# manhtuando97/two-stage-gnn

Measured on AMD Instinct MI355X. Metric: graphs/sec fwd+bwd, DD batch=32 SAGE-3L h=128, higher is better.
Workload: dtype f32; 1 GPU; DD-shaped synthetic graphs (avg 269 nodes / 676 edges, F_in=89), batch=32 per GPU, GcnEncoderGraph (GraphSage 'base') 3 layers h=128, Nmax=1000, slot-BN, CE loss, clip 2.0 + Adam; 1 step(s) per hipGraph launch, seed = rank, 128 untimed settle steps before the warm-up; global_batch=32, parallelism=dp1, launch=hipGraph replay (one graph: forward + backward + bucket + optimiser), rows=8151, edges_directed=40970

## Files before the change

include/tsgnn.h:

```cpp
#ifndef TSGNN_H
#define TSGNN_H
#include <stdint.h>

typedef struct ihipStream_t* tsgnn_stream_t;

#ifdef __cplusplus
extern "C" {
#endif

#define TSGNN_ABI_VERSION 2
int tsgnn_abi_version(void);
const char* tsgnn_strerror(int code);
const char* tsgnn_last_kernel(void);


int tsgnn_scan_workspace_ints(int64_t n, int64_t* ws_ints);
int tsgnn_exclusive_scan_i32(const int* in, int64_t n, int* out, int* ws, tsgnn_stream_t stream);

int tsgnn_row_maps(const int* graph_ptr, int B, int64_t n_rows, int* row_graph, int* row_slot,
                   tsgnn_stream_t stream);

int tsgnn_dense_adj_count(const float* adj, int B, int nmax, const int* graph_ptr, const int* row_graph,
                          int64_t n_rows, int* row_cnt, tsgnn_stream_t stream);
int tsgnn_dense_adj_fill(const float* adj, int B, int nmax, const int* graph_ptr, const int* row_graph,
                         int64_t n_rows, const int* rowptr, int* col, float* val, tsgnn_stream_t stream);

int tsgnn_coo_count(const int64_t* key, int64_t E, int64_t n_rows, int* cnt, int* bad_flag,
                    tsgnn_stream_t stream);
int tsgnn_coo_fill(const int64_t* key, const int64_t* other, int64_t E, int64_t n_rows, const int* rowptr,
                   int* cursor, int* col, int* eid, tsgnn_stream_t stream);


int tsgnn_ingest_layout(int B, int nmax, int64_t row_cap, int ell_w, int64_t tail_cap, int64_t* off);
int tsgnn_host_collate_tu(const int64_t* ds_graph_ptr, const int64_t* ds_rowptr, const int64_t* ds_col, const int64_t* ds_node_label,
                          const int64_t* ds_graph_label, const int64_t* ids, int B, int nmax, int64_t row_cap, int ell_w,
                          int64_t tail_cap, int32_t* staging, int64_t* out);
int tsgnn_onehot_rows_f32(const int* label, int64_t n_rows, int64_t total_rows, int F, float* x, int64_t ldx, tsgnn_stream_t stream);

int tsgnn_ingest_upload_f32(int32_t* dev, const int32_t* host, int64_t words, const int* node_label_dev, int64_t n_rows, int64_t total_rows,
                            int F, float* x, int64_t ldx, tsgnn_stream_t stream);
int tsgnn_ingest_compact_layout(int B, int nmax, int64_t row_cap, int64_t edge_cap, int64_t tail_cap, int64_t* off);
int tsgnn_host_collate_compact(const int64_t* ds_graph_ptr, const int64_t* ds_rowptr, const int64_t* ds_col, const int64_t* ds_node_label,
                               const int64_t* ds_graph_label, const int64_t* ids, int B, int nmax, int64_t row_cap, int64_t edge_cap,
                               int ell_w, int64_t tail_cap, int32_t* staging, int64_t* out);
int tsgnn_ingest_pull_expand_f32(const int32_t* host, int32_t* mirror, int B, int nmax, int64_t row_cap, int64_t edge_cap, int ell_w,
                                 int64_t tail_cap, int32_t* row_graph, int32_t* row_slot, int32_t* ell, int32_t* tail_ptr, int32_t* ell_slots, int32_t* tail_slots, int F, float* x,
                                 int64_t ldx, tsgnn_stream_t stream);
int tsgnn_ingest_pull_expand_ack_f32(const int32_t* host, int32_t* mirror, int B, int nmax, int64_t row_cap, int64_t edge_cap, int ell_w,
                                     int64_t tail_cap, int32_t* row_graph, int32_t* row_slot, int32_t* ell, int32_t* tail_ptr, int32_t* ell_slots, int32_t* tail_slots, int F,
                                     float* x, int64_t ldx, int64_t* host_ack, tsgnn_stream_t stream);
int tsgnn_ingest_pull_f32(const int32_t* host, int32_t* mirror, int B, int nmax, int64_t row_cap, int64_t edge_cap, int64_t tail_cap,
                          tsgnn_stream_t stream);
int tsgnn_ingest_expand_ack_f32(int32_t* mirror, int B, int nmax, int64_t row_cap, int64_t edge_cap, int ell_w, int64_t tail_cap,
                                int32_t* row_graph, int32_t* row_slot, int32_t* ell, int32_t* tail_ptr, int32_t* ell_slots, int32_t* tail_slots, int F, float* x, int64_t ldx,
                                int64_t* host_ack, tsgnn_stream_t stream);
int tsgnn_ingest_arm_pull_rider(const int32_t* host, int32_t* mirror, int B, int nmax, int64_t row_cap, int64_t edge_cap, int64_t tail_cap);
int tsgnn_ingest_arm_pull_rider_parts(const int32_t* host, int32_t* mirror, int B, int nmax, int64_t row_cap, int64_t edge_cap, int64_t tail_cap,
                                      int parts, int skip);
int tsgnn_ingest_arm_expand_rider(int32_t* mirror, int B, int nmax, int64_t row_cap, int64_t edge_cap, int ell_w, int64_t tail_cap,
                                  int32_t* row_graph, int32_t* row_slot, int32_t* ell, int32_t* tail_ptr, int32_t* ell_slots, int32_t* tail_slots, int F, float* x, int64_t ldx,
                                  int64_t* host_ack);
int tsgnn_ingest_flush_pull_rider(tsgnn_stream_t stream);
int tsgnn_ingest_disarm_riders(void);
typedef struct tsgnn_collate_pool tsgnn_collate_pool;
int tsgnn_collate_pool_create(int nthreads, tsgnn_collate_pool** pool);
int tsgnn_collate_pool_submit(tsgnn_collate_pool* pool, const int64_t* ds_graph_ptr, const int64_t* ds_rowptr, const int64_t* ds_col,
                              const int64_t* ds_node_label, const int64_t* ds_graph_label, const int64_t* ids, int B, int nmax,
                              int64_t row_cap, int64_t edge_cap, int ell_w, int64_t tail_cap, int32_t* staging, int64_t* out,
                              void* after_event, int64_t* ticket);
int tsgnn_collate_pool_submit_ack(tsgnn_collate_pool* pool, const int64_t* ds_graph_ptr, const int64_t* ds_rowptr, const int64_t* ds_col,
                                  const int64_t* ds_node_label, const int64_t* ds_graph_label, const int64_t* ids, int B, int nmax,
                                  int64_t row_cap, int64_t edge_cap, int ell_w, int64_t tail_cap, int32_t* staging, int64_t* out,
                                  const int64_t* host_ack, int64_t ack_target, int seq, int64_t* ticket);
int tsgnn_collate_pool_wait(tsgnn_collate_pool* pool, int64_t ticket);
int tsgnn_collate_pool_destroy(tsgnn_collate_pool* pool);

int tsgnn_csr_transpose(const int* rowptr, const int* col, const float* val, int64_t n_rows, int64_t n_cols,
                        int64_t nnz, int* rowptr_t, int* col_t, float* val_t, int* src_e, int* cnt_ws,
                        int* scan_ws, tsgnn_stream_t stream);


int tsgnn_csr_spmm_f32(const int* rowptr, const int* col, const float* val, const float* self_w,
                       const float* x, int64_t ldx, float* y, int64_t ldy, int64_t n_rows, int feat,
                       float self_scalar, int relu_in, int accumulate, tsgnn_stream_t stream);

int tsgnn_csr_to_ell(const int* rowptr, const int* col, int64_t n_rows, int W, int* ell, int* tail_cnt, tsgnn_stream_t stream);
int tsgnn_csr_tail_fill(const int* rowptr, const int* col, const int* tail_ptr, int64_t n_rows, int W, int* tail_col,
                        tsgnn_stream_t stream);
int tsgnn_ell_spmm_f32(const int* ell, int W, const float* x, int64_t ldx, float* y, int64_t ldy, int64_t n_rows, int feat,
                       float self_scalar, tsgnn_stream_t stream);

int tsgnn_gcn_norm_f32(const int* rowptr, const int* col, const float* val, int64_t n_rows, float self_fill,
                       float* dinv, float* val_out, float* self_w, tsgnn_stream_t stream);

int tsgnn_sddmm_rows_f32(const int* rowptr, const int* col, const float* dy, int64_t lddy, const float* x, int64_t ldx,
                         int64_t n_rows, int feat, float* dval, float* dself, tsgnn_stream_t stream);


int tsgnn_gemm_f32(const float* A, int64_t sam, int64_t sak, const float* B, int64_t sbk, int64_t sbn, float* C,
                   int64_t scm, int64_t scn, int M, int N, int K, int batch, int64_t stride_a, int64_t stride_b,
                   int64_t stride_c, const int* seg_ptr, int ragged, int max_seg, float alpha, int accumulate,
                   tsgnn_stream_t stream);
int tsgnn_gemm_splitk_plan(int M, int N, int K, int* ksplit, int64_t* ws_floats);
int tsgnn_gemm_splitk_f32(const float* A, int64_t sam, int64_t sak, const float* B, int64_t sbk, int64_t sbn,
                          float* C, int M, int N, int K, int ksplit, float* ws, int accumulate,
                          tsgnn_stream_t stream);
int tsgnn_linear_wgrad_plan(int64_t rows, int K_in, int N, int64_t ldz, int64_t lddu, int* nslab, int64_t* rows_per_slab,
                            int64_t* ws_floats);
int tsgnn_linear_wgrad_f32(const float* z, int64_t ldz, const float* du, int64_t lddu, int64_t rows, int K_in, int N, int nslab,
                           int64_t rows_per_slab, int64_t bias_only_rows, float* ws, float* dw, float* db, tsgnn_stream_t stream);
int tsgnn_wgrad_reduce_sets_blocks(const int64_t* desc);
int tsgnn_wgrad_reduce_sets_f32(const int64_t* desc, float* normparts, float* step_state, tsgnn_stream_t stream);
int tsgnn_wgrad_reduce_multi_f32(const float* ws0, int nslab0, int K0, int N0, float* dw0, float* db0, const float* ws1, int nslab1,
                                 int K1, int N1, float* dw1, float* db1, const float* ws2, int nslab2, int K2, int N2, float* dw2,
                                 float* db2, const float* ws3, int nslab3, int K3, int N3, float* dw3, float* db3,
                                 float* normparts, float* step_state, tsgnn_stream_t stream);
int tsgnn_wgrad_blocks_plan(int64_t rows, int K_in, int N, int64_t ldz, int64_t lddu, int* nslab, int64_t* rows_per_slab,
                            int64_t* ws_floats);
int tsgnn_wgrad_blocks_f32(const float* z, int64_t ldz, const float* du, int64_t lddu, int64_t rows, int K_in, int N, int nslab,
                           int64_t rows_per_slab, float* ws, float* dw, int64_t lddw, tsgnn_stream_t stream);
int tsgnn_wgrad_blocks_oi_f32(const float* z, int64_t ldz, const float* du, int64_t lddu, int64_t rows, int K_in, int N, int nslab,
                              int64_t rows_per_slab, float* ws, float* dw_oi, int64_t lddw, float* db, tsgnn_stream_t stream);
int tsgnn_ragged_tn_f32(const float* s_mat, int64_t lds_, const float* x, int64_t ldx, int K, int N, const int* slab_row_ptr,
                        int nslab, const int* seg_slab_ptr, int nseg, float* ws, float* out, tsgnn_stream_t stream);
int tsgnn_ragged_tn_direct_supported(int K, int64_t max_rows);
int tsgnn_ragged_tn_direct_f32(const float* s_mat, int64_t lds_, int K, const int* graph_ptr, int B, const float* x0, int64_t ldx0,
                               int N0, float* out0, const float* x1, int64_t ldx1, int N1, float* out1, tsgnn_stream_t stream);
int tsgnn_ragged_tn_direct_ro_f32(const float* s_mat, int64_t lds_, int K, const int* graph_ptr, int B, const float* x0, int64_t ldx0,
                                  int N0, float* out0, const float* x1, int64_t ldx1, int N1, float* out1, float* ro_out,
                                  int64_t ro_ldo, int* ro_arg, int nmax, int64_t n_real, int ghost_zero, tsgnn_stream_t stream);
int tsgnn_wgrad_narrow_plan(int64_t rows, int K_in, int N, int64_t* ws_floats);
int tsgnn_wgrad_narrow_f32(const float* z, int64_t ldz, const float* du, int64_t lddu, int64_t rows, int K_in, int N, float* ws,
                           float* dwb, tsgnn_stream_t stream);
int tsgnn_colsum_f32(const float* x, int64_t ld, int64_t rows, int F, float* out, float* ws, int accumulate,
                     tsgnn_stream_t stream);

int tsgnn_linear_l2norm_f32(const float* z, int64_t ldz, const float* w, int64_t ldw, const float* bias, float* v,
                            int64_t ldv, float* rinv, int64_t rows, int K, int N, int normalize,
                            tsgnn_stream_t stream);
int tsgnn_rowgemm_supported(const float* a, int64_t lda, const float* b, int64_t ldb, const float* c, int64_t ldc, int K, int N,
                            int trans_b);
int tsgnn_rowgemm_f32(const float* a, int64_t lda, const float* b, int64_t ldb, int trans_b, const float* bias, float* c,
                      int64_t ldc, float* rinv, int64_t rows, int K, int N, int normalize, int64_t fill_rows,
                      tsgnn_stream_t stream);
int tsgnn_panel_blocks(int64_t rows, int panel_units);
#define TSGNN_SCHED_8x32 32
#define TSGNN_SCHED_16x24 24
int tsgnn_gather_sched_slots(int64_t rows, int64_t fill_rows, int K, int panel_units, int layer0);
int tsgnn_gather_rowgemm_f32(const int* ell, int ell_w, const int* tail_ptr, const int* tail_col, const float* x, int64_t ldx, const float* b, int64_t ldb, int trans_b,
                             const float* bias, float* c, int64_t ldc, float* rinv, float* zout, int64_t ldz, int64_t rows, int K,
                             int N, int normalize, int64_t fill_rows, tsgnn_stream_t stream);
int tsgnn_gather_rowgemm_st_f32(const int* ell, int ell_w, const int* tail_ptr, const int* tail_col, const float* x, int64_t ldx, const float* b, int64_t ldb, const float* bias,
                                float* c, int64_t ldc, float* rinv, float* zout, int64_t ldz, int64_t rows, int K, int N,
                                int64_t fill_rows, const int* row_slot, unsigned long long* sums, float* ghost, int panel_units,
                                const int64_t* pack_desc, tsgnn_stream_t stream);
int tsgnn_sage_layer_fwd_bn_f32(const int* ell, int ell_w, const int* tail_ptr, const int* tail_col, const float* x, int64_t ldx, const float* w, int64_t ldw, const float* bias,
                                float* v, int64_t ldv, float* rinv, float* zout, int64_t ldz, int64_t rows, int K, int64_t fill_rows,
                                const int* graph_ptr, const int* slot_count, int B, int nslots, int n_ghost, unsigned long long* packed,
                                unsigned long long* packed_out, const int* row_graph, const unsigned long long* sums_in,
                                const float* ghost_in, float* mean_out, float* rstd_out, const int* row_slot,
                                unsigned long long* sums_out, float* ghost_out, const int* ro_map, int ro_map_ch, int panel_units,
                                const float* w_img, tsgnn_stream_t stream);
int tsgnn_sage_layer_fwd_bn_plan(int64_t rows, int64_t fill_rows, int B, int nslots, int panel_units, int* ro_ch, int* n_gemm,
                                 int* n_full);
int tsgnn_sage_layer_fwd_f32(const int* ell, int ell_w, const int* tail_ptr, const int* tail_col, const float* x, int64_t ldx, const float* w, int64_t ldw, const float* bias,
                             float* v, int64_t ldv, float* rinv, float* zout, int64_t ldz, int64_t rows, int K, int64_t fill_rows,
                             const int* graph_ptr, int B, int nslots, int n_ghost, unsigned long long* packed, tsgnn_stream_t stream);
int tsgnn_sage_layer_fwd_ro_f32(const int* ell, int ell_w, const int* tail_ptr, const int* tail_col, const float* x, int64_t ldx, const float* w, int64_t ldw, const float* bias,
                                float* v, int64_t ldv, float* rinv, float* zout, int64_t ldz, int64_t rows, int K, int64_t fill_rows,
                                const int* graph_ptr, int B, int nslots, int n_ghost, unsigned long long* packed,
                                unsigned long long* packed_out, const int* row_graph, tsgnn_stream_t stream);
int tsgnn_sage_layer_bwd_f32(const int* ell, int ell_w, const int* tail_ptr, const int* tail_col, const float* du, int64_t lddu, const float* w, int64_t ldw, float* dxs,
                             int64_t lddxs, const float* z, int64_t ldz, int64_t rows, int nslab, int64_t rows_per_slab,
                             int64_t bias_only_rows, float* ws, int panel_units, const float* w_img, tsgnn_stream_t stream);
int tsgnn_l2norm_bwd_f32(const float* v, int64_t ldv, const float* dv, int64_t lddv, const float* rinv, float* du,
                         int64_t lddu, int64_t rows, int F, tsgnn_stream_t stream);


int tsgnn_bn_slots_fwd_f32(const int* graph_ptr, const int* slot_count, const int* row_slot, int B, int nmax,
                           int64_t n_real, int n_ghost, const float* v, int64_t ldv, int F, int relu, int bn,
                           float* mean, float* rstd, float* y, int64_t ldy, tsgnn_stream_t stream);
int tsgnn_bn_slots_bwd_f32(const int* graph_ptr, const int* slot_count, const int* row_slot, int B, int nmax,
                           int64_t n_real, int n_ghost, const float* v, int64_t ldv, const float* dy, int64_t lddy, int F,
                           int relu, int bn, const float* mean, const float* rstd, float* m1, float* m2, float* dv,
                           int64_t lddv, tsgnn_stream_t stream);

int tsgnn_row_ln_fwd_f32(const float* v, int64_t ldv, int64_t rows, int F, int relu, float* mean, float* rstd, float* y, int64_t ldy,
                         tsgnn_stream_t stream);
int tsgnn_row_ln_bwd_f32(const float* v, int64_t ldv, const float* dy, int64_t lddy, int64_t rows, int F, int relu, const float* mean,
                         const float* rstd, float* dv, int64_t lddv, tsgnn_stream_t stream);

int tsgnn_row_post_bwd_f32(const int* row_graph, int B, int64_t n_real, int64_t rows, const float* v, int64_t ldv, const float* dxs,
                           int64_t lddxs, const float* dout, int64_t ldo, const int* arg, int F, int relu, int ln, const float* mean,
                           const float* rstd, const float* rinv, float* du, int64_t lddu, tsgnn_stream_t stream);

int tsgnn_row_post_nodes_bwd_f32(int64_t n_real, int64_t rows, const float* v, int64_t ldv, const float* dxs, int64_t lddxs,
                                 const float* dnode, int64_t lddn, int ghost_zero, int F, int relu, int ln, const float* mean,
                                 const float* rstd, const float* rinv, float* du, int64_t lddu, tsgnn_stream_t stream);

int tsgnn_readout_max_ws_words(int B, int nmax, int F);
int tsgnn_readout_max_fwd_f32(const int* graph_ptr, const int* slot_count, int B, int nmax, int64_t n_real, int n_ghost,
                              const float* x, int64_t ldx, int F, int relu, unsigned long long* packed_ws, float* out,
                              int64_t ldo, int* arg, tsgnn_stream_t stream);
int tsgnn_readout_max_bwd_f32(const float* dout, int64_t ldo, const int* arg, int B, int F, const float* x, int64_t ldx_in,
                              int relu, int64_t n_real, float* dx, int64_t ldx, tsgnn_stream_t stream);
int tsgnn_readout_max_bwd_rows_f32(const float* dout, int64_t ldo, const int* arg, const int* row_graph, int F, int64_t rows,
                                   int64_t rows_total, const float* add, int64_t ldadd, float* dx, int64_t ldx, tsgnn_stream_t stream);

int tsgnn_pack_rows_f32(const float* src, int nmax, int F, const int* row_graph, const int* row_slot, int64_t n_real,
                        float* dst, int64_t ld, tsgnn_stream_t stream);
int tsgnn_unpack_rows_f32(const int* graph_ptr, int B, int nmax, int64_t n_real, int n_ghost, const float* src, int64_t ld,
                          int F, float fill, float* dst, tsgnn_stream_t stream);
int tsgnn_unpack_rows_bwd_ghost_f32(const int* graph_ptr, int B, int nmax, int64_t n_real, const float* ddst, int F,
                                    float* dsrc, int64_t ld, tsgnn_stream_t stream);


int tsgnn_softmax_ce_f32(const float* logits, int64_t ld, const int64_t* label, int B, int C, float* loss, float* dlogits,
                         tsgnn_stream_t stream);
int tsgnn_adam_from_partials_f32(float* param, const float* grad, float* m, float* v, int64_t n, float lr, float beta1, float beta2,
                                 float eps, float weight_decay, float max_norm, float* state, const float* parts, int nparts,
                                 const float* poison, tsgnn_stream_t stream);
int tsgnn_clip_adam_step_f32(float* param, const float* grad, float* m, float* v, int64_t n, float lr, float beta1,
                             float beta2, float eps, float weight_decay, float max_norm, float grad_scale, float* state,
                             float* ws, const float* poison, tsgnn_stream_t stream);


int tsgnn_dense_stack_supported(int B, int K, int nstack, int L, int fin0, int hidden, int last0, int last1);
int tsgnn_dense_stack_fwd_f32(const int64_t* desc, tsgnn_stream_t stream);
int tsgnn_dense_stack_bwd_f32(const int64_t* desc, tsgnn_stream_t stream);
int tsgnn_dense_stack_max_resident(void);
int tsgnn_dense_stack_barrier_selftest(unsigned* sync, float* err, int expect, tsgnn_stream_t stream);


int tsgnn_node_scores_f32(const float* x, int64_t ldx, int64_t rows, int H, int Fh, const float* a, int64_t lda, float* s,
                          tsgnn_stream_t stream);
int tsgnn_node_scores2_f32(const float* x, int64_t ldx, int64_t rows, int H, int Fh, const float* a1, int64_t lda1, float* s1,
                           const float* a2, int64_t lda2, float* s2, tsgnn_stream_t stream);
int tsgnn_edge_softmax_fwd_f32(const int* rowptr, const int* col, int64_t rows, int H, const float* s_grp, const float* s_oth,
                               int mod, float slope, float* alpha, tsgnn_stream_t stream);
int tsgnn_edge_softmax_bwd_f32(const int* rowptr, const int* col, int64_t rows, int H, const float* s_grp, const float* s_oth,
                               int mod, float slope, const float* alpha, const float* dalpha, float* dt, float* ds_grp,
                               tsgnn_stream_t stream);
int tsgnn_edge_permute_f32(const float* src, const int* perm, int64_t n, int H, int scatter, float* dst, tsgnn_stream_t stream);
int tsgnn_csr_row_sum_f32(const int* rowptr, const float* val, int64_t rows, int H, float* out, tsgnn_stream_t stream);
int tsgnn_csr_row_sum_perm_f32(const int* rowptr, const float* val, const int* eperm, int64_t rows, int H, float* out,
                               tsgnn_stream_t stream);
int tsgnn_csr_spmm_heads_f32(const int* rowptr, const int* col, const float* alpha, int H, int Fh, const float* x, int64_t ldx,
                             int mod, float* y, int64_t ldy, int64_t rows, tsgnn_stream_t stream);
int tsgnn_csr_spmm_heads_epi_f32(const int* rowptr, const int* col, const float* alpha, int H, int Fh, const float* x, int64_t ldx,
                                 int mod, float* y, int64_t ldy, int64_t rows, const float* w1, const float* a1, int64_t lda1,
                                 const float* w2, const float* a2, int64_t lda2, const float* u, int64_t ldu, const float* uw,
                                 int rows_per_seg, const int* row_seg, float uscale, const int* eperm, tsgnn_stream_t stream);
int tsgnn_csr_sddmm_heads_f32(const int* rowptr, const int* col, int H, int Fh, const float* dy, int64_t lddy, const float* x,
                              int64_t ldx, int mod, float* dalpha, int64_t rows, tsgnn_stream_t stream);
int tsgnn_segment_wsum_f32(const float* x, int64_t ldx, const float* w, int H, int Fh, const int* seg_ptr, int nseg, int64_t rows,
                           int64_t max_seg, float scale, int mean, float* ws, float* out, int64_t ldo, tsgnn_stream_t stream);
int tsgnn_segment_wsum2_f32(const float* x, int64_t ldx, const float* w1, const float* w2, int H, int Fh, const int* seg_ptr, int nseg,
                            int64_t rows, int64_t max_seg, float scale, float* ws, float* out1, float* out2, int64_t ldo,
                            tsgnn_stream_t stream);
int tsgnn_gather_wsum_f32(const float* x, int64_t ldx, const int* idx, const float* w, const int* seg_ptr, int nseg, int C, float scale,
                          float* out, int64_t ldo, tsgnn_stream_t stream);
int tsgnn_broadcast_add_f32(float* y, int64_t ldy, int64_t rows, int H, int Fh, const float* w, const float* a, int64_t lda,
                            const float* u, int64_t ldu, int rows_per_seg, float scale, tsgnn_stream_t stream);
int tsgnn_pack_heads_max(void);
int tsgnn_pack_heads_f32(const float* w0, const float* w1, const float* w2, const float* w3, const float* w4, const float* w5,
                         const float* w6, const float* w7, const float* a0, const float* a1, const float* a2, const float* a3,
                         const float* a4, const float* a5, const float* a6, const float* a7, int H, int Fin, int Fo, float* W, float* A,
                         tsgnn_stream_t stream);
int tsgnn_unpack_heads_f32(const float* dW, const float* dA0, const float* dA1, int H, int Fin, int Fo, float* gw, float* ga,
                           tsgnn_stream_t stream);

int tsgnn_gat_fused_supported(int H, int Fh);
int tsgnn_gat_attn_fwd_f32(const float* hp, int64_t ldh, const int* rowptr, const int* col, const int* rp_t, const int* col_t,
                           int64_t rows, int H, int Fh, float slope, const int* row_graph, int nmax, const int* iso_idx,
                           const float* iso_w, const int* iso_ptr, float uscale, int mean_heads, int apply_elu, float drop_p,
                           uint64_t seed, const unsigned long long* drop_ctr, float* stat, float* y, int64_t ldy, tsgnn_stream_t stream);
int tsgnn_gat_bwd_parts(int B);
int tsgnn_gat_attn_bwd_f32(const float* hp, int64_t ldh, const float* y, int64_t ldy, const float* dy, int64_t lddy, const int* rp_t,
                           const int* col_t, int64_t rows, int H, int Fh, float slope, int mean_heads, int apply_elu,
                           const int* graph_ptr, int B, const int* iso_idx, const float* iso_w, const int* iso_ptr,
                           const float* iso_row, int iso_row_ld, float uscale, float drop_p, uint64_t seed,
                           const unsigned long long* drop_ctr, const float* stat, float* dhp, int Ns, float* t1, float* t2, float* S,
                           float* dupart, tsgnn_stream_t stream);
int tsgnn_gat_attn_bwd_ro_f32(const float* hp, int64_t ldh, const float* y, int64_t ldy, const float* dy, int64_t lddy, const int* rp_t,
                              const int* col_t, int64_t rows, int H, int Fh, float slope, int mean_heads, int apply_elu,
                              const int* graph_ptr, int B, const int* iso_idx, const float* iso_w, const int* iso_ptr,
                              const float* iso_row, int iso_row_ld, float uscale, float drop_p, uint64_t seed,
                              const unsigned long long* drop_ctr, const float* stat, float* dhp, int Ns, float* t1, float* t2, float* S,
                              float* dupart, const float* ro_dout, int64_t ro_ldo, const int* ro_arg, const int* row_graph,
                              tsgnn_stream_t stream);
int tsgnn_gat_dropout_mult_f32(float drop_p, uint64_t seed, const unsigned long long* drop_ctr, int64_t i0, int64_t ni, int64_t j0,
                               int64_t nj, int H, float* out, tsgnn_stream_t stream);
int tsgnn_gat_score_rowsum_f32(const int* rowptr, const int* col, const int* eperm, const float* t1, const float* t2, const float* S,
                               int64_t rows, int H, float* dhp, int64_t ldh, int C, const float* dupart, int B, const int* iso_idx,
                               const float* iso_w, const int* iso_ptr, float uscale, tsgnn_stream_t stream);
int tsgnn_gat_pack_desc_words(void);
int tsgnn_gat_pack_f32(const int64_t* desc, tsgnn_stream_t stream);
int tsgnn_gat_unpack_f32(const int64_t* desc, tsgnn_stream_t stream);
int tsgnn_elu_heads_fwd_f32(const float* x, int64_t rows, int H, int Fh, int mean_heads, int apply_elu, float* y, tsgnn_stream_t stream);
int tsgnn_elu_heads_bwd_f32(const float* x, const float* dy, int64_t rows, int H, int Fh, int mean_heads, int apply_elu, float* dx,
                            tsgnn_stream_t stream);


int tsgnn_mlp3_supported(int B, int D0, int D1, int D2, int C);
int tsgnn_mlp3_fwd_f32(const float* x, int64_t ldx, const float* w1, const float* b1, const float* keep, float keep_scale, const float* w2,
                       const float* b2, const float* w3, const float* b3, int B, int D0, int D1, int D2, int C, float* a1, float* a2,
                       float* logp, tsgnn_stream_t stream);
int tsgnn_mlp3_fwd_drop_f32(const float* x, int64_t ldx, const float* w1, const float* b1, float p, uint64_t seed,
                            unsigned long long* state, unsigned long long* used, const float* w2, const float* b2, const float* w3,
                            const float* b3, int B, int D0, int D1, int D2, int C, float* a1, float* a2, float* logp,
                            tsgnn_stream_t stream);
int tsgnn_mlp3_dropout_mask_f32(float p, uint64_t seed, uint64_t counter, int B, int D1, float* out, tsgnn_stream_t stream);
int tsgnn_mlp3_bwd_f32(const float* x, int64_t ldx, const float* w1, const float* w2, const float* w3, const float* a1,
                       const float* a2, const float* logp, const float* dlogp, float keep_scale, int B, int D0, int D1, int D2, int C,
                       float* dw1, float* db1, float* dw2, float* db2, float* dw3, float* db3, float* dx, int64_t lddx,
// ... 306 lines not shown
```

two-stage-gnn_amd/csrc/head.hip:

```cpp
#include "common.h"
#include "../../include/tsgnn.h"
#include "readout_body.h"
#include "ingest_rider.h"

namespace {

__device__ __forceinline__ float4 ld4(const float* p) { return *reinterpret_cast<const float4*>(p); }
__device__ __forceinline__ float pick4(const float (&r)[4], int q) { return q == 0 ? r[0] : q == 1 ? r[1] : q == 2 ? r[2] : r[3]; }

constexpr int HW = 16;

__device__ __forceinline__ void head2_fwd_tail(const float* xs, float* vs, int b, const float* __restrict__ w1,
                                               const float* __restrict__ b1, const float* __restrict__ w2, const float* __restrict__ b2,
                                               int P, int E, int C, float* __restrict__ vec, float* __restrict__ y) {
  const int tid = threadIdx.x, lane = tid & 63, wid = tid >> 6;
  const int P4 = P >> 2;
  for (int j0 = wid; j0 < E; j0 += 8 * HW) {
    float acc[8];
#pragma unroll
    for (int u = 0; u < 8; ++u) acc[u] = 0.f;
    for (int k4 = lane; k4 < P4; k4 += 64) {
      const float4 x = *reinterpret_cast<const float4*>(xs + 4 * k4);
      float4 w[8];
#pragma unroll
      for (int u = 0; u < 8; ++u) {
        const int j = j0 + HW * u;
        w[u] = ld4(w1 + (int64_t)(j < E ? j : 0) * P + 4 * k4);
      }
#pragma unroll
      for (int u = 0; u < 8; ++u) acc[u] += (w[u].x * x.x + w[u].y * x.y) + (w[u].z * x.z + w[u].w * x.w);
    }
#pragma unroll
    for (int u = 0; u < 8; ++u) {
      const int j = j0 + HW * u;
      const float r = wave_sum(acc[u]);
      if (lane == 0 && j < E) { const float v = r + (b1 ? b1[j] : 0.f); vs[j] = v; vec[(int64_t)b * E + j] = v; }
    }
  }
  __syncthreads();
  for (int c = wid; c < C; c += HW) {
    float acc = 0.f;
    for (int j = lane; j < E; j += 64) acc = fmaf(w2[(int64_t)c * E + j], vs[j], acc);
    acc = wave_sum(acc);
    if (lane == 0) y[(int64_t)b * C + c] = acc + (b2 ? b2[c] : 0.f);
  }
}

struct RoTail {
  const float* z; int64_t ldz; int N, c0, F;
  int* arg;
  float* dz; int64_t lddz;
};

__global__ __launch_bounds__(64 * HW) void head2_fwd_kernel(float* __restrict__ out, int64_t ldo, const float* __restrict__ w1,
                                                        const float* __restrict__ b1, const float* __restrict__ w2,
                                                        const float* __restrict__ b2, int P, int E, int C,
                                                        float* __restrict__ vec, float* __restrict__ y, RoTail rt) {
  extern __shared__ __attribute__((aligned(16))) float smem[];
  float* xs = smem;
  float* vs = smem + ((P + 3) & ~3);
  const int b = blockIdx.x, tid = threadIdx.x;
  const int c0 = rt.z ? rt.c0 : P;
  for (int k = tid; k < P; k += 64 * HW) {
    if (k < c0) { xs[k] = out[(int64_t)b * ldo + k]; continue; }
    const int f = k - c0;
    unsigned long long best = 0ull;
    for (int n0 = 0; n0 < rt.N; n0 += 16) {
      float val[16];
#pragma unroll
      for (int u = 0; u < 16; ++u) val[u] = rt.z[((int64_t)b * rt.N + min(n0 + u, rt.N - 1)) * rt.ldz + f];
#pragma unroll
      for (int u = 0; u < 16; ++u) {
        if (n0 + u < rt.N) {
          const unsigned long long q = ((unsigned long long)f32_ordered(val[u]) << 32) |
                                       (unsigned long long)(0xFFFFFFFFu - (unsigned)(b * rt.N + n0 + u));
          best = q > best ? q : best;
        }
      }
    }
    const float v = best ? ordered_f32((unsigned)(best >> 32)) : 0.f;
    xs[k] = v;
    out[(int64_t)b * ldo + k] = v;
    rt.arg[(int64_t)b * rt.F + f] = best ? (int)(0xFFFFFFFFu - (unsigned)(best & 0xFFFFFFFFull)) : -1;
  }
  __syncthreads();
  head2_fwd_tail(xs, vs, b, w1, b1, w2, b2, P, E, C, vec, y);
}

struct ReadoutHeadArgs {
  const unsigned long long* packed; int B, L, Fh, Fl;
  const float* v_last; int64_t ldv;
  const int* graph_ptr; int64_t n_real; int nslots; int n_ghost;
  float* out; int64_t ldo; int* arg;
};
__global__ __launch_bounds__(64 * HW) void readout_head_fwd_kernel(ReadoutHeadArgs a, const float* __restrict__ w1,
                                                               const float* __restrict__ b1, const float* __restrict__ w2,
                                                               const float* __restrict__ b2, int P, int E, int C,
                                                               float* __restrict__ vec, float* __restrict__ y) {
  extern __shared__ __attribute__((aligned(16))) float smem[];
  float* xs = smem;
  float* vs = smem + ((P + 3) & ~3);
  unsigned long long* best = reinterpret_cast<unsigned long long*>(smem + ((P + 3) & ~3) + ((E + 3) & ~3));
  const int b = blockIdx.x, tid = threadIdx.x;
  const int PH = (a.L - 1) * a.Fh;
  for (int k = tid; k < PH; k += 64 * HW) {
    const int l = k / a.Fh, f = k % a.Fh;
    const int64_t i = (int64_t)l * a.B * a.Fh + (int64_t)b * a.Fh + f;
    const unsigned long long p = a.packed[i];
    const float val = p ? ordered_f32((unsigned)(p >> 32)) : 0.f;
    xs[k] = val;
    a.out[(int64_t)b * a.ldo + k] = val;
    a.arg[i] = p ? (int)(0xFFFFFFFFu - (unsigned)(p & 0xFFFFFFFFull)) : -1;
  }
  {
    const int c4 = tid & 31, rl = tid >> 5, F4 = a.Fl >> 2;
    const int g0 = a.graph_ptr[b], sz = a.graph_ptr[b + 1] - g0;
    unsigned long long m0 = 0ull, m1 = 0ull, m2 = 0ull, m3 = 0ull;
    if (c4 < F4) {
      const int nrows = sz + ((a.n_ghost && sz < a.nslots) ? 1 : 0);
      for (int n0 = rl; n0 < nrows; n0 += 8 * HW) {
        float4 t[4];
        int64_t r[4];
#pragma unroll
        for (int u = 0; u < 4; ++u) {
          const int n = n0 + 2 * HW * u;
          r[u] = n < sz ? (int64_t)g0 + n : a.n_real + n;
          t[u] = n < nrows ? ld4(a.v_last + r[u] * a.ldv + 4 * c4) : make_float4(0.f, 0.f, 0.f, 0.f);
        }
#pragma unroll
        for (int u = 0; u < 4; ++u) {
          if (n0 + 2 * HW * u < nrows) {
            const unsigned long long p0 = pack_max(t[u].x, (unsigned)r[u]), p1 = pack_max(t[u].y, (unsigned)r[u]),
                                     p2 = pack_max(t[u].z, (unsigned)r[u]), p3 = pack_max(t[u].w, (unsigned)r[u]);
            m0 = p0 > m0 ? p0 : m0; m1 = p1 > m1 ? p1 : m1; m2 = p2 > m2 ? p2 : m2; m3 = p3 > m3 ? p3 : m3;
          }
        }
      }
      best[rl * a.Fl + 4 * c4 + 0] = m0; best[rl * a.Fl + 4 * c4 + 1] = m1; best[rl * a.Fl + 4 * c4 + 2] = m2; best[rl * a.Fl + 4 * c4 + 3] = m3;
    }
    __syncthreads();
    for (int f = tid; f < a.Fl; f += 64 * HW) {
      unsigned long long m = best[f];
      for (int w = 1; w < 2 * HW; ++w) { const unsigned long long o = best[w * a.Fl + f]; m = o > m ? o : m; }
      const float val = m ? ordered_f32((unsigned)(m >> 32)) : 0.f;
      xs[PH + f] = val;
      a.out[(int64_t)b * a.ldo + PH + f] = val;
      a.arg[(int64_t)(a.L - 1) * a.B * a.Fh + (int64_t)b * a.Fl + f] = m ? (int)(0xFFFFFFFFu - (unsigned)(m & 0xFFFFFFFFull)) : -1;
    }
  }
  __syncthreads();
  head2_fwd_tail(xs, vs, b, w1, b1, w2, b2, P, E, C, vec, y);
}

template <int NJ>
__global__ __launch_bounds__(64 * HW) void packed_head_fwd_kernel(const unsigned long long* __restrict__ packed, int B, int L, int Fh,
                                                              int Fl, float* __restrict__ out, int64_t ldo, int* __restrict__ arg,
                                                              const float* __restrict__ w1, const float* __restrict__ b1,
                                                              const float* __restrict__ w2, const float* __restrict__ b2, int P, int E,
                                                              int C, float* __restrict__ vec, float* __restrict__ y, ExpandRider rider,
                                                              unsigned long long* __restrict__ clear, int64_t clear_n, int clear_packed) {
  extern __shared__ __attribute__((aligned(16))) float smem[];
  if ((int)blockIdx.x >= B) {
    expand_rider_body(rider, blockIdx.x - (unsigned)B, 64 * HW);
    return;
  }
  for (int64_t i2 = (int64_t)blockIdx.x * (64 * HW) + threadIdx.x; i2 < clear_n; i2 += (int64_t)B * (64 * HW)) clear[i2] = 0ull;
  float* xs = smem;
  float* vs = smem + ((P + 3) & ~3);
  const int b = blockIdx.x, tid = threadIdx.x, lane = tid & 63, wid = tid >> 6;
  const int PH = (L - 1) * Fh, P4 = P >> 2;
  unsigned long long pk[2];
  int64_t pidx[2];
#pragma unroll
  for (int u = 0; u < 2; ++u) {
    const int k = tid + u * 64 * HW;
    int64_t idx = 0;
    if (k < P) {
      if (k < PH) { const int l = k / Fh, f = k - l * Fh; idx = (int64_t)l * B * Fh + (int64_t)b * Fh + f; }
      else idx = (int64_t)(L - 1) * B * Fh + (int64_t)b * Fl + (k - PH);
    }
    pidx[u] = idx;
    pk[u] = packed[idx];
    if (k >= P) pk[u] = 0ull;
  }
  float4 w[NJ][2];
#pragma unroll
  for (int u = 0; u < NJ; ++u) {
    const int j = wid + HW * u;
    const float* row = w1 + (int64_t)(j < E ? j : 0) * P;
    w[u][0] = ld4(row + 4 * (lane < P4 ? lane : 0));
    w[u][1] = ld4(row + 4 * (lane + 64 < P4 ? lane + 64 : 0));
  }
#pragma unroll
  for (int u = 0; u < NJ; ++u) {
    if (lane >= P4) w[u][0] = make_float4(0.f, 0.f, 0.f, 0.f);
    if (lane + 64 >= P4) w[u][1] = make_float4(0.f, 0.f, 0.f, 0.f);
  }
  float bj[NJ];
#pragma unroll
  for (int u = 0; u < NJ; ++u) { const int j = wid + HW * u; bj[u] = (b1 && j < E) ? b1[j] : 0.f; }
  float w2v[4];
#pragma unroll
  for (int q = 0; q < 4; ++q) { const int j = lane + 64 * q; w2v[q] = (wid < C && j < E) ? w2[(int64_t)wid * E + j] : 0.f; }
  const float b2v = (b2 && wid < C) ? b2[wid] : 0.f;
#pragma unroll
  for (int u = 0; u < 2; ++u) {
    const int k = tid + u * 64 * HW;
    if (k < P) {
      const unsigned long long p = pk[u];
      const float val = p ? ordered_f32((unsigned)(p >> 32)) : 0.f;
      xs[k] = val;
      out[(int64_t)b * ldo + k] = val;
      arg[pidx[u]] = p ? (int)(0xFFFFFFFFu - (unsigned)(p & 0xFFFFFFFFull)) : -1;
      if (clear_packed) const_cast<unsigned long long*>(packed)[pidx[u]] = 0ull;
    }
  }
  __syncthreads();
  {
    const float4 x0 = lane < P4 ? *reinterpret_cast<const float4*>(xs + 4 * lane) : make_float4(0.f, 0.f, 0.f, 0.f);
    const float4 x1 = lane + 64 < P4 ? *reinterpret_cast<const float4*>(xs + 4 * (lane + 64)) : make_float4(0.f, 0.f, 0.f, 0.f);
    float acc[NJ];
#pragma unroll
    for (int u = 0; u < NJ; ++u)
      acc[u] = ((w[u][0].x * x0.x + w[u][0].y * x0.y) + (w[u][0].z * x0.z + w[u][0].w * x0.w)) +
               ((w[u][1].x * x1.x + w[u][1].y * x1.y) + (w[u][1].z * x1.z + w[u][1].w * x1.w));
    for (int k4 = lane + 128; k4 < P4; k4 += 64) {
      const float4 x = *reinterpret_cast<const float4*>(xs + 4 * k4);
#pragma unroll
      for (int u = 0; u < NJ; ++u) {
        const int j = wid + HW * u;
        const float4 t = ld4(w1 + (int64_t)(j < E ? j : 0) * P + 4 * k4);
        acc[u] += (t.x * x.x + t.y * x.y) + (t.z * x.z + t.w * x.w);
      }
    }
#pragma unroll
    for (int u = 0; u < NJ; ++u) {
      const int j = wid + HW * u;
      const float r = wave_sum(acc[u]);
      if (lane == 0 && j < E) { const float v = r + bj[u]; vs[j] = v; vec[(int64_t)b * E + j] = v; }
    }
  }
  __syncthreads();
  for (int c = wid; c < C; c += HW) {
    float acc = 0.f;
    if (c == wid && E <= 256) {
#pragma unroll
      for (int q = 0; q < 4; ++q) { const int j = lane + 64 * q; if (j < E) acc = fmaf(w2v[q], vs[j], acc); }
    } else {
      for (int j = lane; j < E; j += 64) acc = fmaf(w2[(int64_t)c * E + j], vs[j], acc);
    }
    acc = wave_sum(acc);
    if (lane == 0) y[(int64_t)b * C + c] = acc + ((c == wid) ? b2v : (b2 ? b2[c] : 0.f));
  }
}

__device__ __forceinline__ void head2_bwd_rows(float* smem, int b, const float* __restrict__ dy, const float* __restrict__ dvec,
                                               const float* __restrict__ w1, const float* __restrict__ w2, int P, int E, int C,
                                               float* __restrict__ dout, int64_t ldo) {
  float* ds = smem;
  float* part = smem + ((E + 3) & ~3);
  const int tid = threadIdx.x, wid = tid >> 6, lane = tid & 63;
  for (int j = tid; j < E; j += 64 * HW) {
    float acc = dvec ? dvec[(int64_t)b * E + j] : 0.f;
    for (int c = 0; c < C; ++c) acc = fmaf(dy[(int64_t)b * C + c], w2[(int64_t)c * E + j], acc);
    ds[j] = acc;
  }
  __syncthreads();
  const int P4 = P >> 2;
  for (int k4 = lane; k4 < P4 + ((P & 3) ? 1 : 0); k4 += 64) {
    float4 acc = make_float4(0.f, 0.f, 0.f, 0.f);
    if (k4 < P4) {
      for (int j = wid; j < E; j += HW) {
        const float4 w = ld4(w1 + (int64_t)j * P + 4 * k4);
        const float d = ds[j];
        acc.x = fmaf(d, w.x, acc.x); acc.y = fmaf(d, w.y, acc.y); acc.z = fmaf(d, w.z, acc.z); acc.w = fmaf(d, w.w, acc.w);
      }
      *reinterpret_cast<float4*>(part + wid * ((P + 3) & ~3) + 4 * k4) = acc;
    } else {
      for (int k = 4 * P4; k < P; ++k) {
        float a = 0.f;
        for (int j = wid; j < E; j += HW) a = fmaf(ds[j], w1[(int64_t)j * P + k], a);
        part[wid * ((P + 3) & ~3) + k] = a;
      }
    }
  }
  __syncthreads();
  const int PP = (P + 3) & ~3;
  for (int k = tid; k < P; k += 64 * HW) {
    float a = 0.f;
#pragma unroll
    for (int w = 0; w < HW; ++w) a += part[w * PP + k];
    dout[(int64_t)b * ldo + k] = a;
  }
}

__device__ __forceinline__ void head2_bwd_weights(float* smem , int jb, const float* __restrict__ out, int64_t ldo,
                                                  const float* __restrict__ vec, const float* __restrict__ dy,
                                                  const float* __restrict__ dvec, const float* __restrict__ w2, int B, int P, int E,
                                                  int C, float* __restrict__ dw1, float* __restrict__ db1, float* __restrict__ dw2,
                                                  float* __restrict__ db2, float* __restrict__ normparts) {
  const int tid = threadIdx.x, NTH = 64 * HW;
  const int nj = (E + 3) / 4;
  float sq = 0.f;
  if (jb < nj) {
    const int j0 = 4 * jb;
    for (int i = tid; i < B * 4; i += NTH) {
      const int bb = i >> 2, jj = j0 + (i & 3);
      float a = 0.f;
      if (jj < E) {
        a = dvec ? dvec[(int64_t)bb * E + jj] : 0.f;
        for (int c = 0; c < C; ++c) a = fmaf(dy[(int64_t)bb * C + c], w2[(int64_t)c * E + jj], a);
      }
      smem[i] = a;
    }
    __syncthreads();
    for (int k = tid; k < P; k += NTH) {
      float a0 = 0.f, a1 = 0.f, a2 = 0.f, a3 = 0.f;
      int bb = 0;
      for (; bb + 8 <= B; bb += 8) {
        float x[8];
#pragma unroll
        for (int u = 0; u < 8; ++u) x[u] = out[(int64_t)(bb + u) * ldo + k];
#pragma unroll
        for (int u = 0; u < 8; ++u) {
          const float4 d = *reinterpret_cast<const float4*>(smem + 4 * (bb + u));
          a0 = fmaf(d.x, x[u], a0); a1 = fmaf(d.y, x[u], a1); a2 = fmaf(d.z, x[u], a2); a3 = fmaf(d.w, x[u], a3);
        }
      }
      for (; bb < B; ++bb) {
        const float x = out[(int64_t)bb * ldo + k];
        a0 = fmaf(smem[4 * bb + 0], x, a0); a1 = fmaf(smem[4 * bb + 1], x, a1);
        a2 = fmaf(smem[4 * bb + 2], x, a2); a3 = fmaf(smem[4 * bb + 3], x, a3);
      }
      if (j0 + 0 < E) { dw1[(int64_t)(j0 + 0) * P + k] = a0; sq = fmaf(a0, a0, sq); }
      if (j0 + 1 < E) { dw1[(int64_t)(j0 + 1) * P + k] = a1; sq = fmaf(a1, a1, sq); }
      if (j0 + 2 < E) { dw1[(int64_t)(j0 + 2) * P + k] = a2; sq = fmaf(a2, a2, sq); }
      if (j0 + 3 < E) { dw1[(int64_t)(j0 + 3) * P + k] = a3; sq = fmaf(a3, a3, sq); }
    }
    if (db1 && tid < 4 && j0 + tid < E) {
      float a = 0.f;
      for (int bb = 0; bb < B; ++bb) a += smem[4 * bb + tid];
      db1[j0 + tid] = a;
      sq = fmaf(a, a, sq);
    }
  } else {
    for (int i = tid; i < C * E; i += NTH) {
      const int c = i / E, j = i % E;
      float a = 0.f;
      for (int bb = 0; bb < B; ++bb) a = fmaf(dy[(int64_t)bb * C + c], vec[(int64_t)bb * E + j], a);
      dw2[i] = a;
      sq = fmaf(a, a, sq);
    }
    if (db2) for (int c = tid; c < C; c += NTH) {
      float a = 0.f;
      for (int bb = 0; bb < B; ++bb) a += dy[(int64_t)bb * C + c];
      db2[c] = a;
      sq = fmaf(a, a, sq);
    }
  }
  if (normparts) {
    sq = wave_sum(sq);
    __syncthreads();
    if ((tid & 63) == 0) smem[tid >> 6] = sq;
    __syncthreads();
    if (tid == 0) {
      float t = 0.f;
      for (int w = 0; w < HW; ++w) t += smem[w];
      normparts[jb] = t;
    }
  }
}

__global__ __launch_bounds__(64 * HW) void head2_bwd_kernel(const float* __restrict__ out, int64_t ldo, const float* __restrict__ vec,
                                                        const float* __restrict__ dy, const float* __restrict__ dvec,
                                                        const float* __restrict__ w1, const float* __restrict__ w2, int B, int P, int E,
                                                        int C, float* __restrict__ dout, int64_t lddo, float* __restrict__ dw1,
                                                        float* __restrict__ db1, float* __restrict__ dw2, float* __restrict__ db2,
                                                        float* __restrict__ normparts, const float* __restrict__ ce_y,
                                                        const int64_t* __restrict__ ce_label, float* __restrict__ ce_loss) {
  extern __shared__ __attribute__((aligned(16))) float smem_all[];
  float* smem = smem_all;
  if (ce_label != nullptr) {
    float* dyl = smem_all;
    float* lb = smem_all + ((B * C + 3) & ~3);
    smem = lb + ((B + 3) & ~3);
    const float invB = 1.f / (float)B;
    const bool all_rows = (int)blockIdx.x >= B || blockIdx.x == 0;
    for (int b = all_rows ? (int)threadIdx.x : (int)blockIdx.x + (int)threadIdx.x * B; b < B; b += 64 * HW) {
      const float* row = ce_y + (int64_t)b * C;
      float m = -INFINITY;
      for (int c = 0; c < C; ++c) m = fmaxf(m, row[c]);
      float d = 0.f;
// ... 313 lines not shown
#pragma unroll
    for (int u = 0; u < WB_ROWS; ++u) {
      const int bb = bg + G * u;
      x[u] = ld4(out + (int64_t)((active && bb < B) ? bb : 0) * ldo + 4 * (active ? k4 : 0));
    }
    if (has_ce) { ce_rows(ce, B, C, dyl, lb, -1); __syncthreads(); }
    for (int i = tid; i < 4 * B; i += NTH) {
      const int bb = i >> 2, jj = j0 + (i & 3);
      float a = 0.f;
      if (jj < E) {
        a = i == tid ? dv0 : (dvec ? dvec[(int64_t)bb * E + jj] : 0.f);
        for (int c = 0; c < C; ++c) a = fmaf(dy[(int64_t)bb * C + c], (i == tid && c < 4) ? pick4(w2r, c) : w2[(int64_t)c * E + jj], a);
      }
      dvs[i] = a;
    }
    __syncthreads();
    float4 a0 = make_float4(0.f, 0.f, 0.f, 0.f), a1 = a0, a2 = a0, a3 = a0;
    for (int b0 = 0; b0 < B; b0 += G * WB_ROWS) {
      if (b0 > 0) {
#pragma unroll
        for (int u = 0; u < WB_ROWS; ++u) {
          const int bb = b0 + bg + G * u;
          x[u] = ld4(out + (int64_t)((active && bb < B) ? bb : 0) * ldo + 4 * (active ? k4 : 0));
        }
      }
#pragma unroll
      for (int u = 0; u < WB_ROWS; ++u) {
        const int bb = b0 + bg + G * u;
        if (active && bb < B) {
          const float4 d = *reinterpret_cast<const float4*>(dvs + 4 * bb);
          a0.x = fmaf(d.x, x[u].x, a0.x); a0.y = fmaf(d.x, x[u].y, a0.y); a0.z = fmaf(d.x, x[u].z, a0.z); a0.w = fmaf(d.x, x[u].w, a0.w);
          a1.x = fmaf(d.y, x[u].x, a1.x); a1.y = fmaf(d.y, x[u].y, a1.y); a1.z = fmaf(d.y, x[u].z, a1.z); a1.w = fmaf(d.y, x[u].w, a1.w);
          a2.x = fmaf(d.z, x[u].x, a2.x); a2.y = fmaf(d.z, x[u].y, a2.y); a2.z = fmaf(d.z, x[u].z, a2.z); a2.w = fmaf(d.z, x[u].w, a2.w);
          a3.x = fmaf(d.w, x[u].x, a3.x); a3.y = fmaf(d.w, x[u].y, a3.y); a3.z = fmaf(d.w, x[u].z, a3.z); a3.w = fmaf(d.w, x[u].w, a3.w);
        }
      }
    }
    if (active) {
      float* pp = part + (int64_t)bg * 4 * PP + 4 * k4;
      *reinterpret_cast<float4*>(pp) = a0; *reinterpret_cast<float4*>(pp + PP) = a1;
      *reinterpret_cast<float4*>(pp + 2 * PP) = a2; *reinterpret_cast<float4*>(pp + 3 * PP) = a3;
    }
    __syncthreads();
    for (int i = tid; i < 4 * P; i += NTH) {
      const int jj = i / P, k = i - jj * P;
      if (j0 + jj < E) {
        float a = 0.f;
        for (int q = 0; q < G; ++q) a += part[(q * 4 + jj) * PP + k];
        dw1[(int64_t)(j0 + jj) * P + k] = a;
        sq = fmaf(a, a, sq);
      }
    }
    if (db1 && tid < 4 && j0 + tid < E) {
      float a = 0.f;
      for (int bb = 0; bb < B; ++bb) a += dvs[4 * bb + tid];
      db1[j0 + tid] = a;
      sq = fmaf(a, a, sq);
    }
  } else {
    if (has_ce) { ce_rows(ce, B, C, dyl, lb, -1); __syncthreads(); }
    for (int i = tid; i < C * E; i += NTH) {
      const int c = i / E, j = i - c * E;
      float a = 0.f;
      int bb = 0;
      for (; bb + 8 <= B; bb += 8) {
        float v[8];
#pragma unroll
        for (int u = 0; u < 8; ++u) v[u] = vec[(int64_t)(bb + u) * E + j];
#pragma unroll
        for (int u = 0; u < 8; ++u) a = fmaf(dy[(int64_t)(bb + u) * C + c], v[u], a);
      }
      for (; bb < B; ++bb) a = fmaf(dy[(int64_t)bb * C + c], vec[(int64_t)bb * E + j], a);
      dw2[i] = a;
      sq = fmaf(a, a, sq);
    }
    if (db2) for (int c = tid; c < C; c += NTH) {
      float a = 0.f;
      for (int bb = 0; bb < B; ++bb) a += dy[(int64_t)bb * C + c];
      db2[c] = a;
      sq = fmaf(a, a, sq);
    }
  }
  if (normparts) {
    sq = wave_sum(sq);
    __syncthreads();
    if ((tid & 63) == 0) smem[tid >> 6] = sq;
    __syncthreads();
    if (tid == 0) {
      float t = 0.f;
      for (int w = 0; w < HW; ++w) t += smem[w];
      normparts[jb] = t;
    }
  }
}

}

extern "C" {

int tsgnn_head2_fwd_f32(const float* out, int64_t ldo, const float* w1, const float* b1, const float* w2, const float* b2, int B, int P,
                        int E, int C, float* vec, float* y, tsgnn_stream_t stream) {
  if (!out || !w1 || !w2 || !vec || !y || B <= 0 || P <= 0 || E <= 0 || C <= 0 || ldo < P) return TSGNN_EINVAL;
  if ((P % 4) || P > 4096 || E > 4096 || (reinterpret_cast<uintptr_t>(w1) & 15)) return TSGNN_EUNSUPPORTED;
  const size_t lds = sizeof(float) * (size_t)(((P + 3) & ~3) + E);
  TSGNN_KNAME("head2_fwd_kernel");
  head2_fwd_kernel<<<B, 64 * HW, lds, stream>>>(const_cast<float*>(out), ldo, w1, b1, w2, b2, P, E, C, vec, y, RoTail{});
  TSGNN_CHECK_LAUNCH();
  return TSGNN_OK;
}

int tsgnn_head2_fwd_ro_f32(float* out, int64_t ldo, const float* w1, const float* b1, const float* w2, const float* b2, int B, int P,
                           int E, int C, float* vec, float* y, const float* z, int64_t ldz, int N, int c0, int F, int* arg,
                           tsgnn_stream_t stream) {
  if (!out || !w1 || !w2 || !vec || !y || !z || !arg || B <= 0 || P <= 0 || E <= 0 || C <= 0 || ldo < P || N <= 0 || F <= 0 || c0 < 0 ||
      c0 + F != P || ldz < F)
    return TSGNN_EINVAL;
  if ((P % 4) || P > 4096 || E > 4096 || N > 64 || (reinterpret_cast<uintptr_t>(w1) & 15)) return TSGNN_EUNSUPPORTED;
  const size_t lds = sizeof(float) * (size_t)(((P + 3) & ~3) + E);
  TSGNN_KNAME("head2_fwd_kernel(ro)");
  head2_fwd_kernel<<<B, 64 * HW, lds, stream>>>(out, ldo, w1, b1, w2, b2, P, E, C, vec, y, RoTail{z, ldz, N, c0, F, arg, nullptr, 0});
  TSGNN_CHECK_LAUNCH();
  return TSGNN_OK;
}

int tsgnn_readout_head_fwd_f32(const unsigned long long* packed, int B, int L, int Fh, int Fl, const float* v_last, int64_t ldv,
                               const int* graph_ptr, int64_t n_real, int nslots, int n_ghost, float* out, int64_t ldo, int* arg,
                               const float* w1, const float* b1, const float* w2, const float* b2, int E, int C, float* vec, float* y,
                               tsgnn_stream_t stream) {
  if (!packed || !v_last || !graph_ptr || !out || !arg || !w1 || !w2 || !vec || !y || B <= 0 || L <= 0 || Fh <= 0 || Fl <= 0 ||
      E <= 0 || C <= 0 || nslots <= 0 || (n_ghost != 0 && n_ghost != nslots))
    return TSGNN_EINVAL;
  const int P = (L - 1) * Fh + Fl;
  if ((P % 4) || P > 4096 || E > 4096 || (Fl % 4) || Fl > 128 || (ldv % 4) || ldo < P || (reinterpret_cast<uintptr_t>(w1) & 15) ||
      (reinterpret_cast<uintptr_t>(v_last) & 15))
    return TSGNN_EUNSUPPORTED;
  ReadoutHeadArgs a{packed, B, L, Fh, Fl, v_last, ldv, graph_ptr, n_real, nslots, n_ghost, out, ldo, arg};
  const size_t lds = sizeof(float) * (size_t)(((P + 3) & ~3) + ((E + 3) & ~3)) + sizeof(unsigned long long) * (size_t)(2 * HW) * Fl;
  TSGNN_KNAME("readout_head_fwd_kernel");
  readout_head_fwd_kernel<<<B, 64 * HW, lds, stream>>>(a, w1, b1, w2, b2, P, E, C, vec, y);
  TSGNN_CHECK_LAUNCH();
  return TSGNN_OK;
}

int tsgnn_packed_head_fwd_f32(const unsigned long long* packed, int B, int L, int Fh, int Fl, float* out, int64_t ldo, int* arg,
                              const float* w1, const float* b1, const float* w2, const float* b2, int E, int C, float* vec, float* y,
                              tsgnn_stream_t stream) {
  if (!packed || !out || !arg || !w1 || !w2 || !vec || !y || B <= 0 || L <= 0 || Fh <= 0 || Fl <= 0 || E <= 0 || C <= 0) return TSGNN_EINVAL;
  const int P = (L - 1) * Fh + Fl;
  if ((P % 4) || P > 2048 || E > 8 * HW || ldo < P || (reinterpret_cast<uintptr_t>(w1) & 15)) return TSGNN_EUNSUPPORTED;
  const size_t lds = sizeof(float) * (size_t)(((P + 3) & ~3) + ((E + 3) & ~3));
  const ExpandRider rider = take_expand_rider();
  TSGNN_KNAME("packed_head_fwd_kernel<8>");
  packed_head_fwd_kernel<8><<<(unsigned)B + rider.blocks, 64 * HW, lds, stream>>>(packed, B, L, Fh, Fl, out, ldo, arg, w1, b1, w2, b2, P, E, C,
                                                                               vec, y, rider, nullptr, 0, 0);
  TSGNN_CHECK_LAUNCH();
  return TSGNN_OK;
}

int tsgnn_packed_head_fwd_z_f32(unsigned long long* packed, int B, int L, int Fh, int Fl, float* out, int64_t ldo, int* arg,
                                const float* w1, const float* b1, const float* w2, const float* b2, int E, int C, float* vec, float* y,
                                unsigned long long* clear, int64_t clear_n, tsgnn_stream_t stream) {
  if (!packed || !out || !arg || !w1 || !w2 || !vec || !y || B <= 0 || L <= 0 || Fh <= 0 || Fl <= 0 || E <= 0 || C <= 0 || clear_n < 0 ||
      (clear_n > 0 && !clear))
    return TSGNN_EINVAL;
  const int P = (L - 1) * Fh + Fl;
  if ((P % 4) || P > 2048 || E > 8 * HW || ldo < P || (reinterpret_cast<uintptr_t>(w1) & 15)) return TSGNN_EUNSUPPORTED;
  const size_t lds = sizeof(float) * (size_t)(((P + 3) & ~3) + ((E + 3) & ~3));
  const ExpandRider rider = take_expand_rider();
  TSGNN_KNAME("packed_head_fwd_kernel<8>");
  packed_head_fwd_kernel<8><<<(unsigned)B + rider.blocks, 64 * HW, lds, stream>>>(packed, B, L, Fh, Fl, out, ldo, arg, w1, b1, w2, b2, P, E, C,
                                                                               vec, y, rider, clear, clear_n, 1);
  TSGNN_CHECK_LAUNCH();
  return TSGNN_OK;
}

static int head2_bwd_launch(const float* out, int64_t ldo, const float* vec, const float* dy, const float* dvec, const float* w1,
                            const float* w2, int B, int P, int E, int C, float* dout, int64_t lddo, float* dw1, float* db1,
                            float* dw2, float* db2, float* normparts, const float* ce_y, const int64_t* ce_label, float* ce_loss,
                            tsgnn_stream_t stream, const DuArgs* du = nullptr, const RoTail* rtail = nullptr, int du_map_n = 0,
                            int du_map_chunk = 64, int du_compact = 0) {
  if (!out || !vec || (!dy && !ce_label) || !w1 || !w2 || !dout || !dw1 || !dw2 || B <= 0 || P <= 0 || E <= 0 || C <= 0) return TSGNN_EINVAL;
  if (ce_label && (!ce_y || !ce_loss)) return TSGNN_EINVAL;
  if ((P % 4) || P > 2048 || E > 4096 || B > 1024 || (reinterpret_cast<uintptr_t>(w1) & 15)) return TSGNN_EUNSUPPORTED;
  if ((ldo % 4) == 0 && (lddo % 4) == 0 && !((reinterpret_cast<uintptr_t>(out) | reinterpret_cast<uintptr_t>(dout)) & 15) && (P / 4) <= 512) {
    const int P4 = P / 4;
    const int Gr = 64 * HW / P4 < 16 ? 64 * HW / P4 : 16;
    const int Gw = 768 / P4 < 1 ? 1 : (768 / P4 > 8 ? 8 : 768 / P4);
    size_t role = (size_t)((E + 3) & ~3) + (size_t)Gr * P;
    const size_t wrole = 4 * (size_t)((B + 3) & ~3) + (size_t)Gw * 4 * P;
    if (wrole > role) role = wrole;
    if (role < HW) role = HW;
    size_t lds2 = sizeof(float) * role;
    DuArgs dua{};
    const RoTail rt = rtail ? *rtail : RoTail{};
    unsigned du_blocks = 0;
    int du_chunk = 64;
    if (du) {
      dua = *du;
      const int ncu = device_cu_count();
      const int nodes = dua.chunks;
      const int other = B + (E + 3) / 4 + 1;
      unsigned compact_blocks = 0;
      if (dua.map) du_chunk = du_map_chunk;
      else if (du_compact && B <= 64) {
        constexpr unsigned PADB = 4;
        unsigned n64 = (unsigned)((dua.n_real + 63) / 64) + (unsigned)B;
        if (other + (int)(n64 + PADB) > ncu) { du_chunk = 128; n64 = (unsigned)((dua.n_real + 127) / 128) + (unsigned)B; }
        compact_blocks = n64 + PADB;
        dua.compact = other;
      }
      else if ((B + 1) * ((nodes + 63) / 64) + other > ncu + ncu / 5) du_chunk = 128;
      dua.chunks = (nodes + du_chunk - 1) / du_chunk;
      const int G = 64 * HW / P4 < 16 ? 64 * HW / P4 : 16;
      const size_t drole = (size_t)((E + 3) & ~3) + (size_t)(G + 1) * dua.F;
      if (drole > role) role = drole;
      du_blocks = dua.map ? (unsigned)du_map_n : (compact_blocks ? compact_blocks : (unsigned)(B + 1) * (unsigned)dua.chunks);
    }
    lds2 = sizeof(float) * role;
    if (ce_label) lds2 += sizeof(float) * (size_t)(((B * C + 3) & ~3) + ((B + 3) & ~3));
    if (lds2 <= 160 * 1024 - 1024) {
      static size_t attr_set = 0;
      if (lds2 > 64 * 1024 && lds2 > attr_set) {
        (void)hipFuncSetAttribute(reinterpret_cast<const void*>(head2_bwd2_kernel<64>), hipFuncAttributeMaxDynamicSharedMemorySize, (int)lds2);
        (void)hipFuncSetAttribute(reinterpret_cast<const void*>(head2_bwd2_kernel<128>), hipFuncAttributeMaxDynamicSharedMemorySize, (int)lds2);
        attr_set = lds2;
      }
      TSGNN_KNAME(du_chunk == 128 ? "head2_bwd2_kernel<128>" : "head2_bwd2_kernel<64>");
      if (du_chunk == 128)
        head2_bwd2_kernel<128><<<B + (E + 3) / 4 + 1 + du_blocks, 64 * HW, lds2, stream>>>(out, ldo, vec, dy, dvec, w1, w2, B, P, E, C, dout, lddo,
                                                                                        dw1, db1, dw2, db2, normparts,
                                                                                        CeArgs{ce_y, ce_label, ce_loss}, dua, rt);
      else
        head2_bwd2_kernel<64><<<B + (E + 3) / 4 + 1 + du_blocks, 64 * HW, lds2, stream>>>(out, ldo, vec, dy, dvec, w1, w2, B, P, E, C, dout, lddo,
                                                                                       dw1, db1, dw2, db2, normparts,
                                                                                       CeArgs{ce_y, ce_label, ce_loss}, dua, rt);
      TSGNN_CHECK_LAUNCH();
      return TSGNN_OK;
    }
  }
  if (du || rtail) return TSGNN_EUNSUPPORTED;
  size_t lds = sizeof(float) * (size_t)(((E + 3) & ~3) + HW * ((P + 3) & ~3));
  if (lds < sizeof(float) * (4 * (size_t)B + HW)) lds = sizeof(float) * (4 * (size_t)B + HW);
  if (ce_label) lds += sizeof(float) * (size_t)(((B * C + 3) & ~3) + ((B + 3) & ~3));
  TSGNN_KNAME("head2_bwd_kernel");
  head2_bwd_kernel<<<B + (E + 3) / 4 + 1, 64 * HW, lds, stream>>>(out, ldo, vec, dy, dvec, w1, w2, B, P, E, C, dout, lddo, dw1, db1, dw2,
                                                                db2, normparts, ce_y, ce_label, ce_loss);
  TSGNN_CHECK_LAUNCH();
  return TSGNN_OK;
}

int tsgnn_head2_bwd_f32(const float* out, int64_t ldo, const float* vec, const float* dy, const float* dvec, const float* w1,
                        const float* w2, int B, int P, int E, int C, float* dout, int64_t lddo, float* dw1, float* db1,
                        float* dw2, float* db2, float* normparts, tsgnn_stream_t stream) {
  return head2_bwd_launch(out, ldo, vec, dy, dvec, w1, w2, B, P, E, C, dout, lddo, dw1, db1, dw2, db2, normparts, nullptr, nullptr,
                          nullptr, stream);
}

int tsgnn_head2_bwd_ro_f32(const float* out, int64_t ldo, const float* vec, const float* dy, const float* dvec, const float* w1,
                           const float* w2, int B, int P, int E, int C, float* dout, int64_t lddo, float* dw1, float* db1,
                           float* dw2, float* db2, float* normparts, const int* arg, int c0, int F, int N, float* dz, int64_t lddz,
                           const float* ce_y, const int64_t* ce_label, float* ce_loss, tsgnn_stream_t stream) {
  if (!arg || !dz || N <= 0 || F <= 0 || c0 < 0 || c0 + F > P || lddz < F) return TSGNN_EINVAL;
  if ((dy == nullptr) == (ce_label == nullptr)) return TSGNN_EINVAL;
  const RoTail rt{nullptr, 0, N, c0, F, const_cast<int*>(arg), dz, lddz};
  return head2_bwd_launch(out, ldo, vec, dy, dvec, w1, w2, B, P, E, C, dout, lddo, dw1, db1, dw2, db2, normparts, ce_y, ce_label,
                          ce_loss, stream, nullptr, &rt);
}

int tsgnn_head2_bwd_ce_f32(const float* out, int64_t ldo, const float* vec, const float* y, const int64_t* label, float* loss,
                           const float* dvec, const float* w1, const float* w2, int B, int P, int E, int C, float* dout, int64_t lddo,
                           float* dw1, float* db1, float* dw2, float* db2, float* normparts, tsgnn_stream_t stream) {
  if (!y || !label || !loss) return TSGNN_EINVAL;
  return head2_bwd_launch(out, ldo, vec, nullptr, dvec, w1, w2, B, P, E, C, dout, lddo, dw1, db1, dw2, db2, normparts, y, label, loss,
                          stream);
}

int tsgnn_head2_bwd_du_f32(const float* out, int64_t ldo, const float* vec, const float* y, const int64_t* label, float* loss,
                           const float* dy, const float* dvec, const float* w1, const float* w2, int B, int P, int E, int C, float* dout,
                           int64_t lddo, float* dw1, float* db1, float* dw2, float* db2, float* normparts, const int* graph_ptr,
                           int64_t n_real, int n_ghost_rows, int max_nodes, const float* v, int64_t ldv, const float* rinv, const int* arg,
                           int seg_off, int F, float* du, int64_t lddu, tsgnn_stream_t stream) {
  return tsgnn_head2_bwd_du_map_f32(out, ldo, vec, y, label, loss, dy, dvec, w1, w2, B, P, E, C, dout, lddo, dw1, db1, dw2, db2, normparts,
                                    graph_ptr, n_real, n_ghost_rows, max_nodes, v, ldv, rinv, arg, seg_off, F, du, lddu, nullptr, 0, 64, stream);
}

int tsgnn_head2_bwd_du_map_f32(const float* out, int64_t ldo, const float* vec, const float* y, const int64_t* label, float* loss,
                               const float* dy, const float* dvec, const float* w1, const float* w2, int B, int P, int E, int C,
                               float* dout, int64_t lddo, float* dw1, float* db1, float* dw2, float* db2, float* normparts,
                               const int* graph_ptr, int64_t n_real, int n_ghost_rows, int max_nodes, const float* v, int64_t ldv,
                               const float* rinv, const int* arg, int seg_off, int F, float* du, int64_t lddu, const int* du_map,
                               int n_map, int du_chunk, tsgnn_stream_t stream) {
  if (du_map && (n_map <= 0 || (du_chunk != 64 && du_chunk != 128) || max_nodes > 255 * du_chunk || B > (1 << 22))) return TSGNN_EINVAL;
  const int compact = (!du_map && n_map < 0) ? 1 : 0;
  const int chunks = max_nodes;
  if (!graph_ptr || !v || !rinv || !arg || !du || n_real < 0 || n_ghost_rows < 0 || chunks <= 0 || F <= 0 || seg_off < 0) return TSGNN_EINVAL;
  if ((y == nullptr) == (dy == nullptr)) return TSGNN_EINVAL;
  if (y && (!label || !loss)) return TSGNN_EINVAL;
  if ((F % 4) || F > 128 || (seg_off % 4) || seg_off + F > P || (ldv % 4) || (lddu % 4) || ldv < F || lddu < F || chunks > (1 << 20) ||
      ((reinterpret_cast<uintptr_t>(v) | reinterpret_cast<uintptr_t>(du) | reinterpret_cast<uintptr_t>(arg)) & 15))
    return TSGNN_EUNSUPPORTED;
  if ((n_real + 1024 + B) * (ldv > lddu ? ldv : lddu) >= (int64_t)1 << 30 || (int64_t)E * P >= (int64_t)1 << 30) return TSGNN_EUNSUPPORTED;
  {
    const int P4 = P / 4, G = P4 > 0 ? (64 * HW / P4 < 16 ? 64 * HW / P4 : 16) : 0;
    if ((P % 4) || G < 1 || E > G * RB_ROWS || G * 32 > 64 * HW) return TSGNN_EUNSUPPORTED;
  }
  const DuArgs a{graph_ptr, n_real, n_ghost_rows, chunks, v, ldv, rinv, arg, seg_off, F, du, lddu, du_map, 0};
  return head2_bwd_launch(out, ldo, vec, dy, dvec, w1, w2, B, P, E, C, dout, lddo, dw1, db1, dw2, db2, normparts, y, label, loss, stream, &a,
                          nullptr, n_map, du_chunk, compact);
}

}
```

two-stage-gnn_amd/csrc/layer_fwd.hip:

```cpp
#include "common.h"
#include "../../include/tsgnn.h"
#include "rowgemm_body.h"
#include "readout_body.h"
#include "ingest_rider.h"

namespace {

template <bool RO>
__global__ __launch_bounds__(256) void sage_layer_fwd_kernel(RowGemmArgs ga, SlotArgs sa, unsigned n_gemm, unsigned ro_gx, int F4,
                                                             unsigned long long* __restrict__ packed, unsigned n_main, PullRider pr) {
  extern __shared__ __attribute__((aligned(16))) float smem[];
  if (blockIdx.x < n_gemm) {
    rowgemm_body<4, false, true, 1, RO>(ga, smem, blockIdx.x);
  } else if (blockIdx.x < n_main) {
    const unsigned r = blockIdx.x - n_gemm;
    readout_partial_body<32>(sa, ga.a, ga.lda, F4, packed, r % ro_gx, r / ro_gx, reinterpret_cast<unsigned long long*>(smem));
  } else {
    pull_rider_body(pr, blockIdx.x - n_main);
  }
}

template <bool RO, bool ST, bool UNITS = false, bool BIMG = false, int SCHED = 0>
__global__ __launch_bounds__(256, 2) void sage_layer_fwd_bn_kernel(RowGemmArgs ga, SlotArgs sa, BnReadArgs bn, unsigned n_gemm, unsigned ro_gx,
                                                                int ro_ch, int F4, unsigned long long* __restrict__ packed, unsigned n_main,
                                                                PullRider pr, const int* __restrict__ ro_map) {
  extern __shared__ __attribute__((aligned(16))) float smem[];
  if (blockIdx.x < n_gemm) {
    rowgemm_body<4, false, true, 1, RO, true, ST, UNITS, BIMG, SCHED>(ga, smem, blockIdx.x);
  } else if (blockIdx.x < n_main) {
    unsigned r = blockIdx.x - n_gemm;
    if (ro_map) r = (unsigned)ro_map[r];
    readout_partial_bn_body<32>(sa, bn, ga.a, ga.lda, F4, packed, r % ro_gx, r / ro_gx, ro_ch, reinterpret_cast<unsigned long long*>(smem));
  } else {
    pull_rider_body(pr, blockIdx.x - n_main);
  }
}

}

extern "C" {

int tsgnn_sage_layer_fwd_bn_plan(int64_t rows, int64_t fill_rows, int B, int nslots, int panel_units, int* ro_ch, int* n_gemm, int* n_full) {
  if (!ro_ch || !n_gemm || !n_full || rows <= 0 || B <= 0 || nslots <= 0) return TSGNN_EINVAL;
  const int ncu = device_cu_count();
  int unit_ = 16;
  const unsigned ng = panel_split(rows, ncu, panel_units, n_full, &unit_) + (fill_rows > 0 ? 1u : 0u);
  int ch = 64;
  while (ch < 256 && ng + (unsigned)((nslots + ch - 1) / ch) * (unsigned)B > 2u * (unsigned)ncu) ch *= 2;
  *ro_ch = ch; *n_gemm = (int)ng;
  return TSGNN_OK;
}

int tsgnn_sage_layer_fwd_bn_f32(const int* ell, int ell_w, const int* tail_ptr, const int* tail_col, const float* x, int64_t ldx, const float* w, int64_t ldw, const float* bias,
                                float* v, int64_t ldv, float* rinv, float* zout, int64_t ldz, int64_t rows, int K, int64_t fill_rows,
                                const int* graph_ptr, const int* slot_count, int B, int nslots, int n_ghost, unsigned long long* packed,
                                unsigned long long* packed_out, const int* row_graph, const unsigned long long* sums_in,
                                const float* ghost_in, float* mean_out, float* rstd_out, const int* row_slot,
                                unsigned long long* sums_out, float* ghost_out, const int* ro_map, int ro_map_ch, int panel_units,
                                const float* w_img, tsgnn_stream_t stream) {
  if (!ell || !x || !w || !v || !rinv || !graph_ptr || !slot_count || !packed || !sums_in || !ghost_in || !mean_out || !rstd_out ||
      rows <= 0 || fill_rows < 0 || K <= 0 || B <= 0 || nslots <= 0 || (n_ghost != 0 && n_ghost != nslots) || (packed_out && !row_graph) ||
      (row_slot && (!sums_out || !ghost_out)))
    return TSGNN_EINVAL;
  const bool sched = ell_w == TSGNN_SCHED_8x32;
  if (sched && (tail_ptr || tail_col)) return TSGNN_EINVAL;
  if (!sched && ell_w != 4 && ell_w != 8 && ell_w != 16) return TSGNN_EUNSUPPORTED;
  const uintptr_t al = reinterpret_cast<uintptr_t>(ell) | reinterpret_cast<uintptr_t>(x) | reinterpret_cast<uintptr_t>(w) |
                       reinterpret_cast<uintptr_t>(v) | reinterpret_cast<uintptr_t>(zout) | reinterpret_cast<uintptr_t>(bias) |
                       reinterpret_cast<uintptr_t>(sums_in) | reinterpret_cast<uintptr_t>(sums_out) | reinterpret_cast<uintptr_t>(w_img);
  if ((al & 15) || K != 128 || (ldx % 4) || (ldw % 4) || (ldv % 4) || (zout && (ldz % 4 || ldz < K)) || ldx < K || ldw < 128 || ldv < 128 ||
      nslots > BN_TAB || rows >= (1 << 20) || n_ghost == 0 || (packed_out && row_slot))
    return TSGNN_EUNSUPPORTED;
  if (packed_out && fill_rows <= 0) return TSGNN_EUNSUPPORTED;
  if ((tail_ptr == nullptr) != (tail_col == nullptr)) return TSGNN_EINVAL;
  RowGemmArgs ga{x, ldx, w, ldw, bias, v, ldv, rinv, rows, K, 128, 1, fill_rows, ell, ell_w, zout, ldz, tail_ptr, tail_col,
                 packed_out, graph_ptr, row_graph, B, nslots, n_ghost};
  ga.st_row_slot = row_slot; ga.st_sums = sums_out; ga.st_ghost = ghost_out;
  ga.b_img = reinterpret_cast<const float4*>(w_img);
  ga.bn_sums = sums_in; ga.bn_ghost = ghost_in; ga.bn_slot_count = slot_count; ga.bn_B = B; ga.bn_nslots = nslots; ga.bn_F = K;
  SlotArgs sa{graph_ptr, slot_count, B, nslots, rows, n_ghost};
  BnReadArgs bn{sums_in, ghost_in, K, mean_out, rstd_out};
  const int ncu = device_cu_count();
  const unsigned n_gemm = panel_split(rows, ncu, panel_units, &ga.n_full, &ga.unit) + (fill_rows > 0 ? 1u : 0u);
  int ro_ch = 64;
  while (ro_ch < 256 && n_gemm + (unsigned)((nslots + ro_ch - 1) / ro_ch) * (unsigned)B > 2u * (unsigned)ncu) ro_ch *= 2;
  const unsigned ro_gx = (unsigned)((nslots + ro_ch - 1) / ro_ch);
  if (ro_map && ro_map_ch != ro_ch) ro_map = nullptr;
  size_t lds = w_img ? rowgemm_lds_bytes<4, false, true, 1, true, true>() : rowgemm_lds_bytes<4, false, true, 1, true>();
  const size_t lro = 8 * 128 * sizeof(unsigned long long) + 256 * sizeof(float2);
  if (lds < lro) lds = lro;
  const unsigned n_main = n_gemm + ro_gx * (unsigned)B;
  if (sched && ga.n_full > 0) return TSGNN_EUNSUPPORTED;
  const PullRider pr = take_pull_rider();
  const bool units = ga.unit == 8 || ga.unit == 16;
#define TSGNN_FWD_BN_(RO_, ST_, UN_, IM_, SC_) \
  sage_layer_fwd_bn_kernel<RO_, ST_, UN_, IM_, SC_><<<n_main + pr.blocks, 256, lds, stream>>>(ga, sa, bn, n_gemm, ro_gx, ro_ch, K / 4, packed, n_main, pr, ro_map)
#define TSGNN_FWD_BN(RO_, ST_)                                                                  \
  do {                                                                                          \
    if (units) { if (w_img) TSGNN_FWD_BN_(RO_, ST_, true, true, 0); else TSGNN_FWD_BN_(RO_, ST_, true, false, 0); }   \
    else if (sched) { if (w_img) TSGNN_FWD_BN_(RO_, ST_, false, true, TSGNN_SCHED_8x32); else TSGNN_FWD_BN_(RO_, ST_, false, false, TSGNN_SCHED_8x32); } \
    else { if (w_img) TSGNN_FWD_BN_(RO_, ST_, false, true, 0); else TSGNN_FWD_BN_(RO_, ST_, false, false, 0); }       \
  } while (0)
  if (packed_out) {
    TSGNN_KNAME("sage_layer_fwd_bn_kernel<true,false,%s>", units ? "true" : "false");
    TSGNN_FWD_BN(true, false);
  } else if (row_slot) {
    TSGNN_KNAME("sage_layer_fwd_bn_kernel<false,true,%s>", units ? "true" : "false");
    TSGNN_FWD_BN(false, true);
  } else {
    TSGNN_KNAME("sage_layer_fwd_bn_kernel<false,false,%s>", units ? "true" : "false");
    TSGNN_FWD_BN(false, false);
  }
#undef TSGNN_FWD_BN
#undef TSGNN_FWD_BN_
  TSGNN_CHECK_LAUNCH();
  return TSGNN_OK;
}

int tsgnn_sage_layer_fwd_ro_f32(const int* ell, int ell_w, const int* tail_ptr, const int* tail_col, const float* x, int64_t ldx, const float* w, int64_t ldw, const float* bias,
                                float* v, int64_t ldv, float* rinv, float* zout, int64_t ldz, int64_t rows, int K, int64_t fill_rows,
                                const int* graph_ptr, int B, int nslots, int n_ghost, unsigned long long* packed,
                                unsigned long long* packed_out, const int* row_graph, tsgnn_stream_t stream) {
  if (!ell || !x || !w || !v || !rinv || !graph_ptr || !packed || rows <= 0 || fill_rows < 0 || K <= 0 || B <= 0 || nslots <= 0 ||
      (n_ghost != 0 && n_ghost != nslots) || (packed_out && !row_graph))
    return TSGNN_EINVAL;
  if (ell_w != 4 && ell_w != 8 && ell_w != 16) return TSGNN_EUNSUPPORTED;
  const uintptr_t al = reinterpret_cast<uintptr_t>(ell) | reinterpret_cast<uintptr_t>(x) | reinterpret_cast<uintptr_t>(w) |
                       reinterpret_cast<uintptr_t>(v) | reinterpret_cast<uintptr_t>(zout) | reinterpret_cast<uintptr_t>(bias);
  if ((al & 15) || K != 128 || (ldx % 4) || (ldw % 4) || (ldv % 4) || (zout && (ldz % 4 || ldz < K)) || ldx < K || ldw < 128 || ldv < 128)
    return TSGNN_EUNSUPPORTED;
  if ((tail_ptr == nullptr) != (tail_col == nullptr)) return TSGNN_EINVAL;
  if (packed_out && n_ghost && fill_rows <= 0) return TSGNN_EUNSUPPORTED;
  RowGemmArgs ga{x, ldx, w, ldw, bias, v, ldv, rinv, rows, K, 128, 1, fill_rows, ell, ell_w, zout, ldz, tail_ptr, tail_col,
                 packed_out, graph_ptr, row_graph, B, nslots, n_ghost};
  SlotArgs sa{graph_ptr, nullptr, B, nslots, rows, n_ghost};
  const unsigned n_gemm = (unsigned)ceil_div64(rows, 32) + (fill_rows > 0 ? 1u : 0u);
  const unsigned ro_gx = (unsigned)((nslots + 63) / 64);
  size_t lds = rowgemm_lds_bytes<4, false, true>();
  if (lds < 8 * 128 * sizeof(unsigned long long)) lds = 8 * 128 * sizeof(unsigned long long);
  const unsigned n_main = n_gemm + ro_gx * (unsigned)B;
  const PullRider pr = take_pull_rider();
  if (packed_out) {
    TSGNN_KNAME("sage_layer_fwd_kernel<true>");
    sage_layer_fwd_kernel<true><<<n_main + pr.blocks, 256, lds, stream>>>(ga, sa, n_gemm, ro_gx, K / 4, packed, n_main, pr);
  } else {
    TSGNN_KNAME("sage_layer_fwd_kernel<false>");
    sage_layer_fwd_kernel<false><<<n_main + pr.blocks, 256, lds, stream>>>(ga, sa, n_gemm, ro_gx, K / 4, packed, n_main, pr);
  }
  TSGNN_CHECK_LAUNCH();
  return TSGNN_OK;
}

int tsgnn_sage_layer_fwd_f32(const int* ell, int ell_w, const int* tail_ptr, const int* tail_col, const float* x, int64_t ldx, const float* w, int64_t ldw, const float* bias,
                             float* v, int64_t ldv, float* rinv, float* zout, int64_t ldz, int64_t rows, int K, int64_t fill_rows,
                             const int* graph_ptr, int B, int nslots, int n_ghost, unsigned long long* packed, tsgnn_stream_t stream) {
  return tsgnn_sage_layer_fwd_ro_f32(ell, ell_w, tail_ptr, tail_col, x, ldx, w, ldw, bias, v, ldv, rinv, zout, ldz, rows, K, fill_rows,
                                     graph_ptr, B, nslots, n_ghost, packed, nullptr, nullptr, stream);
}

}
```

two-stage-gnn_amd/csrc/rowgemm.hip:

```cpp
#include "common.h"
#include "../../include/tsgnn.h"

#include <cstdlib>
#include "rowgemm_body.h"
#include "ingest_rider.h"
#include "pack_body.h"
#include "rowgemm_big_body.h"

namespace {

inline unsigned ks2_max_blocks() {
  static const unsigned n = [] { const char* e = getenv("TSGNN_KS2_MAX_BLOCKS"); return e ? (unsigned)atoi(e) : (unsigned)device_cu_count(); }();
  return n;
}
inline bool rowgemm_ks2_enabled() {
  static const bool on = [] { const char* e = getenv("TSGNN_ROWGEMM_KS2"); return !(e && e[0] == '0'); }();
  return on;
}

template <int NT, bool TRANS_B, bool GATHER>
__global__ __launch_bounds__(256) void rowgemm_kernel(RowGemmArgs g) {
  extern __shared__ __attribute__((aligned(16))) float smem[];
  rowgemm_body<NT, TRANS_B, GATHER>(g, smem, blockIdx.x);
}
// ... 66 lines not shown
template <int U, bool TRANS_B>
void launch_big(const RowGemmArgs& g, hipStream_t s) {
  constexpr size_t lds = rowgemm_big_lds_bytes<U, TRANS_B>();
  static const int bpc = [] {
    if (lds > 64 * 1024)
      (void)hipFuncSetAttribute(reinterpret_cast<const void*>(rowgemm_big_kernel<U, TRANS_B>), hipFuncAttributeMaxDynamicSharedMemorySize, (int)lds);
    int n = 0;
    if (hipOccupancyMaxActiveBlocksPerMultiprocessor(&n, reinterpret_cast<const void*>(rowgemm_big_kernel<U, TRANS_B>), 256, lds) != hipSuccess || n < 1) n = 1;
    return n;
  }();
  const unsigned npanels = (unsigned)ceil_div64(g.rows, 32);
  const unsigned ny = (unsigned)((g.N + 127) / 128);
  const unsigned heavy = (unsigned)(g.N / 128 + ((g.N % 128) > 32 ? 1 : 0));
  unsigned grid = (unsigned)device_cu_count() * (unsigned)bpc / (heavy ? heavy : 1u);
  if (grid > npanels) grid = npanels;
  if (grid == 0) grid = 1;
  if (ny > 1) {
    const unsigned per = (npanels + grid - 1) / grid;
    grid = (npanels + per - 1) / per;
  }
  TSGNN_KNAME("rowgemm_big_kernel<%d,%s>", U, TRANS_B ? "true" : "false");
  rowgemm_big_kernel<U, TRANS_B><<<dim3(grid, ny), 256, lds, s>>>(g, npanels);
}

template <bool TRANS_B>
bool try_big(const RowGemmArgs& g, hipStream_t s) {
  const bool wide = g.N > 128;
  const int64_t mn = wide ? rowgemm_big_wide_min_rows() : rowgemm_big_min_rows();
  if (mn <= 0 || g.rows < mn || g.N > 384 || g.K > 128 || (TRANS_B && (g.K % 4)) || (g.N % 4)) return false;
  if (g.N > 128 && (g.normalize || g.fill_rows > 0 || g.rinv)) return false;
  if (g.K <= 96) launch_big<12, TRANS_B>(g, s);
  else launch_big<16, TRANS_B>(g, s);
  return true;
}

template <bool TRANS_B>
bool try_colsplit(const RowGemmArgs& g, hipStream_t s) {
  const unsigned nblk = (unsigned)ceil_div64(g.rows, 32);
  if (g.normalize || g.fill_rows > 0 || g.N <= 128 || (g.N % 4) || nblk == 0 || nblk > colsplit_max_panels() ||
      !rowgemm_colsplit_enabled())
    return false;
  const size_t lds = rowgemm_lds_bytes<4, TRANS_B, false>();
  TSGNN_KNAME("rowgemm_colsplit_kernel<4,%s>", TRANS_B ? "true" : "false");
  rowgemm_colsplit_kernel<4, TRANS_B><<<dim3(nblk, (unsigned)((g.N + 127) / 128)), 256, lds, s>>>(g);
  return true;
}

template <int NT, bool TRANS_B, bool GATHER>
void launch_rowgemm(const RowGemmArgs& g, hipStream_t s) {
  const unsigned nblk = (unsigned)(ceil_div64(g.rows, 32) + (g.fill_rows > 0 ? 1 : 0));
  if constexpr (GATHER && NT <= 4) {
    if (g.K > KC && nblk <= ks2_max_blocks() && rowgemm_ks2_enabled()) {
      constexpr size_t lds2 = rowgemm_lds_bytes<NT, TRANS_B, true, 2>();
      static bool attr = false;
      if (!attr && lds2 > 64 * 1024) {
        (void)hipFuncSetAttribute(reinterpret_cast<const void*>(rowgemm_gather_ks2_kernel<NT, TRANS_B>),
                                  hipFuncAttributeMaxDynamicSharedMemorySize, (int)lds2);
        attr = true;
      }
      TSGNN_KNAME("rowgemm_gather_ks2_kernel<%d,%s>", NT, TRANS_B ? "true" : "false");
      rowgemm_gather_ks2_kernel<NT, TRANS_B><<<nblk, 512, lds2, s>>>(g);
      return;
    }
  }
  const size_t lds = rowgemm_lds_bytes<NT, TRANS_B, GATHER>();
  TSGNN_KNAME("rowgemm_kernel<%d,%s,%s>", NT, TRANS_B ? "true" : "false", GATHER ? "true" : "false");
  rowgemm_kernel<NT, TRANS_B, GATHER><<<nblk, 256, lds, s>>>(g);
}

template <bool TRANS_B, bool GATHER>
void dispatch_rowgemm(const RowGemmArgs& g, hipStream_t s) {
  switch ((g.N + 31) / 32) {
    case 1: launch_rowgemm<1, TRANS_B, GATHER>(g, s); break;
    case 2: launch_rowgemm<2, TRANS_B, GATHER>(g, s); break;
    case 3: launch_rowgemm<3, TRANS_B, GATHER>(g, s); break;
    case 4: launch_rowgemm<4, TRANS_B, GATHER>(g, s); break;
    default:
      if constexpr (!GATHER) {
        switch ((g.N + 31) / 32) {
          case 5: launch_rowgemm<5, TRANS_B, false>(g, s); break;
          case 6: launch_rowgemm<6, TRANS_B, false>(g, s); break;
          case 7: launch_rowgemm<7, TRANS_B, false>(g, s); break;
          default: launch_rowgemm<8, TRANS_B, false>(g, s); break;
        }
      }
      break;
  }
}

}

extern "C" {

int tsgnn_rowgemm_supported(const float* a, int64_t lda, const float* b, int64_t ldb, const float* c, int64_t ldc, int K, int N,
                            int trans_b) {
  const bool al = ((reinterpret_cast<uintptr_t>(a) | reinterpret_cast<uintptr_t>(b)) & 15) == 0;
  if (!al || (lda % 4) || (ldb % 4) || N > 384 || N <= 0 || K <= 0) return 0;
  if (lda < ((K + 3) / 4) * 4) return 0;
  if (!trans_b && (N % 4)) return 0;
  if (trans_b && (K % 4)) return 0;
  (void)c; (void)ldc;
  return 1;
}

int tsgnn_rowgemm_f32(const float* a, int64_t lda, const float* b, int64_t ldb, int trans_b, const float* bias, float* c,
                      int64_t ldc, float* rinv, int64_t rows, int K, int N, int normalize, int64_t fill_rows,
                      tsgnn_stream_t stream) {
  if (!a || !b || !c || rows < 0 || fill_rows < 0 || K <= 0 || N <= 0 || lda < K || ldc < N) return TSGNN_EINVAL;
  if (!tsgnn_rowgemm_supported(a, lda, b, ldb, c, ldc, K, N, trans_b)) return TSGNN_EUNSUPPORTED;
  if (fill_rows > 0 && ((N % 4) || (ldc % 4) || (reinterpret_cast<uintptr_t>(c) & 15) ||
                        (bias && (reinterpret_cast<uintptr_t>(bias) & 15))))
    return TSGNN_EUNSUPPORTED;
  if (rows == 0 && fill_rows == 0) return TSGNN_OK;
  RowGemmArgs g{a, lda, b, ldb, bias, c, ldc, rinv, rows, K, N, normalize, fill_rows, nullptr, 0, nullptr, 0};
  if (trans_b) {
    if (!try_big<true>(g, stream) && !try_colsplit<true>(g, stream)) {
      if (N > 256) return TSGNN_EUNSUPPORTED;
      dispatch_rowgemm<true, false>(g, stream);
    }
  } else {
    if (!try_big<false>(g, stream) && !try_colsplit<false>(g, stream)) {
      if (N > 256) return TSGNN_EUNSUPPORTED;
      dispatch_rowgemm<false, false>(g, stream);
    }
  }
  TSGNN_CHECK_LAUNCH();
  return TSGNN_OK;
}

int tsgnn_gather_rowgemm_st_f32(const int* ell, int ell_w, const int* tail_ptr, const int* tail_col, const float* x, int64_t ldx, const float* b, int64_t ldb, const float* bias,
                                float* c, int64_t ldc, float* rinv, float* zout, int64_t ldz, int64_t rows, int K, int N,
                                int64_t fill_rows, const int* row_slot, unsigned long long* sums, float* ghost, int panel_units,
                                const int64_t* pack_desc, tsgnn_stream_t stream) {
  if (!ell || !x || !b || !c || !row_slot || !sums || !ghost || rows <= 0 || fill_rows < 0 || K <= 0 || N <= 0 || ldx < K || ldc < N)
    return TSGNN_EINVAL;
  const bool sched = ell_w == TSGNN_SCHED_8x32 || ell_w == TSGNN_SCHED_16x24;
  if (sched && (tail_ptr || tail_col)) return TSGNN_EINVAL;
  if (!sched && ell_w != 4 && ell_w != 8 && ell_w != 16) return TSGNN_EUNSUPPORTED;
  if (!tsgnn_rowgemm_supported(x, ldx, b, ldb, c, ldc, K, N, 0) || N > 128 || N <= 96 || K > 128 || (reinterpret_cast<uintptr_t>(ell) & 15) ||
      (reinterpret_cast<uintptr_t>(sums) & 15))
    return TSGNN_EUNSUPPORTED;
  if (zout && ((ldz % 4) || ldz < K || (reinterpret_cast<uintptr_t>(zout) & 15))) return TSGNN_EUNSUPPORTED;
  if ((N % 4) || (ldc % 4) || (reinterpret_cast<uintptr_t>(c) & 15) || (bias && (reinterpret_cast<uintptr_t>(bias) & 15))) return TSGNN_EUNSUPPORTED;
  PackRider pk{};
  if (pack_desc) {
    if (reinterpret_cast<uintptr_t>(pack_desc) & 7) return TSGNN_EINVAL;
    const int nsets = (int)pack_desc[0];
    if (nsets <= 0 || nsets > PACK_RIDER_SETS) return TSGNN_EINVAL;
    for (int t = 0; t < nsets; ++t) {
      const int rc = pack_set_from_desc(pack_desc + 1 + 6 * t, pk.s[t]);
      if (rc != TSGNN_OK) return rc;
    }
    pk.blocks = (unsigned)nsets;
  }
  if ((tail_ptr == nullptr) != (tail_col == nullptr)) return TSGNN_EINVAL;
  RowGemmArgs g{x, ldx, b, ldb, bias, c, ldc, rinv, rows, K, N, 1, fill_rows, ell, ell_w, zout, ldz, tail_ptr, tail_col};
  g.st_row_slot = row_slot; g.st_sums = sums; g.st_ghost = ghost;
  unsigned nblk = (unsigned)(ceil_div64(rows, 32) + (fill_rows > 0 ? 1 : 0));
  const bool ks2 = K > KC && nblk <= ks2_max_blocks() && rowgemm_ks2_enabled();
  if (!ks2)
    nblk = panel_split(rows, device_cu_count(), panel_units, &g.n_full, &g.unit) + (fill_rows > 0 ? 1u : 0u);
  if (sched && ell_w != (ks2 ? TSGNN_SCHED_16x24 : (g.unit == 8 || g.unit == 16) ? 0 : TSGNN_SCHED_8x32)) return TSGNN_EUNSUPPORTED;
  if (ks2) {
    constexpr size_t lds2 = rowgemm_lds_bytes<4, false, true, 2>();
    static bool attr = false;
    if (!attr && lds2 > 64 * 1024) {
      (void)hipFuncSetAttribute(reinterpret_cast<const void*>(rowgemm_gather_ks2_st_kernel<0>), hipFuncAttributeMaxDynamicSharedMemorySize, (int)lds2);
      (void)hipFuncSetAttribute(reinterpret_cast<const void*>(rowgemm_gather_ks2_st_kernel<TSGNN_SCHED_16x24>), hipFuncAttributeMaxDynamicSharedMemorySize, (int)lds2);
      attr = true;
    }
    const PullRider pr = take_pull_rider(512);
    pk.blocks *= PACK_SET_ENTRIES / 512;
    TSGNN_KNAME("rowgemm_gather_ks2_st_kernel");
    if (sched) rowgemm_gather_ks2_st_kernel<TSGNN_SCHED_16x24><<<nblk + pk.blocks + pr.blocks, 512, lds2, stream>>>(g, pr, nblk, pk);
    else rowgemm_gather_ks2_st_kernel<0><<<nblk + pk.blocks + pr.blocks, 512, lds2, stream>>>(g, pr, nblk, pk);
  } else {
    const PullRider pr = take_pull_rider(256);
    pk.blocks *= PACK_SET_ENTRIES / 256;
    TSGNN_KNAME("rowgemm_gather_st_kernel<%s>", (g.unit == 8 || g.unit == 16) ? "true" : "false");
    if (g.unit == 8 || g.unit == 16) rowgemm_gather_st_kernel<true><<<nblk + pk.blocks + pr.blocks, 256, rowgemm_lds_bytes<4, false, true>(), stream>>>(g, pr, nblk, pk);
    else if (sched) rowgemm_gather_st_kernel<false, TSGNN_SCHED_8x32><<<nblk + pk.blocks + pr.blocks, 256, rowgemm_lds_bytes<4, false, true>(), stream>>>(g, pr, nblk, pk);
    else rowgemm_gather_st_kernel<false><<<nblk + pk.blocks + pr.blocks, 256, rowgemm_lds_bytes<4, false, true>(), stream>>>(g, pr, nblk, pk);
  }
  TSGNN_CHECK_LAUNCH();
  return TSGNN_OK;
}

int tsgnn_panel_blocks(int64_t rows, int panel_units) {
  if (rows <= 0) return 0;
  int nf = 0, un = 16;
  return (int)panel_split(rows, device_cu_count(), panel_units, &nf, &un);
}

int tsgnn_gather_sched_slots(int64_t rows, int64_t fill_rows, int K, int panel_units, int layer0) {
  if (rows <= 0) return 0;
  if (layer0) {
    const unsigned nblk = (unsigned)(ceil_div64(rows, 32) + (fill_rows > 0 ? 1 : 0));
    if (K > KC && nblk <= ks2_max_blocks() && rowgemm_ks2_enabled()) return TSGNN_SCHED_16x24;
  }
  int nf = 0, un = 32;
  (void)panel_split(rows, device_cu_count(), panel_units, &nf, &un);
  return nf > 0 ? 0 : TSGNN_SCHED_8x32;
}

int tsgnn_gather_rowgemm_f32(const int* ell, int ell_w, const int* tail_ptr, const int* tail_col, const float* x, int64_t ldx, const float* b, int64_t ldb, int trans_b,
                             const float* bias, float* c, int64_t ldc, float* rinv, float* zout, int64_t ldz, int64_t rows, int K,
                             int N, int normalize, int64_t fill_rows, tsgnn_stream_t stream) {
  if (!ell || !x || !b || !c || rows < 0 || fill_rows < 0 || K <= 0 || N <= 0 || ldx < K || ldc < N) return TSGNN_EINVAL;
  if (ell_w != 4 && ell_w != 8 && ell_w != 16) return TSGNN_EUNSUPPORTED;
  if (!tsgnn_rowgemm_supported(x, ldx, b, ldb, c, ldc, K, N, trans_b) || N > 128 || K > 128 || (reinterpret_cast<uintptr_t>(ell) & 15))
    return TSGNN_EUNSUPPORTED;
  if (zout && ((ldz % 4) || ldz < K || (reinterpret_cast<uintptr_t>(zout) & 15))) return TSGNN_EUNSUPPORTED;
  if (fill_rows > 0 && ((N % 4) || (ldc % 4) || (reinterpret_cast<uintptr_t>(c) & 15) ||
                        (bias && (reinterpret_cast<uintptr_t>(bias) & 15))))
    return TSGNN_EUNSUPPORTED;
  if (rows == 0 && fill_rows == 0) return TSGNN_OK;
  if ((tail_ptr == nullptr) != (tail_col == nullptr)) return TSGNN_EINVAL;
  RowGemmArgs g{x, ldx, b, ldb, bias, c, ldc, rinv, rows, K, N, normalize, fill_rows, ell, ell_w, zout, ldz, tail_ptr, tail_col};
  if (trans_b) dispatch_rowgemm<true, true>(g, stream);
  else dispatch_rowgemm<false, true>(g, stream);
  TSGNN_CHECK_LAUNCH();
  return TSGNN_OK;
}

}
```

two-stage-gnn_amd/csrc/rowgemm_body.h:

```cpp
#pragma once
#include "common.h"
#include <type_traits>
#include <cstdlib>

namespace {


typedef float f32x16 __attribute__((ext_vector_type(16)));
constexpr int KC = 32;
constexpr int LDA_S = KC + 4;
constexpr float NORM_EPS = 1e-12f;

struct RowGemmArgs {
  const float* a; int64_t lda;
  const float* b; int64_t ldb;
  const float* bias;
  float* c; int64_t ldc;
  float* rinv;
  int64_t rows; int K; int N;
  int normalize;
  int64_t fill_rows;
  const int* ell; int ell_w;
  float* zout; int64_t ldz;
  const int* tail_ptr; const int* tail_col;
  unsigned long long* ro_packed;
  const int* ro_graph_ptr; const int* ro_row_graph;
  int ro_B, ro_nslots, ro_nghost;
  const int* st_row_slot; unsigned long long* st_sums; float* st_ghost;
  const unsigned long long* bn_sums; const float* bn_ghost; const int* bn_slot_count; int bn_B, bn_nslots, bn_F;
  int n_full;
  int unit;
  const float4* b_img;
};

inline int panel_unit_rows(int64_t rows, int ncu) {
  static const int forced = [] { const char* e = getenv("TSGNN_PANEL_UNIT"); const int v = e ? atoi(e) : 0; return (v == 8 || v == 16) ? v : 0; }();
  if (forced) return forced;
  return ((rows + 31) / 32 - ncu) <= ncu / 16 ? 8 : 16;
}
inline unsigned panel_split(int64_t rows, int ncu, int panel_units, int* n_full, int* unit) {
  const int64_t P = (rows + 31) / 32;
  *n_full = 0; *unit = 32;
  if (!panel_units || ncu < 8) return (unsigned)P;
  if (P <= ncu || P - ncu > ncu / 2) return (unsigned)P;
  const int nf = ncu & ~7;
  *n_full = nf;
  const int u = *unit = panel_unit_rows(rows, ncu);
  return (unsigned)nf + (unsigned)((rows - 32 * (int64_t)nf + u - 1) / u);
}

constexpr int BN_TAB = 1024;
constexpr float BN_FWD_EPS = 1e-5f;
constexpr double BN_FIX = 1099511627776.0;

__device__ __forceinline__ unsigned long long rg_pack_max(float val, unsigned r) {
  return ((unsigned long long)f32_ordered(val) << 32) | (unsigned long long)(0xFFFFFFFFu - r);
}

__device__ __forceinline__ float4 ldg4(const float* p) { return *reinterpret_cast<const float4*>(p); }

#ifndef TSGNN_EXP_DROP_NB16
#define TSGNN_EXP_DROP_NB16 0
#endif
constexpr int GN = 8;
constexpr int LDA_F = 128;

template <int NT, bool TRANS_B, bool GATHER, int KS = 1, bool READOUT = false, bool BNIN = false, bool STATS = false, bool UNITS = false,
          bool BIMG = false, int SCHED = 0>
__device__ __forceinline__ void rowgemm_body(const RowGemmArgs& g, float* smem_all, unsigned bid) {
  static_assert(KS == 1 || (KS == 2 && GATHER && NT <= 4), "the split-K variant is built for the gather kernel, widths <= 128");
  static_assert(!READOUT || (NT <= 4 && KS == 1), "the readout epilogue is built for one column tile per wave");
  static_assert(!BNIN || (GATHER && KS == 1), "batch-norm on the fly lives in the gather prologue of the one-group kernel");
  static_assert(!STATS || NT <= 4, "the statistics epilogue is built for one column tile per wave");
  static_assert(!BIMG || (GATHER && KS == 1 && NT == 4), "the image variant is built for the one-group gather kernel at K = N = 128");
  static_assert(SCHED == 0 || (GATHER && !UNITS && SCHED == (KS == 2 ? 24 : 32)), "gather schedules: 8 x 32 (one group) / 16 x 24 (two groups), plain panels");
  constexpr int NP = 32 * NT;
  constexpr int TPW = (NT + 3) / 4;
  constexpr int BV = NT;
  constexpr int A_FLOATS = GATHER ? 0 : 32 * LDA_S;
  constexpr int B_FLOATS = TRANS_B ? NP * LDA_S : KC * NP;
  constexpr int STAGE = A_FLOATS + B_FLOATS;
  const int tid_all = threadIdx.x;
  const int grp = KS == 2 ? (tid_all >> 8) : 0;
  const int tid = KS == 2 ? (tid_all & 255) : tid_all, lane = tid & 63, wid = tid >> 6;
  const int i = lane & 31, h = lane >> 5;
  const int Kc = KS == 1 ? g.K : ((g.K + 2 * KC - 1) / (2 * KC)) * KC;
  const int kb = grp * Kc;
  const int Kv = KS == 1 ? g.K : min(g.K - kb, Kc);
  constexpr int GRP = BIMG ? 256 : (KS == 2 && 2 * STAGE < 4096 + 256) ? 4096 + 256 : 2 * STAGE;
  float* smem = smem_all + grp * GRP;
  float* Apanel = smem_all + KS * GRP + (KS == 2 ? 0 : 256);
  float* scratch = KS == 2 ? smem_all + GRP + 4096 : smem_all + GRP;
  const unsigned npanels = (unsigned)((g.rows + 31) / 32);
  int64_t m0, rows_hi;
  if constexpr (UNITS) {
    const int un = g.unit == 8 ? 8 : 16;
    const unsigned nfull = (unsigned)g.n_full, nhalf = (unsigned)((g.rows - 32 * (int64_t)nfull + un - 1) / un);
    if (bid < nfull) { m0 = (int64_t)xcd_remap(bid, nfull) * 32; rows_hi = m0 + 32; }
    else if (bid < nfull + nhalf) { m0 = 32 * (int64_t)nfull + un * (int64_t)xcd_remap(bid - nfull, nhalf); rows_hi = min(m0 + un, g.rows); }
    else { m0 = (int64_t)npanels * 32; rows_hi = m0; }
  } else {
    m0 = (bid < npanels ? (int64_t)xcd_remap(bid, npanels) : (int64_t)bid) * 32;
    rows_hi = g.rows;
  }
  TR(0);
  if (m0 >= g.rows) {
    if (KS == 2 && grp == 1) return;
    float* fred = smem_all;
    const int N4 = g.N / 4, rpp = 256 / N4;
    const int c4 = tid % N4, rsub = tid / N4;
    float4 bv = make_float4(0.f, 0.f, 0.f, 0.f);
    if (g.bias && rsub < rpp) bv = ldg4(g.bias + 4 * c4);
    float ss = rsub == 0 ? (bv.x * bv.x + bv.y * bv.y) + (bv.z * bv.z + bv.w * bv.w) : 0.f;
    ss = wave_sum(ss);
    if (lane == 0) fred[wid] = ss;
    __syncthreads();
    float sc = 1.f;
    if (g.normalize) sc = fminf(__builtin_amdgcn_rsqf((fred[0] + fred[1]) + (fred[2] + fred[3])), 1.0f / NORM_EPS);
    const float4 out = make_float4(bv.x * sc, bv.y * sc, bv.z * sc, bv.w * sc);
    if constexpr (STATS) {
      if (g.st_ghost && wid == 0) {
        const float a = fmaxf(out.x, 0.f), b = fmaxf(out.y, 0.f), c = fmaxf(out.z, 0.f), d = fmaxf(out.w, 0.f);
        float g1 = rsub == 0 ? (a + b) + (c + d) : 0.f, g2 = rsub == 0 ? (a * a + b * b) + (c * c + d * d) : 0.f;
        g1 = wave_sum(g1); g2 = wave_sum(g2);
        if (lane == 0) { g.st_ghost[0] = g1; g.st_ghost[1] = g2; }
      }
    }
    if (rsub < rpp) {
      for (int64_t r = rsub; r < g.fill_rows; r += rpp) {
        *reinterpret_cast<float4*>(g.c + (g.rows + r) * g.ldc + 4 * c4) = out;
        if (g.rinv && c4 == 0) g.rinv[g.rows + r] = sc;
      }
      if constexpr (READOUT) {
        if (g.ro_packed && g.ro_nghost) {
          for (int b = rsub; b < g.ro_B; b += rpp) {
            const int sz = g.ro_graph_ptr[b + 1] - g.ro_graph_ptr[b];
            if (sz < g.ro_nslots && sz < g.fill_rows) {
              const unsigned row = (unsigned)(g.rows + sz);
              unsigned long long* dst = g.ro_packed + (int64_t)b * g.N + 4 * c4;
              atomicMax(dst + 0, rg_pack_max(out.x, row)); atomicMax(dst + 1, rg_pack_max(out.y, row));
              atomicMax(dst + 2, rg_pack_max(out.z, row)); atomicMax(dst + 3, rg_pack_max(out.w, row));
            }
          }
        }
      }
    }
    return;
  }
  int ro_gf = 0, ro_gl = 0;
  if constexpr (READOUT) {
    if (g.ro_packed) {
      ro_gf = g.ro_row_graph[m0];
      ro_gl = g.ro_row_graph[min(m0 + 31, rows_hi - 1)];
    }
  }

  const int am = tid >> 3, ak4 = tid & 7;
  const bool a_row_ok = (m0 + am) < rows_hi;
  const float* ap = g.a + ((a_row_ok && !GATHER) ? (m0 + am) : 0) * g.lda + 4 * ak4 + (GATHER ? 0 : kb);
  const float* bp[BV];
  int b_k[BV];
  int b_lds[BV];
  bool b_nok[BV];
#pragma unroll
  for (int q = 0; q < BV; ++q) {
    const int idx = q * 256 + tid;
    if (!TRANS_B) {
      const int k = idx / (NP / 4), n4 = idx % (NP / 4);
      b_nok[q] = 4 * n4 < g.N;
      bp[q] = g.b + (int64_t)(k + kb) * g.ldb + (b_nok[q] ? 4 * n4 : 0);
      b_k[q] = k;
      b_lds[q] = k * NP + 4 * n4;
    } else {
      const int n = idx / (KC / 4), k4 = idx % (KC / 4);
      b_nok[q] = n < g.N;
      bp[q] = g.b + (int64_t)(b_nok[q] ? n : 0) * g.ldb + 4 * k4 + kb;
      b_k[q] = 4 * k4;
      b_lds[q] = n * LDA_S + 4 * k4;
    }
  }
  struct Staged {
    float4 ra;
    float4 rb[BV];
    int a_valid;
    unsigned b_valid;
    bool plain;
  };
  const bool panel_full = (m0 + 32) <= rows_hi && g.N == NP;
  auto fetch = [&](Staged& s, int k0) {
    s.plain = panel_full && (k0 + KC) <= Kv;
    s.a_valid = 0;
    s.b_valid = 0;
    if (GATHER) {
#pragma unroll
      for (int q = 0; q < BV; ++q) {
        const bool kok = (k0 + b_k[q]) < Kv;
        if (!TRANS_B) s.rb[q] = ldg4(kok ? bp[q] + (int64_t)k0 * g.ldb : bp[q] - (int64_t)b_k[q] * g.ldb);
        else s.rb[q] = ldg4(kok ? bp[q] + k0 : bp[q] - b_k[q]);
        s.b_valid |= (kok && b_nok[q]) ? (1u << q) : 0u;
      }
      s.plain = false;
      return;
    }
    if (s.plain) {
      s.ra = ldg4(ap + k0);
#pragma unroll
      for (int q = 0; q < BV; ++q) s.rb[q] = ldg4(TRANS_B ? bp[q] + k0 : bp[q] + (int64_t)k0 * g.ldb);
      return;
    }
    const int gk = k0 + 4 * ak4;
    const bool ok = a_row_ok && gk < Kv;
    s.a_valid = ok ? min(4, Kv - gk) : 0;
    s.ra = ldg4(gk < Kv ? ap + k0 : ap - 4 * ak4);
#pragma unroll
    for (int q = 0; q < BV; ++q) {
      const bool kok = (k0 + b_k[q]) < Kv;
      if (!TRANS_B) s.rb[q] = ldg4(kok ? bp[q] + (int64_t)k0 * g.ldb : bp[q] - (int64_t)b_k[q] * g.ldb);
      else s.rb[q] = ldg4(kok ? bp[q] + k0 : bp[q] - b_k[q]);
      s.b_valid |= (kok && b_nok[q]) ? (1u << q) : 0u;
    }
  };
  auto commit = [&](const Staged& s, float* st) {
    if (GATHER) {
#pragma unroll
      for (int q = 0; q < BV; ++q)
        *reinterpret_cast<float4*>(st + A_FLOATS + b_lds[q]) = ((s.b_valid >> q) & 1u) ? s.rb[q] : make_float4(0.f, 0.f, 0.f, 0.f);
      return;
    }
    if (s.plain) {
      *reinterpret_cast<float4*>(st + am * LDA_S + 4 * ak4) = s.ra;
#pragma unroll
      for (int q = 0; q < BV; ++q) *reinterpret_cast<float4*>(st + A_FLOATS + b_lds[q]) = s.rb[q];
      return;
    }
    float4 va = s.ra;
    if (s.a_valid < 4) va.w = 0.f;
    if (s.a_valid < 3) va.z = 0.f;
    if (s.a_valid < 2) va.y = 0.f;
    if (s.a_valid < 1) va.x = 0.f;
    *reinterpret_cast<float4*>(st + am * LDA_S + 4 * ak4) = va;
#pragma unroll
    for (int q = 0; q < BV; ++q)
      *reinterpret_cast<float4*>(st + A_FLOATS + b_lds[q]) = ((s.b_valid >> q) & 1u) ? s.rb[q] : make_float4(0.f, 0.f, 0.f, 0.f);
  };
  auto frags = [&](const float* st, int k0, float (&af)[KC / 2], float (&bf)[TPW][KC / 2]) {
    const float* As = GATHER ? Apanel : st;
    constexpr int lda_s = GATHER ? LDA_F : LDA_S;
    const int kq = GATHER ? (kb + k0) >> 2 : 0;
    const float* Bs = st + A_FLOATS;
#pragma unroll
    for (int u = 0; u < KC / 8; ++u) {
      const float4 v = GATHER ? *reinterpret_cast<const float4*>(As + i * lda_s + 4 * ((kq + 2 * u + h) ^ (i & 7)))
                              : *reinterpret_cast<const float4*>(As + i * lda_s + 8 * u + 4 * h);
      af[4 * u] = v.x; af[4 * u + 1] = v.y; af[4 * u + 2] = v.z; af[4 * u + 3] = v.w;
    }
    if constexpr (BIMG) return;
#pragma unroll
    for (int t = 0; t < TPW; ++t) {
      const int tile = wid + 4 * t;
      if (4 * (t + 1) <= NT || tile < NT) {
#pragma unroll
        for (int u = 0; u < KC / 8; ++u) {
          if (!TRANS_B) {
#pragma unroll
            for (int c = 0; c < 4; ++c) bf[t][4 * u + c] = Bs[(8 * u + 4 * h + c) * NP + tile * 32 + i];
          } else {
            const float4 v = *reinterpret_cast<const float4*>(Bs + (tile * 32 + i) * LDA_S + 8 * u + 4 * h);
            bf[t][4 * u] = v.x; bf[t][4 * u + 1] = v.y; bf[t][4 * u + 2] = v.z; bf[t][4 * u + 3] = v.w;
          }
        }
      } else {
#pragma unroll
        for (int j = 0; j < KC / 2; ++j) bf[t][j] = 0.f;
      }
    }
  };

  f32x16 acc[TPW];
#pragma unroll
  for (int t = 0; t < TPW; ++t)
#pragma unroll
    for (int r = 0; r < 16; ++r) acc[t][r] = 0.f;

  constexpr int NS = (NT <= 4 && !GATHER) ? 4 : 2;
  Staged st[NS];
  constexpr int NPASS = 4 / KS;
  int ids[NPASS][GN];
  constexpr int NSL = SCHED ? SCHED : 1;
  int sid[NSL];
  int s_first = 0;
  unsigned s_end = 0u, s_short = 0u;
  if constexpr (SCHED != 0) {
    const int4* rec = reinterpret_cast<const int4*>(g.ell) + ((m0 >> 5) * (8 * KS) + (tid_all >> 5)) * ((4 + SCHED) / 4);
    const int4 hd = rec[0];
    s_first = hd.x; s_end = (unsigned)hd.z; s_short = (unsigned)hd.w;
#pragma unroll
    for (int q = 0; q < SCHED / 4; ++q) {
      const int4 v = rec[1 + q];
      sid[4 * q] = v.x; sid[4 * q + 1] = v.y; sid[4 * q + 2] = v.z; sid[4 * q + 3] = v.w;
    }
  } else if (GATHER) {
    const int rsub = tid_all >> 5;
#pragma unroll
    for (int p = 0; p < NPASS; ++p) {
      const int64_t row = m0 + 8 * KS * p + rsub;
#pragma unroll
      for (int q = 0; q < GN / 4; ++q) {
        int4 v = make_int4(-1, -1, -1, -1);
        if (row < rows_hi && 4 * q < g.ell_w) v = *reinterpret_cast<const int4*>(g.ell + row * g.ell_w + 4 * q);
        ids[p][4 * q] = v.x; ids[p][4 * q + 1] = v.y; ids[p][4 * q + 2] = v.z; ids[p][4 * q + 3] = v.w;
      }
    }
  }
  constexpr int BN_PT = BN_TAB / 256;
  float2* bn_tab = reinterpret_cast<float2*>(Apanel + 32 * LDA_F);
  ulonglong2 bn_s[BNIN ? BN_PT : 1];
  int bn_have[BNIN ? BN_PT : 1];
  float bn_g1 = 0.f, bn_g2 = 0.f;
  if constexpr (BNIN) {
#pragma unroll
    for (int q = 0; q < BN_PT; ++q) {
      const int n = min(tid_all + 256 * q, g.bn_nslots - 1);
      bn_s[q] = *reinterpret_cast<const ulonglong2*>(g.bn_sums + 2 * n);
      bn_have[q] = g.bn_slot_count[n];
    }
    bn_g1 = g.bn_ghost[0]; bn_g2 = g.bn_ghost[1];
  }
  int st_slot = -1;
  if constexpr (STATS) {
    if (g.st_sums && wid == 0 && grp == 0 && lane < 32 && (m0 + lane) < rows_hi) st_slot = g.st_row_slot[m0 + lane];
  }
  if constexpr (!BIMG) {
#pragma unroll
    for (int c = 0; c < NS; ++c)
      if (c == 0 || c * KC < Kc) fetch(st[c], c * KC);
  }
  float bq[BIMG ? 4 * KC / 2 : 1];
  auto img_fetch = [&](int u0) {
    const float4* img = g.b_img + (wid * 16 + u0) * 64 + lane;
#pragma unroll
    for (int u = 0; u < 8; ++u) {
      const float4 v = img[u * 64];
      bq[4 * (u0 + u)] = v.x; bq[4 * (u0 + u) + 1] = v.y; bq[4 * (u0 + u) + 2] = v.z; bq[4 * (u0 + u) + 3] = v.w;
    }
  };
  if (GATHER) {
    const int c4 = tid_all & 31, rsub = tid_all >> 5;
    const bool colok = 4 * c4 < g.K;
    if constexpr (BNIN) {
      const double inv_cnt = 1.0 / ((double)g.bn_B * (double)g.bn_F);
#pragma unroll
      for (int q = 0; q < BN_PT; ++q) {
        const int n = tid_all + 256 * q;
        if (n < g.bn_nslots) {
          const float2 ms = bn_stats_from_sums(bn_s[q].x, bn_s[q].y, bn_have[q], bn_g1, bn_g2, g.bn_B, inv_cnt, BN_FWD_EPS);
          bn_tab[n] = make_float2(ms.y, ms.x * ms.y);
        }
      }
    }
    if constexpr (SCHED != 0) {
      float4 sv[NSL];
#pragma unroll
      for (int s = 0; s < SCHED; ++s) {
        sv[s] = make_float4(0.f, 0.f, 0.f, 0.f);
        if (colok && sid[s] >= 0) sv[s] = ldg4(g.a + (int64_t)(BNIN ? (sid[s] & 0xFFFFF) : sid[s]) * g.lda + 4 * c4);
      }
      if constexpr (BIMG) {
        __builtin_amdgcn_sched_barrier(0);
        img_fetch(0);
        __builtin_amdgcn_sched_barrier(0);
      }
      if constexpr (BNIN) {
        __syncthreads();
#pragma unroll
        for (int s = 0; s < SCHED; ++s) {
          if (sid[s] >= 0) {
            const float2 rm = bn_tab[sid[s] >> 20];
            float4& t = sv[s];
            t.x = fmaf(fmaxf(t.x, 0.f), rm.x, -rm.y); t.y = fmaf(fmaxf(t.y, 0.f), rm.x, -rm.y);
            t.z = fmaf(fmaxf(t.z, 0.f), rm.x, -rm.y); t.w = fmaf(fmaxf(t.w, 0.f), rm.x, -rm.y);
          }
        }
      }
      const unsigned e_any = (unsigned)__builtin_amdgcn_readlane((int)s_end, 0) | (unsigned)__builtin_amdgcn_readlane((int)s_end, 32);
      const unsigned nshort = ~s_short;
      float z0 = __uint_as_float((nshort & 1u) << 31);
      float4 va = make_float4(z0, z0, z0, z0);
      float* ap = Apanel + s_first * LDA_F;
      int pr = s_first;
      const bool zok = g.zout != nullptr && colok;
      int64_t zoff = (m0 + s_first) * g.ldz + 4 * c4;
      int zleft = zok ? (int)min(rows_hi - (m0 + s_first), (int64_t)32) : 0;
#pragma unroll
      for (int s = 0; s < SCHED; ++s) {
        va.x += sv[s].x; va.y += sv[s].y; va.z += sv[s].z; va.w += sv[s].w;
        if ((e_any >> s) & 1u) {
          if ((s_end >> s) & 1u) {
            *reinterpret_cast<float4*>(ap + 4 * (c4 ^ (pr & 7))) = va;
            if (zleft > 0) st_out(reinterpret_cast<float4*>(g.zout + zoff), va);
            ++pr; ap += LDA_F; zoff += g.ldz; --zleft;
            if (s + 1 < SCHED) {
              z0 = __uint_as_float(((nshort >> (s + 1)) & 1u) << 31);
              va = make_float4(z0, z0, z0, z0);
            }
          }
        }
      }
      if constexpr (BIMG) {
        __builtin_amdgcn_sched_barrier(0);
        img_fetch(8);
        __builtin_amdgcn_sched_barrier(0);
      }
    } else {
    float4 nbv[NPASS][GN];
#pragma unroll
    for (int p = 0; p < NPASS; ++p)
#pragma unroll
      for (int k = 0; k < GN; ++k) {
        nbv[p][k] = make_float4(0.f, 0.f, 0.f, 0.f);
        if (colok && ids[p][k] >= 0) nbv[p][k] = ldg4(g.a + (int64_t)(BNIN ? (ids[p][k] & 0xFFFFF) : ids[p][k]) * g.lda + 4 * c4);
      }
    if constexpr (BIMG) {
      __builtin_amdgcn_sched_barrier(0);
      img_fetch(0);
      __builtin_amdgcn_sched_barrier(0);
    }
    if constexpr (BNIN) {
      __syncthreads();
#pragma unroll
      for (int p = 0; p < NPASS; ++p)
#pragma unroll
        for (int k = 0; k < GN; ++k) {
          if (ids[p][k] >= 0) {
            const float2 rm = bn_tab[ids[p][k] >> 20];
            float4& t = nbv[p][k];
            t.x = fmaf(fmaxf(t.x, 0.f), rm.x, -rm.y); t.y = fmaf(fmaxf(t.y, 0.f), rm.x, -rm.y);
            t.z = fmaf(fmaxf(t.z, 0.f), rm.x, -rm.y); t.w = fmaf(fmaxf(t.w, 0.f), rm.x, -rm.y);
          }
        }
    }
#pragma unroll
    for (int p = 0; p < NPASS; ++p) {
      const int64_t row = m0 + 8 * KS * p + rsub;
      float4 va = nbv[p][0];
#pragma unroll
      for (int k = 1; k < GN; ++k) { va.x += nbv[p][k].x; va.y += nbv[p][k].y; va.z += nbv[p][k].z; va.w += nbv[p][k].w; }
      bool table_full = g.ell_w <= GN && ids[p][GN - 1] >= 0;
      if (!TSGNN_EXP_DROP_NB16 && colok && g.ell_w > GN && ids[p][GN - 1] >= 0) {
        static_assert(GN == 8, "the second half of a 16-wide table");
        const int4 e0 = *reinterpret_cast<const int4*>(g.ell + row * g.ell_w + 8), e1 = *reinterpret_cast<const int4*>(g.ell + row * g.ell_w + 12);
        const int js[8] = {e0.x, e0.y, e0.z, e0.w, e1.x, e1.y, e1.z, e1.w};
        table_full = js[7] >= 0;
        float4 t[8];
#pragma unroll
        for (int k = 0; k < 8; ++k) t[k] = ldg4(g.a + (int64_t)(js[k] >= 0 ? (BNIN ? (js[k] & 0xFFFFF) : js[k]) : 0) * g.lda + 4 * c4);
#pragma unroll
        for (int k = 0; k < 8; ++k) {
          if (js[k] >= 0) {
            if constexpr (BNIN) {
              const float2 rm = bn_tab[js[k] >> 20];
              t[k].x = fmaf(fmaxf(t[k].x, 0.f), rm.x, -rm.y); t[k].y = fmaf(fmaxf(t[k].y, 0.f), rm.x, -rm.y);
              t[k].z = fmaf(fmaxf(t[k].z, 0.f), rm.x, -rm.y); t[k].w = fmaf(fmaxf(t[k].w, 0.f), rm.x, -rm.y);
            }
            va.x += t[k].x; va.y += t[k].y; va.z += t[k].z; va.w += t[k].w;
          }
        }
      }
      if (colok && g.tail_ptr && row < rows_hi && table_full) {
        for (int e = g.tail_ptr[row]; e < g.tail_ptr[row + 1]; ++e) {
          const int j = g.tail_col[e];
          float4 t = ldg4(g.a + (int64_t)(BNIN ? (j & 0xFFFFF) : j) * g.lda + 4 * c4);
          if constexpr (BNIN) {
            const float2 rm = bn_tab[j >> 20];
            t.x = fmaf(fmaxf(t.x, 0.f), rm.x, -rm.y); t.y = fmaf(fmaxf(t.y, 0.f), rm.x, -rm.y);
            t.z = fmaf(fmaxf(t.z, 0.f), rm.x, -rm.y); t.w = fmaf(fmaxf(t.w, 0.f), rm.x, -rm.y);
          }
          va.x += t.x; va.y += t.y; va.z += t.z; va.w += t.w;
        }
      }
      {
        const int pr = 8 * KS * p + rsub;
        *reinterpret_cast<float4*>(Apanel + pr * LDA_F + 4 * (c4 ^ (pr & 7))) = va;
      }
      if (g.zout && colok && row < rows_hi) st_out(reinterpret_cast<float4*>(g.zout + row * g.ldz + 4 * c4), va);
    }
    if constexpr (BIMG) {
      __builtin_amdgcn_sched_barrier(0);
      img_fetch(8);
      __builtin_amdgcn_sched_barrier(0);
    }
    }
  }
  float bias_v[TPW];
#pragma unroll
  for (int t = 0; t < TPW; ++t) {
    const int cn = (wid + 4 * t) * 32 + i;
    bias_v[t] = (g.bias && (wid + 4 * t) < NT && cn < g.N) ? g.bias[cn] : 0.f;
  }
  TR(1);
  if constexpr (!BIMG) {
    commit(st[0], smem);
    if (KC < Kc) commit(st[1], smem + STAGE);
  }
  __syncthreads();
  TR(2);
  float fa[2][KC / 2], fb[2][TPW][KC / 2];
  frags(smem, 0, fa[0], fb[0]);
  if constexpr (BIMG) {
#pragma unroll
    for (int c = 0; c < 4; ++c) {
      if (c < 3) frags(smem, (c + 1) * KC, fa[(c + 1) & 1], fb[0]);
      __builtin_amdgcn_sched_barrier(0);
#pragma unroll
      for (int j = 0; j < KC / 2; ++j) acc[0] = __builtin_amdgcn_mfma_f32_32x32x2f32(fa[c & 1][j], bq[16 * c + j], acc[0], 0, 0, 0);
      __builtin_amdgcn_sched_barrier(0);
      TR(3 + 2 * c);
      TR(4 + 2 * c);
    }
  }
  if (NS == 2 && !BIMG) {
    if (2 * KC < Kc) fetch(st[0], 2 * KC);
    if (3 * KC < Kc) fetch(st[1], 3 * KC);
  }
  auto body = [&](auto ci_, int c) {
    constexpr int CI = decltype(ci_)::value;
    constexpr int P = CI & 1;
    const int k0 = c * KC;
    if (k0 + KC < Kc) frags(smem + (P ^ 1) * STAGE, k0 + KC, fa[P ^ 1], fb[P ^ 1]);
    if (NS == 4 && c >= 0 && k0 + 4 * KC < Kc) fetch(st[CI % NS], k0 + 4 * KC);
    __builtin_amdgcn_sched_barrier(0);
#pragma unroll
    for (int j = 0; j < 8; ++j) acc[0] = __builtin_amdgcn_mfma_f32_32x32x2f32(fa[P][j], fb[P][0][j], acc[0], 0, 0, 0);
    __builtin_amdgcn_sched_barrier(0);
    if (k0 + 2 * KC < Kc) commit(st[(CI + 2) % NS], smem + P * STAGE);
    if (NS == 2 && k0 + 4 * KC < Kc) fetch(st[CI % NS], k0 + 4 * KC);
    __builtin_amdgcn_sched_barrier(0);
#pragma unroll
    for (int j = 8; j < KC / 2; ++j) acc[0] = __builtin_amdgcn_mfma_f32_32x32x2f32(fa[P][j], fb[P][0][j], acc[0], 0, 0, 0);
#pragma unroll
    for (int t = 1; t < TPW; ++t) {
      if (4 * (t + 1) <= NT || (wid + 4 * t) < NT) {
#pragma unroll
        for (int j = 0; j < KC / 2; ++j) acc[t] = __builtin_amdgcn_mfma_f32_32x32x2f32(fa[P][j], fb[P][t][j], acc[t], 0, 0, 0);
      }
    }
    TR(3 + 2 * min(c, 3));
    if (Kc > 2 * KC) __syncthreads();
    TR(4 + 2 * min(c, 3));
  };
  for (int c = 0; !BIMG && c * KC < Kc; c += 4) {
    body(std::integral_constant<int, 0>{}, c);
    if ((c + 1) * KC < Kc) body(std::integral_constant<int, 1>{}, c + 1);
    if ((c + 2) * KC < Kc) body(std::integral_constant<int, 2>{}, c + 2);
    if ((c + 3) * KC < Kc) body(std::integral_constant<int, 3>{}, c + 3);
  }
  if (KS == 2) {
    float* xch = smem_all + GRP;
    if (grp == 1) {
#pragma unroll
      for (int r = 0; r < 16; ++r) xch[(wid * 16 + r) * 64 + lane] = acc[0][r];
    }
    __syncthreads();
    TR(7);
    if (grp == 1) { TR_END(); return; }
#pragma unroll
    for (int r = 0; r < 16; ++r) acc[0][r] += xch[(wid * 16 + r) * 64 + lane];
    TR(8);
  }

  float scale[16];
#pragma unroll
  for (int r = 0; r < 16; ++r) scale[r] = 1.f;
  if (g.bias || g.normalize) {
    float ss[16];
    float q1[STATS ? 16 : 1], q2[STATS ? 16 : 1];
#pragma unroll
    for (int r = 0; r < 16; ++r) ss[r] = 0.f;
#pragma unroll
    for (int t = 0; t < TPW; ++t) {
      const int tile = wid + 4 * t;
      const int cn = tile * 32 + i;
      const bool okc = tile < NT && cn < g.N;
      const float bv = bias_v[t];
#pragma unroll
      for (int r = 0; r < 16; ++r) {
        const float v = okc ? acc[t][r] + bv : 0.f;
        acc[t][r] = v;
        ss[r] = fmaf(v, v, ss[r]);
        if constexpr (STATS) { const float rl = fmaxf(v, 0.f); q1[r] = rl; q2[r] = rl * rl; }
      }
    }
    if (g.normalize) {
      float* red = scratch;
      float* inv = red + 128 + wid * 32;
      float* redq = smem_all;
      if constexpr (STATS) { if (Kc <= 2 * KC) __syncthreads(); }
      float tot = row16_sum_transpose(ss);
      tot += __shfl_xor(tot, 16, 64);
      float t1 = 0.f, t2 = 0.f;
      if constexpr (STATS) {
        t1 = row16_sum_transpose(q1); t2 = row16_sum_transpose(q2);
        t1 += __shfl_xor(t1, 16, 64); t2 += __shfl_xor(t2, 16, 64);
      }
      TR(11);
      if ((lane & 16) == 0) {
        const int r = lane & 15, row = (r & 3) + 8 * (r >> 2) + 4 * h;
        red[row * 4 + wid] = tot;
        if constexpr (STATS) { redq[row * 4 + wid] = t1; redq[128 + row * 4 + wid] = t2; }
      }
      __syncthreads();
      TR(12);
      if (lane < 32) {
        const float4 p = *reinterpret_cast<const float4*>(red + lane * 4);
        const float rs = fminf(__builtin_amdgcn_rsqf((p.x + p.y) + (p.z + p.w)), 1.0f / NORM_EPS);
        inv[lane] = rs;
        if (g.rinv && wid == 0 && (m0 + lane) < rows_hi) g.rinv[m0 + lane] = rs;
        if constexpr (STATS) {
          if (g.st_sums && wid == 0 && st_slot >= 0) {
            const float4 a = *reinterpret_cast<const float4*>(redq + lane * 4), b = *reinterpret_cast<const float4*>(redq + 128 + lane * 4);
            const float s1 = ((a.x + a.y) + (a.z + a.w)) * rs, s2 = ((b.x + b.y) + (b.z + b.w)) * (rs * rs);
            atomicAdd(g.st_sums + 2 * st_slot, (unsigned long long)__double2ll_rn((double)s1 * BN_FIX));
            atomicAdd(g.st_sums + 2 * st_slot + 1, (unsigned long long)__double2ll_rn((double)s2 * BN_FIX));
          }
        }
      }
      __syncthreads();
#pragma unroll
      for (int q = 0; q < 4; ++q) {
        const float4 v = *reinterpret_cast<const float4*>(inv + 8 * q + 4 * h);
        scale[4 * q] = v.x; scale[4 * q + 1] = v.y; scale[4 * q + 2] = v.z; scale[4 * q + 3] = v.w;
      }
    }
  }
  const bool full = panel_full;
#pragma unroll
  for (int t = 0; t < TPW; ++t) {
    const int tile = wid + 4 * t;
    if (tile < NT) {
      const int cn = tile * 32 + i;
      float* cp = g.c + (m0 + 4 * h) * g.ldc + cn;
      if (full) {
#pragma unroll
        for (int r = 0; r < 16; ++r) st_out(cp + (int64_t)((r & 3) + 8 * (r >> 2)) * g.ldc, acc[t][r] * scale[r]);
      } else {
#pragma unroll
        for (int r = 0; r < 16; ++r) {
          const int64_t gm = m0 + (r & 3) + 8 * (r >> 2) + 4 * h;
          if (gm < rows_hi && cn < g.N) cp[(int64_t)((r & 3) + 8 * (r >> 2)) * g.ldc] = acc[t][r] * scale[r];
        }
      }
    }
  }
  if constexpr (READOUT) {
    if (g.ro_packed) {
      const int cn = wid * 32 + i;
      const int64_t last = min(m0 + 31, rows_hi - 1);
      for (int b = ro_gf; b <= ro_gl; ++b) {
        int64_t lo = m0, hi = last + 1;
        if (ro_gf != ro_gl) { lo = max(lo, (int64_t)g.ro_graph_ptr[b]); hi = min(hi, (int64_t)g.ro_graph_ptr[b + 1]); }
        unsigned long long best = 0ull;
#pragma unroll
        for (int r = 0; r < 16; ++r) {
          const int64_t gm = m0 + (r & 3) + 8 * (r >> 2) + 4 * h;
          if (gm >= lo && gm < hi) {
            const unsigned long long p = rg_pack_max(acc[0][r] * scale[r], (unsigned)gm);
            best = p > best ? p : best;
          }
        }
        const unsigned olo = __shfl_xor((unsigned)(best & 0xFFFFFFFFull), 32, 64), ohi = __shfl_xor((unsigned)(best >> 32), 32, 64);
        const unsigned long long other = ((unsigned long long)ohi << 32) | olo;
        best = other > best ? other : best;
        if (h == 0 && best && cn < g.N) atomicMax(&g.ro_packed[(int64_t)b * g.N + cn], best);
      }
    }
  }
  TR(13);
  TR_END();
}


template <int NT, bool TRANS_B, bool GATHER, int KS = 1, bool BNIN = false, bool BIMG = false>
constexpr size_t rowgemm_lds_bytes() {
  constexpr int NP = 32 * NT;
  constexpr int STAGE2 = BIMG ? 256 : 2 * ((GATHER ? 0 : 32 * LDA_S) + (TRANS_B ? NP * LDA_S : KC * NP));
  constexpr int GRP = (KS == 2 && STAGE2 < 4096 + 256) ? 4096 + 256 : STAGE2;
  return sizeof(float) * (KS * GRP + (KS == 2 ? 0 : 128 + 4 * 32) + (GATHER ? 32 * LDA_F : 0) + (BNIN ? 2 * BN_TAB : 0));
}

}
```

two-stage-gnn_amd/graph.py:

```python
import numpy as np
import torch

from . import _native as nat


def _i32(n, device):
    return torch.empty(int(n), dtype=torch.int32, device=device)


def _scan_ws(n, device):
    need = np.zeros(1, dtype=np.int64)
    nat.call_nostream("scan_workspace_ints", int(n), need.ctypes.data)
    return _i32(need[0], device)


def exclusive_scan(counts):
    n = counts.numel()
    out = _i32(n + 1, counts.device)
    nat.call("exclusive_scan_i32", counts, n, out, _scan_ws(n, counts.device))
    return out


SCHED_SHAPES = ((8, 32), (16, 24))
SCHED_HEADER = 4
# ... 190 lines not shown
    @classmethod
    def structure_only(cls, sizes, nmax, device, ghosts=True):
        g = cls()
        g.layout = "packed" if ghosts else "padded"
        g._set_sizes(sizes, nmax, device, ghosts=ghosts)
        g.rowptr = torch.zeros(g.total_rows + 1, dtype=torch.int32, device=device)
        g.col = _i32(1, device)
        g.symmetric = True
        return g

    @classmethod
    def from_csr(cls, rowptr, col, val, sizes, nmax, assume_symmetric=True):
        g = cls()
        g._set_sizes(sizes, nmax, rowptr.device)
        if rowptr.numel() != g.total_rows + 1:
            raise ValueError("rowptr must have n_rows + nmax + 1 entries (empty ghost rows included)")
        g.rowptr, g.col, g.val = rowptr, col, val
        g.nnz = int(col.numel())
        g.symmetric = bool(assume_symmetric)
        return g

    def row_slabs(self, rows_per_slab=64):
        cache = getattr(self, "_slabs", None)
        if cache is None or cache[3] != rows_per_slab:
            starts, seg = [], [0]
            off = 0
            for n in self.sizes:
                n = int(n)
                starts.extend(range(off, off + n, rows_per_slab))
                seg.append(len(starts))
                off += n
            srp = np.asarray(starts + [off], dtype=np.int32)
            cache = self._slabs = (torch.from_numpy(srp).to(self.device),
                                   torch.from_numpy(np.asarray(seg, dtype=np.int32)).to(self.device), len(starts), rows_per_slab)
        return cache[0], cache[1], cache[2]

    def ell(self):
        if self.val is not None:
            return None
        if getattr(self, "_ell", None) is None:
            R = self.total_rows
            deg = self.rowptr[1:] - self.rowptr[:-1]
            maxdeg = int(deg.max().item()) if R > 0 else 0
            W = 4 if maxdeg <= 4 else (8 if maxdeg <= 8 else 16)
            ell = _i32(max(R * W, 1), self.device)
            tail_cnt = torch.zeros(R, dtype=torch.int32, device=self.device) if maxdeg > W else None
            nat.call("csr_to_ell", self.rowptr, self.col, R, W, ell, tail_cnt)
            tail = None
            if tail_cnt is not None:
                tail_ptr = exclusive_scan(tail_cnt)
                tail_col = _i32(max(int(tail_ptr[-1].item()), 1), self.device)
                nat.call("csr_tail_fill", self.rowptr, self.col, tail_ptr, R, W, tail_col)
                tail = (tail_ptr, tail_col)
            self._ell = (ell, W, tail)
        return self._ell

    def ell_slots(self):
        if getattr(self, "_ell_slots", None) is None:
            e = self.ell()
            if e is None or self.total_rows >= (1 << 20) or self.nmax > 1024 or self.row_slot is None:
                self._ell_slots = False
            else:
                ell, W, tail = e
                slot_of = self.row_slot.to(torch.int64)

                def pack(ids32, n):
                    ids = ids32[:n].to(torch.int64)
                    ok = (ids >= 0) & (ids < self.n_rows)
                    packed = torch.where(ok, (slot_of[ids.clamp(0, max(self.n_rows - 1, 0))] << 20) | ids, torch.full_like(ids, -1))
                    out = _i32(max(ids32.numel(), 1), self.device)
                    out[:n] = packed.to(torch.int32)
                    return out
                table = pack(ell, self.total_rows * W)
                tcol = pack(tail[1], int(tail[0][-1].item())) if tail is not None else None
                self._ell_slots = (table, tcol)
        return self._ell_slots if self._ell_slots is not False else None

    def gather_schedule(self, shape, slots=False, ncu=None):
        shape = (int(shape[0]), int(shape[1]))
        if ncu is None:
            ncu = torch.cuda.get_device_properties(self.device).multi_processor_count
        cache = self.__dict__.setdefault("_gather_sched", {})
        key = (shape, bool(slots), int(ncu))
        if key not in cache:
            sched = None
            if (self.val is None and self.sizes is not None and getattr(self, "ghost_slots_fixed", None) is None and self.n_rows > 0
                    and not unit_cut(self.n_rows, int(ncu), self.panel_units)
                    and not (slots and (self.total_rows >= (1 << 20) or self.nmax > 1024 or self.row_slot is None))):
                rec = pack_gather_schedule(self.rowptr.cpu().numpy(), self.col.cpu().numpy(), self.n_rows, shape,
                                           self.row_slot.cpu().numpy() if slots else None)
                if rec is not None:
                    sched = torch.from_numpy(rec).to(self.device)
            cache[key] = sched
        return cache[key]

    def du_map(self, other_blocks):
        if self.sizes is None or getattr(self, "ghost_slots_fixed", None) is not None:
            return None, (-1 if self.B <= 64 else 0), 64
        cache = self.__dict__.setdefault("_du_maps", {})
        key = int(other_blocks)
        if key not in cache:
            sizes = np.asarray(self.sizes, dtype=np.int64)
            ncu = torch.cuda.get_device_properties(self.device).multi_processor_count
            chunk = 64
            if key + int(np.maximum(1, -(-sizes // 64)).sum()) > ncu:
                chunk = 128
            if int(sizes.max()) > 255 * chunk or self.B >= (1 << 22):
                cache[key] = (None, 0, 64)
            else:
                ent = [(b << 8) | c for b in range(self.B) for c in range(max(1, -(-int(sizes[b]) // chunk)))]
                cache[key] = (torch.from_numpy(np.asarray(ent, dtype=np.int32)).to(self.device), len(ent), chunk)
        return cache[key]

    def readout_map(self, nslots, fill_rows):
        if self.sizes is None:
            return None, 0
        key = (int(nslots), int(fill_rows))
        cache = self.__dict__.setdefault("_ro_maps", {})
        if key not in cache:
            ch = np.zeros(1, dtype=np.int32)
            ng = np.zeros(1, dtype=np.int32)
            nf = np.zeros(1, dtype=np.int32)
            nat.call_nostream("sage_layer_fwd_bn_plan", int(self.n_rows), int(fill_rows), int(self.B), int(nslots), int(self.panel_units),
                              ch.ctypes.data, ng.ctypes.data, nf.ctypes.data)
            ch, ng, nf = int(ch[0]), int(ng[0]), int(nf[0])
            chunks = -(-int(nslots) // ch)
            npan = nf or -(-self.n_rows // 32)
            q, r = divmod(npan, 8)
            start = np.zeros(9, dtype=np.int64)
            for x in range(8):
                start[x + 1] = start[x] + (q + 1 if x < r else q)
            gp = np.concatenate([[0], np.cumsum(np.asarray(self.sizes, dtype=np.int64))])
            mid_panel = ((gp[:-1] + gp[1:]) // 2) // 32
            xcd_of_graph = np.clip(np.searchsorted(start, mid_panel, side="right") - 1, 0, 7)
            want = [[] for _ in range(8)]
            for b in range(self.B):
                for c in range(chunks):
                    want[int(xcd_of_graph[b])].append(b * chunks + c)
            items = self.B * chunks
            slots = [[k for k in range(items) if (ng + k) % 8 == x] for x in range(8)]
            ro = np.full(items, -1, dtype=np.int32)
            left = []
            for x in range(8):
                n = min(len(want[x]), len(slots[x]))
                ro[slots[x][:n]] = want[x][:n]
                left += want[x][n:]
                slots[x] = slots[x][n:]
            free = [k for x in range(8) for k in slots[x]]
            ro[free] = left
            assert (np.sort(ro) == np.arange(items)).all()
            cache[key] = (torch.from_numpy(ro).to(self.device), ch)
        return cache[key]

    def bn_workspace(self, B, L, Fh, Fl, nslots):
        key = (B, L, Fh, Fl, nslots)
        ws = getattr(self, "_bn_ws", None)
        if ws is None or ws["key"] != key:
            words = (L - 1) * 2 * nslots
            from . import message_passing as mp
            ws = {"key": key, "sums": mp.register_clear_on_error(torch.zeros(max(words, 2), dtype=torch.int64, device=self.device)),
                  "ghost": mp.register_clear_on_error(torch.zeros(max(2 * (L - 1), 2), dtype=torch.float32, device=self.device)),
                  "packed": mp.register_clear_on_error(torch.zeros(B * ((L - 1) * Fh + Fl) + Fl, dtype=torch.int64, device=self.device)),
                  "dirty": False}
            self._bn_ws = ws
        return ws

    def _ensure_transpose(self):
        if self._t is None:
            R1 = self.total_rows
            dev = self.device
            rowptr_t = _i32(R1 + 1, dev)
            col_t = _i32(max(self.nnz, 1), dev)
            val_t = torch.empty(max(self.nnz, 1), dtype=torch.float32, device=dev) if self.val is not None else None
            src_e = _i32(max(self.nnz, 1), dev)
            nat.call("csr_transpose", self.rowptr, self.col, self.val, R1, R1, self.nnz, rowptr_t, col_t, val_t,
                     src_e, _i32(max(R1, 1), dev), _scan_ws(R1, dev))
            self._t = (rowptr_t, col_t, val_t)
            self.src_e_t = src_e
        return self._t

    def transpose_map(self):
        rp, col, _ = self._ensure_transpose()
        return rp, col, self.src_e_t

    def transposed(self, val="graph"):
        if isinstance(val, str):
            val = self.val
        if self.symmetric:
            return self.rowptr, self.col, val
        t = self._ensure_transpose()
        if val is self.val:
            return t
        return t[0], t[1], (val[self.src_e_t.long()] if val is not None else None)

    def new_features(self, feat, zero=False):
        f = torch.zeros if zero else torch.empty
        return f(self.total_rows, feat, dtype=torch.float32, device=self.device)
```

two-stage-gnn_amd/sage_stack.py:

```python
import numpy as np
import torch

from . import _native as nat
from . import message_passing as mp


def eligible(g, convs, bn, x):
    if not bn or g.B > 128 or len(convs) < 2:
        return False
    hid = convs[0].output_dim
    for i, c in enumerate(convs):
        if c.add_self or not c.normalize_embedding or c.dropout > 0.001:
            return False
        if c.output_dim % 4 or c.output_dim > 128:
            return False
        if i < len(convs) - 1 and c.output_dim != hid:
            return False
    return x.dim() == 2 and x.size(1) % 4 == 0 and x.is_cuda and x.stride(0) % 4 == 0


def _aggregate_raw(g, x, transposed=False, rows=None):
    n = g.total_rows if rows is None else rows
    if g.val is None and mp.ell_ok(x) and g.total_rows <= mp.ELL_MAX_ROWS and (not transposed or g.symmetric):
        return mp.spmm_ell(g, x, rows=n)
    rp, col, val = g.transposed() if transposed else (g.rowptr, g.col, g.val)
    return mp.spmm_raw(rp, col, val, x, n)


import os

FUSED_TAIL = os.environ.get("TSGNN_FUSED_TAIL", "1") != "0"
MERGED_FWD = os.environ.get("TSGNN_MERGED_FWD", "1") != "0"
MERGED_BWD = os.environ.get("TSGNN_MERGED_BWD", "1") != "0"
GATHER_MAX_ROWS = int(os.environ.get("TSGNN_GATHER_MAX_ROWS", 65536))
GATHER_FUSED = os.environ.get("TSGNN_GATHER_FUSED", "1") != "0"
EPILOGUE_READOUT = os.environ.get("TSGNN_EPILOGUE_READOUT", "1") != "0"
LAST_LAYER_ROWS = os.environ.get("TSGNN_LAST_LAYER_ROWS", "1") != "0"
RO_MAP = os.environ.get("TSGNN_RO_MAP", "1") != "0"
FUSED_BN = os.environ.get("TSGNN_FUSED_BN", "1") != "0"
SLOT_WGRAD = os.environ.get("TSGNN_SLOT_WGRAD", "0") != "0"
HEAD_DU = os.environ.get("TSGNN_HEAD_DU", "1") != "0"


GATHER_SCHED = os.environ.get("TSGNN_GATHER_SCHED", "1") != "0"
GATHER_SCHED_L0 = os.environ.get("TSGNN_GATHER_SCHED_L0", "1") != "0"
DU_MAP = os.environ.get("TSGNN_DU_MAP", "1") != "0"
SLABS_BESIDE = os.environ.get("TSGNN_SLABS_BESIDE", "1") != "0"
NSLAB_MAX = int(os.environ.get("TSGNN_NSLAB_MAX", "0"))
_ncu = {}


def _cu_count(dev):
    n = _ncu.get(dev)
    if n is None:
        n = _ncu[dev] = torch.cuda.get_device_properties(dev).multi_processor_count
    return n


def _slabs_beside_panels(nslab, rps, need, rows, K, N, dev, panel_units):
    if not SLABS_BESIDE or nslab <= 0:
        return nslab, rps, need
    if NSLAB_MAX and nslab > NSLAB_MAX:
        rps = (-(-rows // NSLAB_MAX) + 7) // 8 * 8
        nslab = -(-rows // rps)
        need = nslab * (K + 1) * N
    ncu = _cu_count(dev)
    npan = int(nat.lib().tsgnn_panel_blocks(int(rows), int(panel_units)))
    if npan <= ncu or 2 * nslab + npan <= 2 * ncu:
        return nslab, rps, need
    cap = max(32, (2 * ncu - npan) // 2)
    rps = -(-rows // cap)
    rps = (rps + 7) // 8 * 8
    nslab = -(-rows // rps)
    return nslab, rps, nslab * (K + 1) * N


def _gather_ok(g, x):
    if not GATHER_FUSED or g.val is not None or not mp.ell_ok(x) or g.total_rows > GATHER_MAX_ROWS:
        return False
    return True


def _gather_sched(g, slots=False, layer0_k=0, fill=0):
    if not GATHER_SCHED:
        return None, 0
    code = int(nat.lib().tsgnn_gather_sched_slots(int(g.n_rows), int(fill), int(layer0_k), int(g.panel_units), 1 if layer0_k else 0))
    if not code:
        return None, 0
    sched = g.gather_schedule((16, 24) if code == 24 else (8, 32), slots=slots)
    return (sched, code) if sched is not None else (None, 0)


def _flush_readout(g, B, sn, sg, pending):
    if pending is not None:
        y, pk = pending
        nat.call("readout_partial_f32", g.graph_ptr, B, sn, g.n_rows, sg, y, y.stride(0), y.size(1), pk)


_PER_GRAPH = [False]

_IMG_FLOATS = 16384
_IMG_LAYERS = 4


class per_graph_stats:
    def __init__(self, on=True):
        self.on = bool(on)

    def __enter__(self):
        self.prev = _PER_GRAPH[0]
        _PER_GRAPH[0] = self.on

    def __exit__(self, *exc):
        _PER_GRAPH[0] = self.prev
        return False


class _SageStack(torch.autograd.Function):

    @staticmethod
    def forward(ctx, x0, g, has_bias, n_head, nodes, *params):
        head = params[len(params) - n_head:] if n_head else None
        params = params[:len(params) - n_head] if n_head else params
        L = len(params) // 2
        Ws = [params[2 * l].contiguous() for l in range(L)]
        bs = [params[2 * l + 1] if has_bias else None for l in range(L)]
        dev = x0.device
        R, B = g.total_rows, g.B
        Fh, Fl = Ws[0].size(1), Ws[-1].size(1)
        total = B * ((L - 1) * Fh + Fl)
        packed = torch.empty(total + Fl, dtype=torch.int64, device=dev) if not nodes else None
        cat = torch.empty(R, (L - 1) * Fh + Fl, dtype=torch.float32, device=dev) if nodes else None
        x = mp._check(x0, R)
        gs = g.n_ghost
        if g.n_ghost > 0 and x.stride(0) % 4 == 0 and all(
                Ws[l].size(1) % 4 == 0 and Ws[l].data_ptr() % 16 == 0 and (bs[l] is None or bs[l].data_ptr() % 16 == 0)
                for l in range(L)):
            fixed = getattr(g, "ghost_slots_fixed", None)
            gs = min(g.nmax, (int(fixed) if fixed is not None else int(g.sizes.max()) + 1))
        if nodes == 1:
            gs = g.n_ghost
        sn, sg = (gs, gs) if g.n_ghost else (g.nmax, 0)
        saved = []
        off = 0
        pending_ro = None
        keep = []
        last_ro_done = False
        bnf = None
        per_graph = ctx.per_graph = bool(_PER_GRAPH[0])
        if per_graph and head is not None:
            raise NotImplementedError("per-graph statistics: the readout and the node-feature form of the stack only")
        if (FUSED_BN and not per_graph and head is not None and not nodes and L >= 2 and g.n_ghost == g.nmax and sn == sg and sn <= 1024
                and Fh == 128 and Fl == 128 and Ws[0].size(0) <= 128 and x.size(1) % 4 == 0 and MERGED_FWD and EPILOGUE_READOUT
                and _gather_ok(g, x) and all(Ws[l].size(0) == 128 and Ws[l].stride(0) % 4 == 0 for l in range(1, L))
                and all(Ws[l].data_ptr() % 16 == 0 and (bs[l] is None or bs[l].data_ptr() % 16 == 0) for l in range(L))
                and mp.rowgemm_ok(x, x.stride(0), Ws[0], Ws[0].stride(0), Ws[0].size(0), Fh, False)
                and head[0].size(0) <= 128 and (L - 1) * Fh + Fl <= 2048 and g.row_graph is not None):
            ell_s = g.ell_slots()
            if ell_s is not None:
                bnf = g.bn_workspace(B, L, Fh, Fl, sn)
                if bnf["dirty"]:
                    bnf["sums"].zero_(); bnf["ghost"].zero_(); bnf["packed"].zero_()
                bnf["dirty"] = True
                packed = bnf["packed"]
        ctx.w_img = ctx.pack_desc = None
        if bnf is not None:
            ell, ell_w, tail = g.ell()
            tp, tc = tail if tail is not None else (None, None)
            ell_s, tc_s = ell_s
            sums, ghost = bnf["sums"], bnf["ghost"]
            ro_map, ro_ch = g.readout_map(sn, gs) if RO_MAP else (None, 0)
            w_img = pack_desc = None
            if 1 <= L - 1 <= _IMG_LAYERS:
                w_img = torch.empty(2 * (L - 1), _IMG_FLOATS, dtype=torch.float32, device=dev)
                pack_desc = np.empty(1 + 12 * (L - 1), dtype=np.int64)
                pack_desc[0] = 2 * (L - 1)
                for l in range(1, L):
                    for kn in (1, 0):
                        t = 2 * (l - 1) + (1 - kn)
                        pack_desc[1 + 6 * t:7 + 6 * t] = (Ws[l].data_ptr(), Ws[l].stride(0), 128, 128, kn, w_img[t].data_ptr())
                bnf["pack_desc"] = pack_desc
            ctx.w_img, ctx.pack_desc = w_img, pack_desc
            sch0, sch0_w = _gather_sched(g, layer0_k=Ws[0].size(0), fill=gs) if GATHER_SCHED_L0 else (None, 0)
            schs, schs_w = _gather_sched(g, slots=True)
            for l in range(L):
                K, N = Ws[l].size(0), Ws[l].size(1)
                v = torch.empty(R, N, dtype=torch.float32, device=dev)
                rinv = torch.empty(R, dtype=torch.float32, device=dev)
                z = torch.empty(R, x.size(1) if l == 0 else Fh, dtype=torch.float32, device=dev)
                s_out = sums[l * 2 * sn:(l + 1) * 2 * sn] if l < L - 1 else None
                g_out = ghost[2 * l:2 * l + 2] if l < L - 1 else None
                if l == 0:
                    e_, w_, tp_, tc_ = (sch0, sch0_w, None, None) if sch0 is not None else (ell, ell_w, tp, tc)
                    nat.call("gather_rowgemm_st_f32", e_, w_, tp_, tc_, x, x.stride(0), Ws[0], Ws[0].stride(0), bs[0], v, v.stride(0), rinv, z,
                             z.stride(0), g.n_rows, K, N, gs, g.row_slot, s_out, g_out, int(g.panel_units),
                             pack_desc.ctypes.data if pack_desc is not None else None)
                    mean = rstd = None
                else:
                    pm, pr_ = saved[l - 1][3], saved[l - 1][4]
                    last = l == L - 1
                    e_, w_, tp_, tc_ = (schs, schs_w, None, None) if schs is not None else (ell_s, ell_w, tp, tc_s)
                    nat.call("sage_layer_fwd_bn_f32", e_, w_, tp_, tc_, saved[l - 1][1], saved[l - 1][1].stride(0), Ws[l], Ws[l].stride(0), bs[l],
                             v, v.stride(0), rinv, z, z.stride(0), g.n_rows, K, gs, g.graph_ptr, g.slot_count, B, sn, sg,
                             packed[(l - 1) * B * Fh:(l - 1) * B * Fh + B * Fh],
                             packed[l * B * Fh:l * B * Fh + (B + 1) * N] if last else None, g.row_graph,
                             sums[(l - 1) * 2 * sn:l * 2 * sn], ghost[2 * (l - 1):2 * l], pm, pr_,
                             None if last else g.row_slot, s_out, g_out, ro_map, ro_ch, int(g.panel_units),
                             w_img[2 * (l - 1)] if w_img is not None else None)
                if l < L - 1:
                    mean = torch.empty(g.nmax, dtype=torch.float32, device=dev)
                    rstd = torch.empty(g.nmax, dtype=torch.float32, device=dev)
                else:
                    mean = rstd = None
                saved.append((z, v, rinv, mean, rstd, True))
            last_ro_done = True
        for l in (range(L) if bnf is None else ()):
            K, N = Ws[l].size(0), Ws[l].size(1)
            if nodes and l == L - 1:
                v = cat[:, (L - 1) * Fh:]
            else:
                v = torch.empty(R, N, dtype=torch.float32, device=dev)
            rinv = torch.empty(R, dtype=torch.float32, device=dev)
            lean = (g.n_ghost > 0 and x.stride(0) % 4 == 0 and N % 4 == 0 and Ws[l].data_ptr() % 16 == 0
                    and (bs[l] is None or bs[l].data_ptr() % 16 == 0))
            fused = lean and N <= 128 and _gather_ok(g, x) and mp.rowgemm_ok(x, x.stride(0), Ws[l], Ws[l].stride(0), K, N, False)
            if (fused and MERGED_FWD and pending_ro is not None and K == 128 and N == 128 and x.size(1) == 128
                    and Ws[l].stride(0) % 4 == 0):
                ell, ell_w, tail = g.ell()
                tp, tc = tail if tail is not None else (None, None)
                z = torch.empty(R, x.size(1), dtype=torch.float32, device=dev)
                if EPILOGUE_READOUT and l == L - 1 and not nodes and l > 0 and (not g.n_ghost or gs > 0):
                    nat.call("sage_layer_fwd_ro_f32", ell, ell_w, tp, tc, x, x.stride(0), Ws[l], Ws[l].stride(0), bs[l], v, v.stride(0),
                             rinv, z, z.stride(0), g.n_rows, K, gs, g.graph_ptr, B, sn, sg, pending_ro[1],
                             packed[off:off + (B + 1) * N], g.row_graph)
                    last_ro_done = True
                else:
                    nat.call("sage_layer_fwd_f32", ell, ell_w, tp, tc, x, x.stride(0), Ws[l], Ws[l].stride(0), bs[l], v, v.stride(0), rinv,
                             z, z.stride(0), g.n_rows, K, gs, g.graph_ptr, B, sn, sg, pending_ro[1])
                pending_ro = None
            elif fused:
                _flush_readout(g, B, sn, sg, pending_ro)
                pending_ro = None
                ell, ell_w, tail = g.ell()
                tp, tc = tail if tail is not None else (None, None)
                z = torch.empty(R, x.size(1), dtype=torch.float32, device=dev)
                nat.call("gather_rowgemm_f32", ell, ell_w, tp, tc, x, x.stride(0), Ws[l], Ws[l].stride(0), 0, bs[l], v, v.stride(0), rinv,
                         z, z.stride(0), g.n_rows, K, N, 1, gs)
            else:
                _flush_readout(g, B, sn, sg, pending_ro)
                pending_ro = None
                z = _aggregate_raw(g, x, rows=g.n_rows if lean else None)
                if lean and mp.rowgemm_ok(z, z.stride(0), Ws[l], Ws[l].stride(0), K, N, False):
                    nat.call("rowgemm_f32", z, z.stride(0), Ws[l], Ws[l].stride(0), 0, bs[l], v, v.stride(0), rinv, g.n_rows, K, N, 1,
                             gs)
                elif mp.rowgemm_ok(z, z.stride(0), Ws[l], Ws[l].stride(0), K, N, False):
                    if lean:
                        z[g.n_rows:].zero_()
                        lean = False
                    nat.call("rowgemm_f32", z, z.stride(0), Ws[l], Ws[l].stride(0), 0, bs[l], v, v.stride(0), rinv, R, K, N, 1, 0)
                else:
                    if lean:
                        z[g.n_rows:].zero_()
                        lean = False
                    nat.call("linear_l2norm_f32", z, z.stride(0), Ws[l], Ws[l].stride(0), bs[l], v, v.stride(0), rinv, R, K, N, 1)
            pk = packed[off:off + B * N] if not nodes else None
            if l < L - 1 and per_graph:
                mean = torch.empty(R, dtype=torch.float32, device=dev)
                rstd = torch.empty(R, dtype=torch.float32, device=dev)
                y = torch.empty_like(v) if not nodes else cat[:, l * Fh:(l + 1) * Fh]
                if l == 0 and not nodes:
                    packed[:total].zero_()
                nat.call("row_ln_fwd_f32", v, v.stride(0), g.n_rows + sg, N, 1, mean, rstd, y, y.stride(0))
                if not nodes:
                    pending_ro = (y, pk)
                keep.append(y)
                x = y
            elif l < L - 1:
                mean = torch.empty(g.nmax, dtype=torch.float32, device=dev)
                rstd = torch.empty(g.nmax, dtype=torch.float32, device=dev)
                y = torch.empty_like(v) if not nodes else cat[:, l * Fh:(l + 1) * Fh]
                nat.call("slot_bn_fwd_f32", g.graph_ptr, g.slot_count, B, sn, g.n_rows, sg, v, v.stride(0), N, 1,
                         mean, rstd, y, y.stride(0), packed if (l == 0 and not nodes) else None, total)
                if not nodes:
                    pending_ro = (y, pk)
                keep.append(y)
                x = y
            else:
                mean = rstd = None
                if head is None and not nodes and not last_ro_done:
                    nat.call("readout_partial_f32", g.graph_ptr, B, sn, g.n_rows, sg, v, v.stride(0), N, pk)
            saved.append((z, v, rinv, mean, rstd, lean))
            off += B * N
        ctx.nodes = nodes
        if nodes:
            if nodes == 2 and g.n_ghost:
                nat.defer_zero(cat[g.n_rows:])
            ctx.g, ctx.L, ctx.has_bias, ctx.dims = g, L, has_bias, (Fh, Fl)
            ctx.slots = (sn, sg)
            ctx.Ws, ctx.saved, ctx.arg = Ws, saved, None
            ctx.params = params
            ctx.head = None
            return cat
        out = torch.empty(B, (L - 1) * Fh + Fl, dtype=torch.float32, device=dev)
        arg = torch.empty(total, dtype=torch.int32, device=dev)
        ctx.g, ctx.L, ctx.has_bias, ctx.dims = g, L, has_bias, (Fh, Fl)
        ctx.slots = (sn, sg)
        ctx.Ws, ctx.saved, ctx.arg = Ws, saved, arg
        ctx.params = params
        ctx.x0_ld = x.size(1) if L == 0 else x0.size(1)
        ctx.head = None
        if head is None:
            nat.call("readout_decode_layers_f32", packed, B, L, Fh, Fl, out, out.stride(0), arg)
            return out
        w1, b1, w2, b2 = head
        w1c, w2c = w1.contiguous(), w2.contiguous()
        E, C = w1c.size(0), w2c.size(0)
        vec = torch.empty(B, E, dtype=torch.float32, device=dev)
        y = torch.empty(B, C, dtype=torch.float32, device=dev)
        v_last = saved[-1][1]
        if bnf is not None:
            nat.call("packed_head_fwd_z_f32", packed, B, L, Fh, Fl, out, out.stride(0), arg, w1c, b1, w2c, b2, E, C, vec, y,
                     bnf["sums"], (L - 1) * 2 * sn)
            bnf["dirty"] = False
        elif last_ro_done and E <= 128 and out.size(1) <= 2048:
            nat.call("packed_head_fwd_f32", packed, B, L, Fh, Fl, out, out.stride(0), arg, w1c, b1, w2c, b2, E, C, vec, y)
        else:
            nat.call("readout_head_fwd_f32", packed, B, L, Fh, Fl, v_last, v_last.stride(0), g.graph_ptr, g.n_rows, sn, sg, out,
                     out.stride(0), arg, w1c, b1, w2c, b2, E, C, vec, y)
        ctx.head = (out, vec, w1c, w2c, head)
        ctx.set_materialize_grads(False)
        return vec, y

    @staticmethod
    def backward(ctx, *gouts):
        g, L = ctx.g, ctx.L
        Fh, Fl = ctx.dims
        R, B = g.total_rows, g.B
        w_img = ctx.w_img
        head_grads = ()
        du_last = None
        if ctx.head is None:
            dout = gouts[0].contiguous()
            dev = dout.device
        else:
            out, vec, w1c, w2c, (pw1, pb1, pw2, pb2) = ctx.head
            dvec, dy = gouts
            dev = out.device
            P, E, C = out.size(1), w1c.size(0), w2c.size(0)
            if dy is None and dvec is None:
                return (None,) * (5 + 2 * L + 4)
            ce = mp.take_deferred_ce(dy) if dy is not None else None
            if ce is None:
                dy = dy.contiguous() if dy is not None else torch.zeros(B, C, device=dev)
            dvec = dvec.contiguous() if dvec is not None else None
            dout = torch.empty(B, P, dtype=torch.float32, device=dev)
            dw1, s1 = mp._sink_or_new(pw1, (E, P), dev)
            dw2, s2 = mp._sink_or_new(pw2, (C, E), dev)
            db1, s3 = mp._sink_or_new(pb1, (E,), dev) if pb1 is not None else (None, False)
            db2, s4 = mp._sink_or_new(pb2, (C,), dev) if pb2 is not None else (None, False)
            parts = mp.head_norm_slots((s1, s2, s3, s4), (pb1 is not None, pb2 is not None), (pw1, pb1, pw2, pb2), E)
            sn_, sg_ = ctx.slots
            v_l, rinv_l, lean_l = ctx.saved[L - 1][1], ctx.saved[L - 1][2], ctx.saved[L - 1][5]
            if (HEAD_DU and LAST_LAYER_ROWS and not ctx.nodes and L > 1 and lean_l and Fl % 4 == 0 and Fl <= 128 and g.n_ghost == g.nmax
                    and sn_ == sg_ and g.n_ghost >= B and ctx.needs_input_grad[5 + 2 * (L - 1)] and v_l.stride(0) % 4 == 0):
                du_l = torch.empty(R, Fl, dtype=torch.float32, device=dev)
                argl = ctx.arg[(L - 1) * B * Fh:(L - 1) * B * Fh + B * Fl]
                dmap, ndmap, dchunk = g.du_map(B + (E + 3) // 4 + 1) if DU_MAP else (None, 0, 64)
                if nat.try_call("head2_bwd_du_map_f32", out, out.stride(0), vec, ce[0] if ce is not None else None,
                                ce[1] if ce is not None else None, ce[2] if ce is not None else None, None if ce is not None else dy, dvec,
                                w1c, w2c, B, P, E, C, dout, dout.stride(0), dw1, db1, dw2, db2, parts, g.graph_ptr, g.n_rows, sg_,
                                sn_, v_l, v_l.stride(0), rinv_l, argl, (L - 1) * Fh, Fl, du_l, du_l.stride(0), dmap, ndmap, dchunk):
                    du_last = du_l
            if du_last is not None:
                pass
            elif ce is not None:
                nat.call("head2_bwd_ce_f32", out, out.stride(0), vec, ce[0], ce[1], ce[2], dvec, w1c, w2c, B, P, E, C, dout,
                         dout.stride(0), dw1, db1, dw2, db2, parts)
            else:
                nat.call("head2_bwd_f32", out, out.stride(0), vec, dy, dvec, w1c, w2c, B, P, E, C, dout, dout.stride(0), dw1, db1, dw2,
                         db2, parts)
            head_grads = (None if s1 else dw1, None if s3 else db1, None if s2 else dw2, None if s4 else db2)
            if mp.GRAD_SINK is not None and s1 and s2 and (s3 or pb1 is None) and (s4 or pb2 is None):
                mp.GRAD_SINK.ready((pw1, pb1, pw2, pb2))
        sn, sg = ctx.slots
        grads = [None] * (2 * L)
        dxs = None
        dx0 = None
        keep = []
        red = mp.WgradSets(mp.wgrad_reduce_multi, max_sets_with_shares=4)
        for l in range(L - 1, -1, -1):
            z, v, rinv, mean, rstd, lean = ctx.saved[l]
            W = ctx.Ws[l]
            K, N = W.size(0), W.size(1)
            last = l == L - 1
            du = du_last if (last and du_last is not None) else torch.empty(R, N, dtype=torch.float32, device=dev)
            bo = sg
            if ctx.nodes:
                dsl = argl = None
                dnode = dout[:, l * Fh:l * Fh + N]
            else:
                dsl = dout[:, l * Fh:l * Fh + N]
                argl = ctx.arg[l * B * Fh:l * B * Fh + B * N]
                dnode = None
            if last and du_last is not None:
                bo = B
            elif (LAST_LAYER_ROWS and last and not ctx.nodes and dxs is None and N % 4 == 0 and N <= 128 and g.n_ghost == g.nmax
                    and sn == sg and dout.stride(0) % 4 == 0 and dsl.data_ptr() % 16 == 0 and g.row_graph is not None):
                nat.call("readout_l2_bwd_f32", g.graph_ptr, g.row_graph, B, g.n_rows, sg, v, v.stride(0), dsl, dout.stride(0), argl, N, rinv,
                         du, du.stride(0))
            elif (SLOT_WGRAD and l == 0 and L > 1 and not ctx.nodes and not ctx.needs_input_grad[0] and lean and B <= 32 and N == 128
                  and K <= 128 and sn == sg and g.n_ghost == g.nmax and ctx.needs_input_grad[5] and z.stride(0) % 4 == 0
                  and z.data_ptr() % 16 == 0 and v.data_ptr() % 16 == 0 and (not ctx.has_bias or ctx.needs_input_grad[6])):
                per = int(os.environ.get("TSGNN_SLOT_WGRAD_PER", "2"))
                nblk = max(1, -(-sn // per))
                ws0 = torch.empty(nblk * (K + 1) * N, dtype=torch.float32, device=dev)
                nat.call("slot_post_wgrad_f32", g.graph_ptr, g.slot_count, B, sn, g.n_rows, sg, v, v.stride(0), dxs,
                         dxs.stride(0) if dxs is not None else 0, dsl, dout.stride(0) if dsl is not None else 0, argl, N, 1, 1, mean, rstd,
                         rinv, z, z.stride(0), K, ws0, nblk)
                dw = red.grad(ctx.params[0], (K, N))
                db = red.grad(ctx.params[1] if ctx.has_bias else None, (N,))
                red.add((ws0, nblk, K, N, dw, db))
                grads[0], grads[1] = red.autograd_grad(dw), red.autograd_grad(db)
                continue
            elif ctx.per_graph and ctx.nodes:
                nat.call("row_post_nodes_bwd_f32", g.n_rows, g.n_rows + sg, v, v.stride(0), dxs, dxs.stride(0) if dxs is not None else 0,
                         dnode, dnode.stride(0), 1 if ctx.nodes == 2 else 0, N, 0 if last else 1, 0 if last else 1, mean, rstd, rinv, du,
                         du.stride(0))
            elif ctx.per_graph:
                nat.call("row_post_bwd_f32", g.row_graph, B, g.n_rows, g.n_rows + sg, v, v.stride(0), dxs,
                         dxs.stride(0) if dxs is not None else 0, dsl, dout.stride(0), argl, N, 0 if last else 1, 0 if last else 1, mean,
                         rstd, rinv, du, du.stride(0))
            else:
                nat.call("slot_post_bwd_f32", g.graph_ptr, g.slot_count, B, sn, g.n_rows, sg, v, v.stride(0), dxs,
                         dxs.stride(0) if dxs is not None else 0, dnode, dnode.stride(0) if dnode is not None else 0, dsl,
                         dout.stride(0) if dsl is not None else 0, argl, N, 0 if last else 1, 0 if last else 1, mean, rstd, rinv, du,
                         du.stride(0))
            want_w = ctx.needs_input_grad[5 + 2 * l]
            want_b = ctx.has_bias and ctx.needs_input_grad[6 + 2 * l]
            merged = False
            if (MERGED_BWD and want_w and lean and l > 0 and K == 128 and N == 128 and g.symmetric and z.size(1) == K
                    and _gather_ok(g, du) and z.data_ptr() % 16 == 0 and du.data_ptr() % 16 == 0 and W.data_ptr() % 16 == 0
                    and W.stride(0) % 4 == 0):
                nslab, rps, need = mp.wgrad_plan(g.n_rows, K, N, z.stride(0), du.stride(0))
                nslab, rps, need = _slabs_beside_panels(nslab, rps, need, g.n_rows, K, N, dev, g.panel_units)
                if 0 < nslab < 512:
                    ell, ell_w, tail = g.ell()
                    tp, tc = tail if tail is not None else (None, None)
                    schb, schb_w = _gather_sched(g)
                    if schb is not None:
                        ell, ell_w, tp, tc = schb, schb_w, None, None
                    ws = torch.empty(need, dtype=torch.float32, device=dev)
                    dxs = torch.empty(R, K, dtype=torch.float32, device=dev)
                    nat.call("sage_layer_bwd_f32", ell, ell_w, tp, tc, du, du.stride(0), W, W.stride(0), dxs, dxs.stride(0), z, z.stride(0),
                             g.n_rows, nslab, rps, bo, ws, int(g.panel_units),
                             w_img[2 * (l - 1) + 1] if w_img is not None else None)
                    dw = red.grad(ctx.params[2 * l], (K, N))
                    db = red.grad(ctx.params[2 * l + 1] if want_b else None, (N,))
                    red.add((ws, nslab, K, N, dw, db))
                    grads[2 * l], grads[2 * l + 1] = red.autograd_grad(dw), red.autograd_grad(db)
                    keep.append(du)
                    merged = True
            if merged:
                continue
            if want_w:
                if not lean and sg < g.n_ghost:
                    du[g.n_rows + sg:].zero_()
                sl = mp.linear_wgrad_slabs(z, K, du[:g.n_rows + bo] if lean else du, bias_only_rows=bo if lean else 0)
                if sl is not None:
                    dw = red.grad(ctx.params[2 * l], (K, N))
                    db = red.grad(ctx.params[2 * l + 1] if want_b else None, (N,))
                    red.add((sl[0], sl[1], K, N, dw, db))
                    dw, db = red.autograd_grad(dw), red.autograd_grad(db)
                else:
# ... 217 lines not shown
```

Baseline: 263,700 graphs/s.

## Add optional per-panel readout table replacing atomicMax, and bound schedule walk

Adds an opt-in path (TSGNN_RO_PANEL, off by default) where the last layer's max-readout writes per-panel partial maxima into a table with plain stores instead of atomicMax on the packed buffer. The head kernel then reduces and clears that table before decoding. This targets atomic contention on the readout, at the cost of extra table memory, extra head work and some LDS. Separately, the SCHED=24, KS=2 gather path now loads and walks only the 8-slot groups that actually contain segment ends, which skips useless loads for short rows but adds branches.

```diff
diff --git a/include/tsgnn.h b/include/tsgnn.h
--- a/include/tsgnn.h
+++ b/include/tsgnn.h
@@ -161,6 +161,7 @@
                                 const float* ghost_in, float* mean_out, float* rstd_out, const int* row_slot,
                                 unsigned long long* sums_out, float* ghost_out, const int* ro_map, int ro_map_ch, int panel_units,
                                 const float* w_img, tsgnn_stream_t stream);
+int tsgnn_ro_panel_arm(unsigned long long* tab, const int* panel_j, int B, int J, int Fl);
 int tsgnn_sage_layer_fwd_bn_plan(int64_t rows, int64_t fill_rows, int B, int nslots, int panel_units, int* ro_ch, int* n_gemm,
                                  int* n_full);
 int tsgnn_sage_layer_fwd_f32(const int* ell, int ell_w, const int* tail_ptr, const int* tail_col, const float* x, int64_t ldx, const float* w, int64_t ldw, const float* bias,
diff --git a/two-stage-gnn_amd/csrc/head.hip b/two-stage-gnn_amd/csrc/head.hip
--- a/two-stage-gnn_amd/csrc/head.hip
+++ b/two-stage-gnn_amd/csrc/head.hip
@@ -2,6 +2,7 @@
 #include "../../include/tsgnn.h"
 #include "readout_body.h"
 #include "ingest_rider.h"
+#include "ro_table.h"
 
 namespace {
 
@@ -152,13 +153,14 @@
   head2_fwd_tail(xs, vs, b, w1, b1, w2, b2, P, E, C, vec, y);
 }
 
-template <int NJ>
+template <int NJ, bool TAB = false>
 __global__ __launch_bounds__(64 * HW) void packed_head_fwd_kernel(const unsigned long long* __restrict__ packed, int B, int L, int Fh,
                                                               int Fl, float* __restrict__ out, int64_t ldo, int* __restrict__ arg,
                                                               const float* __restrict__ w1, const float* __restrict__ b1,
                                                               const float* __restrict__ w2, const float* __restrict__ b2, int P, int E,
                                                               int C, float* __restrict__ vec, float* __restrict__ y, ExpandRider rider,
-                                                              unsigned long long* __restrict__ clear, int64_t clear_n, int clear_packed) {
+                                                              unsigned long long* __restrict__ clear, int64_t clear_n, int clear_packed,
+                                                              unsigned long long* __restrict__ ro_tab, int ro_J) {
   extern __shared__ __attribute__((aligned(16))) float smem[];
   if ((int)blockIdx.x >= B) {
     expand_rider_body(rider, blockIdx.x - (unsigned)B, 64 * HW);
@@ -171,17 +173,30 @@
   const int PH = (L - 1) * Fh, P4 = P >> 2;
   unsigned long long pk[2];
   int64_t pidx[2];
-#pragma unroll
-  for (int u = 0; u < 2; ++u) {
-    const int k = tid + u * 64 * HW;
+  auto pindex = [&](int k) {
     int64_t idx = 0;
     if (k < P) {
       if (k < PH) { const int l = k / Fh, f = k - l * Fh; idx = (int64_t)l * B * Fh + (int64_t)b * Fh + f; }
       else idx = (int64_t)(L - 1) * B * Fh + (int64_t)b * Fl + (k - PH);
     }
+    return idx;
+  };
+#pragma unroll
+  for (int u = 0; u < 2; ++u) {
+    const int k = tid + u * 64 * HW;
+    const int64_t idx = pindex(k);
     pidx[u] = idx;
     pk[u] = packed[idx];
     if (k >= P) pk[u] = 0ull;
+  }
+  constexpr int TQ = TAB ? 5 : 1;
+  static_assert(HW == 16, "the table decode deals 8 threads to each of 128 columns");
+  unsigned long long tb[TQ];
+  const int tcol = tid & 127, tsub = tid >> 7;
+  if constexpr (TAB) {
+    const unsigned long long* tp = ro_tab + (int64_t)b * ro_J * 128 + tcol;
+#pragma unroll
+    for (int q = 0; q < TQ; ++q) { const int j = tsub + 8 * q; tb[q] = tp[(j < ro_J ? j : 0) * 128]; }
   }
   float4 w[NJ][2];
 #pragma unroll
@@ -196,13 +211,35 @@
     if (lane >= P4) w[u][0] = make_float4(0.f, 0.f, 0.f, 0.f);
     if (lane + 64 >= P4) w[u][1] = make_float4(0.f, 0.f, 0.f, 0.f);
   }
-  float bj[NJ];
-#pragma unroll
-  for (int u = 0; u < NJ; ++u) { const int j = wid + HW * u; bj[u] = (b1 && j < E) ? b1[j] : 0.f; }
+  float bj[TAB ? 1 : NJ];
+  if constexpr (TAB) { const int j = wid + HW * (lane < NJ ? lane : 0); bj[0] = (b1 && j < E) ? b1[j] : 0.f; }
+  else {
+#pragma unroll
+    for (int u = 0; u < NJ; ++u) { const int j = wid + HW * u; bj[u] = (b1 && j < E) ? b1[j] : 0.f; }
+  }
   float w2v[4];
 #pragma unroll
   for (int q = 0; q < 4; ++q) { const int j = lane + 64 * q; w2v[q] = (wid < C && j < E) ? w2[(int64_t)wid * E + j] : 0.f; }
   const float b2v = (b2 && wid < C) ? b2[wid] : 0.f;
+  if constexpr (TAB) {
+    unsigned long long* red = reinterpret_cast<unsigned long long*>(smem + ((P + 3) & ~3) + ((E + 3) & ~3));
+    unsigned long long m = 0ull;
+#pragma unroll
+    for (int q = 0; q < TQ; ++q) {
+      const int j = tsub + 8 * q;
+      if (j < ro_J) { m = tb[q] > m ? tb[q] : m; ro_tab[((int64_t)b * ro_J + j) * 128 + tcol] = 0ull; }
+    }
+    red[tsub * 128 + tcol] = m;
+    __syncthreads();
+#pragma unroll
+    for (int u = 0; u < 2; ++u) {
+      const int k = tid + u * 64 * HW;
+      if (k >= PH && k < P) {
+#pragma unroll
+        for (int s = 0; s < 8; ++s) { const unsigned long long o = red[s * 128 + (k - PH)]; pk[u] = o > pk[u] ? o : pk[u]; }
+      }
+    }
+  }
 #pragma unroll
   for (int u = 0; u < 2; ++u) {
     const int k = tid + u * 64 * HW;
@@ -211,8 +248,9 @@
       const float val = p ? ordered_f32((unsigned)(p >> 32)) : 0.f;
       xs[k] = val;
       out[(int64_t)b * ldo + k] = val;
-      arg[pidx[u]] = p ? (int)(0xFFFFFFFFu - (unsigned)(p & 0xFFFFFFFFull)) : -1;
-      if (clear_packed) const_cast<unsigned long long*>(packed)[pidx[u]] = 0ull;
+      const int64_t pi = TAB ? pindex(k) : pidx[u];
+      arg[pi] = p ? (int)(0xFFFFFFFFu - (unsigned)(p & 0xFFFFFFFFull)) : -1;
+      if (clear_packed) const_cast<unsigned long long*>(packed)[pi] = 0ull;
     }
   }
   __syncthreads();
@@ -237,7 +275,8 @@
     for (int u = 0; u < NJ; ++u) {
       const int j = wid + HW * u;
       const float r = wave_sum(acc[u]);
-      if (lane == 0 && j < E) { const float v = r + bj[u]; vs[j] = v; vec[(int64_t)b * E + j] = v; }
+      const float bu = TAB ? __shfl(bj[0], u, 64) : bj[TAB ? 0 : u];
+      if (lane == 0 && j < E) { const float v = r + bu; vs[j] = v; vec[(int64_t)b * E + j] = v; }
     }
   }
   __syncthreads();
@@ -857,7 +896,7 @@
   const ExpandRider rider = take_expand_rider();
   TSGNN_KNAME("packed_head_fwd_kernel<8>");
   packed_head_fwd_kernel<8><<<(unsigned)B + rider.blocks, 64 * HW, lds, stream>>>(packed, B, L, Fh, Fl, out, ldo, arg, w1, b1, w2, b2, P, E, C,
-                                                                               vec, y, rider, nullptr, 0, 0);
+                                                                               vec, y, rider, nullptr, 0, 0, nullptr, 0);
   TSGNN_CHECK_LAUNCH();
   return TSGNN_OK;
 }
@@ -870,11 +909,21 @@
     return TSGNN_EINVAL;
   const int P = (L - 1) * Fh + Fl;
   if ((P % 4) || P > 2048 || E > 8 * HW || ldo < P || (reinterpret_cast<uintptr_t>(w1) & 15)) return TSGNN_EUNSUPPORTED;
-  const size_t lds = sizeof(float) * (size_t)(((P + 3) & ~3) + ((E + 3) & ~3));
+  size_t lds = sizeof(float) * (size_t)(((P + 3) & ~3) + ((E + 3) & ~3));
+  const RoTable rt = take_ro_table();
+  if (rt.tab && (rt.B != B || rt.Fl != Fl || Fl != 128 || rt.J > RO_TABLE_MAX_J || rt.J < 1)) return TSGNN_EUNSUPPORTED;
   const ExpandRider rider = take_expand_rider();
+  if (rt.tab) {
+    lds += sizeof(unsigned long long) * 8 * 128;
+    TSGNN_KNAME("packed_head_fwd_kernel<8,true>");
+    packed_head_fwd_kernel<8, true><<<(unsigned)B + rider.blocks, 64 * HW, lds, stream>>>(packed, B, L, Fh, Fl, out, ldo, arg, w1, b1, w2, b2, P, E, C,
+                                                                                      vec, y, rider, clear, clear_n, 1, rt.tab, rt.J);
+    TSGNN_CHECK_LAUNCH();
+    return TSGNN_OK;
+  }
   TSGNN_KNAME("packed_head_fwd_kernel<8>");
   packed_head_fwd_kernel<8><<<(unsigned)B + rider.blocks, 64 * HW, lds, stream>>>(packed, B, L, Fh, Fl, out, ldo, arg, w1, b1, w2, b2, P, E, C,
-                                                                               vec, y, rider, clear, clear_n, 1);
+                                                                               vec, y, rider, clear, clear_n, 1, nullptr, 0);
   TSGNN_CHECK_LAUNCH();
   return TSGNN_OK;
 }
diff --git a/two-stage-gnn_amd/csrc/layer_fwd.hip b/two-stage-gnn_amd/csrc/layer_fwd.hip
--- a/two-stage-gnn_amd/csrc/layer_fwd.hip
+++ b/two-stage-gnn_amd/csrc/layer_fwd.hip
@@ -3,6 +3,9 @@
 #include "rowgemm_body.h"
 #include "readout_body.h"
 #include "ingest_rider.h"
+#include "ro_table.h"
+
+thread_local RoTable tsgnn_ro_table_ = {nullptr, nullptr, 0, 0, 0};
 
 namespace {
 
@@ -91,6 +94,14 @@
   if (lds < lro) lds = lro;
   const unsigned n_main = n_gemm + ro_gx * (unsigned)B;
   if (sched && ga.n_full > 0) return TSGNN_EUNSUPPORTED;
+  if (packed_out) {
+    const RoTable rt = take_ro_table();
+    if (rt.tab) {
+      if (ga.n_full > 0 || rt.B != B || rt.Fl != 128 || rt.J < (nslots + 31) / 32 + 2 || rt.J > RO_TABLE_MAX_J || !rt.panel_j)
+        return TSGNN_EUNSUPPORTED;
+      ga.ro_tab = rt.tab; ga.ro_panel_j = rt.panel_j; ga.ro_J = rt.J;
+    }
+  }
   const PullRider pr = take_pull_rider();
   const bool units = ga.unit == 8 || ga.unit == 16;
 #define TSGNN_FWD_BN_(RO_, ST_, UN_, IM_, SC_) \
@@ -102,7 +113,7 @@
     else { if (w_img) TSGNN_FWD_BN_(RO_, ST_, false, true, 0); else TSGNN_FWD_BN_(RO_, ST_, false, false, 0); }       \
   } while (0)
   if (packed_out) {
-    TSGNN_KNAME("sage_layer_fwd_bn_kernel<true,false,%s>", units ? "true" : "false");
+    TSGNN_KNAME("sage_layer_fwd_bn_kernel<true,false,%s>%s", units ? "true" : "false", ga.ro_tab ? " ro_tab" : "");
     TSGNN_FWD_BN(true, false);
   } else if (row_slot) {
     TSGNN_KNAME("sage_layer_fwd_bn_kernel<false,true,%s>", units ? "true" : "false");
@@ -114,6 +125,14 @@
 #undef TSGNN_FWD_BN
 #undef TSGNN_FWD_BN_
   TSGNN_CHECK_LAUNCH();
+  return TSGNN_OK;
+}
+
+int tsgnn_ro_panel_arm(unsigned long long* tab, const int* panel_j, int B, int J, int Fl) {
+  if (!tab) { tsgnn_ro_table_.tab = nullptr; return TSGNN_OK; }
+  if (!panel_j || B <= 0 || J < 3 || Fl <= 0) return TSGNN_EINVAL;
+  if (J > RO_TABLE_MAX_J || Fl != 128 || (reinterpret_cast<uintptr_t>(tab) & 15)) return TSGNN_EUNSUPPORTED;
+  tsgnn_ro_table_ = RoTable{tab, panel_j, B, J, Fl};
   return TSGNN_OK;
 }
 
diff --git a/two-stage-gnn_amd/csrc/ro_table.h b/two-stage-gnn_amd/csrc/ro_table.h
--- /dev/null
+++ b/two-stage-gnn_amd/csrc/ro_table.h
@@ -0,0 +1,11 @@
+#pragma once
+#include "common.h"
+
+struct RoTable { unsigned long long* tab; const int* panel_j; int B, J, Fl; };
+extern thread_local RoTable tsgnn_ro_table_;
+constexpr int RO_TABLE_MAX_J = 40;
+static inline RoTable take_ro_table() {
+  const RoTable r = tsgnn_ro_table_;
+  tsgnn_ro_table_.tab = nullptr;
+  return r;
+}
diff --git a/two-stage-gnn_amd/csrc/rowgemm.hip b/two-stage-gnn_amd/csrc/rowgemm.hip
--- a/two-stage-gnn_amd/csrc/rowgemm.hip
+++ b/two-stage-gnn_amd/csrc/rowgemm.hip
@@ -242,6 +242,9 @@
       if (rc != TSGNN_OK) return rc;
     }
     pk.blocks = (unsigned)nsets;
+#ifdef TSGNN_EXP_NO_PACK_RIDERS
+    pk.blocks = 0;
+#endif
   }
   if ((tail_ptr == nullptr) != (tail_col == nullptr)) return TSGNN_EINVAL;
   RowGemmArgs g{x, ldx, b, ldb, bias, c, ldc, rinv, rows, K, N, 1, fill_rows, ell, ell_w, zout, ldz, tail_ptr, tail_col};
diff --git a/two-stage-gnn_amd/csrc/rowgemm_body.h b/two-stage-gnn_amd/csrc/rowgemm_body.h
--- a/two-stage-gnn_amd/csrc/rowgemm_body.h
+++ b/two-stage-gnn_amd/csrc/rowgemm_body.h
@@ -31,6 +31,7 @@
   int n_full;
   int unit;
   const float4* b_img;
+  unsigned long long* ro_tab; const int* ro_panel_j; int ro_J;
 };
 
 inline int panel_unit_rows(int64_t rows, int ncu) {
@@ -61,6 +62,12 @@
 
 #ifndef TSGNN_EXP_DROP_NB16
 #define TSGNN_EXP_DROP_NB16 0
+#endif
+#ifndef TSGNN_EXP_RO_PLAIN_STORE
+#define TSGNN_EXP_RO_PLAIN_STORE 0
+#endif
+#ifndef TSGNN_EXP_WALK_ALL
+#define TSGNN_EXP_WALK_ALL 0
 #endif
 constexpr int GN = 8;
 constexpr int LDA_F = 128;
@@ -137,9 +144,15 @@
             const int sz = g.ro_graph_ptr[b + 1] - g.ro_graph_ptr[b];
             if (sz < g.ro_nslots && sz < g.fill_rows) {
               const unsigned row = (unsigned)(g.rows + sz);
-              unsigned long long* dst = g.ro_packed + (int64_t)b * g.N + 4 * c4;
-              atomicMax(dst + 0, rg_pack_max(out.x, row)); atomicMax(dst + 1, rg_pack_max(out.y, row));
-              atomicMax(dst + 2, rg_pack_max(out.z, row)); atomicMax(dst + 3, rg_pack_max(out.w, row));
+              if (g.ro_tab) {
+                unsigned long long* dst = g.ro_tab + ((int64_t)b * g.ro_J + (g.ro_J - 1)) * g.N + 4 * c4;
+                dst[0] = rg_pack_max(out.x, row); dst[1] = rg_pack_max(out.y, row);
+                dst[2] = rg_pack_max(out.z, row); dst[3] = rg_pack_max(out.w, row);
+              } else {
+                unsigned long long* dst = g.ro_packed + (int64_t)b * g.N + 4 * c4;
+                atomicMax(dst + 0, rg_pack_max(out.x, row)); atomicMax(dst + 1, rg_pack_max(out.y, row));
+                atomicMax(dst + 2, rg_pack_max(out.z, row)); atomicMax(dst + 3, rg_pack_max(out.w, row));
+              }
             }
           }
         }
@@ -148,10 +161,12 @@
     return;
   }
   int ro_gf = 0, ro_gl = 0;
+  int ro_j0 = 0;
   if constexpr (READOUT) {
     if (g.ro_packed) {
       ro_gf = g.ro_row_graph[m0];
       ro_gl = g.ro_row_graph[min(m0 + 31, rows_hi - 1)];
+      if constexpr (!UNITS) { if (g.ro_tab) ro_j0 = g.ro_panel_j[m0 >> 5]; }
     }
   }
 
@@ -359,11 +374,25 @@
       }
     }
     if constexpr (SCHED != 0) {
+      const unsigned e_any = (unsigned)__builtin_amdgcn_readlane((int)s_end, 0) | (unsigned)__builtin_amdgcn_readlane((int)s_end, 32);
+      constexpr bool BOUND = KS == 2 && SCHED == 24 && !TSGNN_EXP_WALK_ALL;
+      const bool more8 = (e_any >> 8) != 0u, more16 = (e_any >> 16) != 0u;
       float4 sv[NSL];
-#pragma unroll
-      for (int s = 0; s < SCHED; ++s) {
-        sv[s] = make_float4(0.f, 0.f, 0.f, 0.f);
-        if (colok && sid[s] >= 0) sv[s] = ldg4(g.a + (int64_t)(BNIN ? (sid[s] & 0xFFFFF) : sid[s]) * g.lda + 4 * c4);
+      auto request = [&](auto lo_, auto hi_) {
+#pragma unroll
+        for (int s = decltype(lo_)::value; s < decltype(hi_)::value; ++s) {
+          sv[s] = make_float4(0.f, 0.f, 0.f, 0.f);
+          if (colok && sid[s] >= 0) sv[s] = ldg4(g.a + (int64_t)(BNIN ? (sid[s] & 0xFFFFF) : sid[s]) * g.lda + 4 * c4);
+        }
+      };
+      using I0 = std::integral_constant<int, 0>; using I8 = std::integral_constant<int, 8>; using I16 = std::integral_constant<int, 16>;
+      using IS = std::integral_constant<int, SCHED>;
+      if constexpr (BOUND) {
+        request(I0{}, I8{});
+        if (more8) request(I8{}, I16{});
+        if (more16) request(I16{}, IS{});
+      } else {
+        request(I0{}, IS{});
       }
       if constexpr (BIMG) {
         __builtin_amdgcn_sched_barrier(0);
@@ -382,7 +411,6 @@
           }
         }
       }
-      const unsigned e_any = (unsigned)__builtin_amdgcn_readlane((int)s_end, 0) | (unsigned)__builtin_amdgcn_readlane((int)s_end, 32);
       const unsigned nshort = ~s_short;
       float z0 = __uint_as_float((nshort & 1u) << 31);
       float4 va = make_float4(z0, z0, z0, z0);
@@ -391,20 +419,29 @@
       const bool zok = g.zout != nullptr && colok;
       int64_t zoff = (m0 + s_first) * g.ldz + 4 * c4;
       int zleft = zok ? (int)min(rows_hi - (m0 + s_first), (int64_t)32) : 0;
-#pragma unroll
-      for (int s = 0; s < SCHED; ++s) {
-        va.x += sv[s].x; va.y += sv[s].y; va.z += sv[s].z; va.w += sv[s].w;
-        if ((e_any >> s) & 1u) {
-          if ((s_end >> s) & 1u) {
-            *reinterpret_cast<float4*>(ap + 4 * (c4 ^ (pr & 7))) = va;
-            if (zleft > 0) st_out(reinterpret_cast<float4*>(g.zout + zoff), va);
-            ++pr; ap += LDA_F; zoff += g.ldz; --zleft;
-            if (s + 1 < SCHED) {
-              z0 = __uint_as_float(((nshort >> (s + 1)) & 1u) << 31);
-              va = make_float4(z0, z0, z0, z0);
+      auto walk = [&](auto lo_, auto hi_) {
+#pragma unroll
+        for (int s = decltype(lo_)::value; s < decltype(hi_)::value; ++s) {
+          va.x += sv[s].x; va.y += sv[s].y; va.z += sv[s].z; va.w += sv[s].w;
+          if ((e_any >> s) & 1u) {
+            if ((s_end >> s) & 1u) {
+              *reinterpret_cast<float4*>(ap + 4 * (c4 ^ (pr & 7))) = va;
+              if (zleft > 0) st_out(reinterpret_cast<float4*>(g.zout + zoff), va);
+              ++pr; ap += LDA_F; zoff += g.ldz; --zleft;
+              if (s + 1 < SCHED) {
+                z0 = __uint_as_float(((nshort >> (s + 1)) & 1u) << 31);
+                va = make_float4(z0, z0, z0, z0);
+              }
             }
           }
         }
+      };
+      if constexpr (BOUND) {
+        walk(I0{}, I8{});
+        if (more8) walk(I8{}, I16{});
+        if (more16) walk(I16{}, IS{});
+      } else {
+        walk(I0{}, IS{});
       }
       if constexpr (BIMG) {
         __builtin_amdgcn_sched_barrier(0);
@@ -670,7 +707,14 @@
         const unsigned olo = __shfl_xor((unsigned)(best & 0xFFFFFFFFull), 32, 64), ohi = __shfl_xor((unsigned)(best >> 32), 32, 64);
         const unsigned long long other = ((unsigned long long)ohi << 32) | olo;
         best = other > best ? other : best;
-        if (h == 0 && best && cn < g.N) atomicMax(&g.ro_packed[(int64_t)b * g.N + cn], best);
+        if (h == 0 && best && cn < g.N) {
+          if (!UNITS && g.ro_tab) {
+            const int j = b == ro_gf ? ro_j0 : 0;
+            if (j >= 0 && j < g.ro_J - 1 && b < g.ro_B) g.ro_tab[((int64_t)b * g.ro_J + j) * g.N + cn] = best;
+          }
+          else if (TSGNN_EXP_RO_PLAIN_STORE) g.ro_packed[(int64_t)b * g.N + cn] = best;
+          else atomicMax(&g.ro_packed[(int64_t)b * g.N + cn], best);
+        }
       }
     }
   }
diff --git a/two-stage-gnn_amd/graph.py b/two-stage-gnn_amd/graph.py
--- a/two-stage-gnn_amd/graph.py
+++ b/two-stage-gnn_amd/graph.py
@@ -366,6 +366,22 @@
             cache[key] = (torch.from_numpy(ro).to(self.device), ch)
         return cache[key]
 
+    def ro_panel_words(self, ncu=None):
+        if ncu is None:
+            ncu = torch.cuda.get_device_properties(self.device).multi_processor_count
+        cache = self.__dict__.setdefault("_ro_panel_words", {})
+        key = int(ncu)
+        if key not in cache:
+            words = None
+            if (self.sizes is not None and getattr(self, "ghost_slots_fixed", None) is None and self.n_rows > 0
+                    and not unit_cut(self.n_rows, key, self.panel_units)):
+                gp = np.concatenate([[0], np.cumsum(np.asarray(self.sizes, dtype=np.int64))])
+                first = 32 * np.arange(-(-self.n_rows // 32), dtype=np.int64)
+                owner = np.searchsorted(gp, first, side="right") - 1
+                words = torch.from_numpy((first // 32 - gp[owner] // 32).astype(np.int32)).to(self.device)
+            cache[key] = words
+        return cache[key]
+
     def bn_workspace(self, B, L, Fh, Fl, nslots):
         key = (B, L, Fh, Fl, nslots)
         ws = getattr(self, "_bn_ws", None)
@@ -376,6 +392,8 @@
                   "ghost": mp.register_clear_on_error(torch.zeros(max(2 * (L - 1), 2), dtype=torch.float32, device=self.device)),
                   "packed": mp.register_clear_on_error(torch.zeros(B * ((L - 1) * Fh + Fl) + Fl, dtype=torch.int64, device=self.device)),
                   "dirty": False}
+            ws["ro_J"] = -(-nslots // 32) + 2
+            ws["ro_tab"] = mp.register_clear_on_error(torch.zeros(B * ws["ro_J"] * Fl, dtype=torch.int64, device=self.device))
             self._bn_ws = ws
         return ws
 
diff --git a/two-stage-gnn_amd/sage_stack.py b/two-stage-gnn_amd/sage_stack.py
--- a/two-stage-gnn_amd/sage_stack.py
+++ b/two-stage-gnn_amd/sage_stack.py
@@ -44,6 +44,7 @@
 
 GATHER_SCHED = os.environ.get("TSGNN_GATHER_SCHED", "1") != "0"
 GATHER_SCHED_L0 = os.environ.get("TSGNN_GATHER_SCHED_L0", "1") != "0"
+RO_PANEL = os.environ.get("TSGNN_RO_PANEL", "0") != "0"
 DU_MAP = os.environ.get("TSGNN_DU_MAP", "1") != "0"
 SLABS_BESIDE = os.environ.get("TSGNN_SLABS_BESIDE", "1") != "0"
 NSLAB_MAX = int(os.environ.get("TSGNN_NSLAB_MAX", "0"))
@@ -160,7 +161,7 @@
             if ell_s is not None:
                 bnf = g.bn_workspace(B, L, Fh, Fl, sn)
                 if bnf["dirty"]:
-                    bnf["sums"].zero_(); bnf["ghost"].zero_(); bnf["packed"].zero_()
+                    bnf["sums"].zero_(); bnf["ghost"].zero_(); bnf["packed"].zero_(); bnf["ro_tab"].zero_()
                 bnf["dirty"] = True
                 packed = bnf["packed"]
         ctx.w_img = ctx.pack_desc = None
@@ -183,6 +184,10 @@
             ctx.w_img, ctx.pack_desc = w_img, pack_desc
             sch0, sch0_w = _gather_sched(g, layer0_k=Ws[0].size(0), fill=gs) if GATHER_SCHED_L0 else (None, 0)
             schs, schs_w = _gather_sched(g, slots=True)
+            ro_words = g.ro_panel_words() if (RO_PANEL and Fl == 128 and bnf["ro_J"] <= 40) else None
+            ro_arm = None
+            if ro_words is not None:
+                ro_arm = lambda t=bnf["ro_tab"], w=ro_words, J=bnf["ro_J"]: nat.call_nostream("ro_panel_arm", t, w, B, J, Fl)
             for l in range(L):
                 K, N = Ws[l].size(0), Ws[l].size(1)
                 v = torch.empty(R, N, dtype=torch.float32, device=dev)
@@ -200,6 +205,8 @@
                     pm, pr_ = saved[l - 1][3], saved[l - 1][4]
                     last = l == L - 1
                     e_, w_, tp_, tc_ = (schs, schs_w, None, None) if schs is not None else (ell_s, ell_w, tp, tc_s)
+                    if last and ro_arm is not None:
+                        nat.defer(ro_arm)
                     nat.call("sage_layer_fwd_bn_f32", e_, w_, tp_, tc_, saved[l - 1][1], saved[l - 1][1].stride(0), Ws[l], Ws[l].stride(0), bs[l],
                              v, v.stride(0), rinv, z, z.stride(0), g.n_rows, K, gs, g.graph_ptr, g.slot_count, B, sn, sg,
                              packed[(l - 1) * B * Fh:(l - 1) * B * Fh + B * Fh],
@@ -319,6 +326,8 @@
         y = torch.empty(B, C, dtype=torch.float32, device=dev)
         v_last = saved[-1][1]
         if bnf is not None:
+            if ro_arm is not None:
+                nat.defer(ro_arm)
             nat.call("packed_head_fwd_z_f32", packed, B, L, Fh, Fl, out, out.stride(0), arg, w1c, b1, w2c, b2, E, C, vec, y,
                      bnf["sums"], (L - 1) * 2 * sn)
             bnf["dirty"] = False
```

Result: slower. 245,100 graphs/s (-7.0%).
